# DegardinBruno/Kinetic-GAN

Measured on AMD Instinct MI355X. Metric: G+D train-step samples/sec, NTU (N,3,64,25) bs=64 at 1/2/4/8 MI355X, higher is better.
Workload: dtype f32; 1 GPU; ntu shapes (N,3,64,25), 60 classes, mlp4, G+D WGAN-GP iteration, 64 samples/GPU; global_batch=64, parallelism=dp1, launch=hipgraph

## Files before the change

include/kgan_hip.h:

```cpp
#ifndef KGAN_HIP_H
#define KGAN_HIP_H

#include <stdint.h>

#ifdef __cplusplus
extern "C" {
#endif

#define KG_ABI_VERSION 9

enum { KG_ACT_NONE = 0, KG_ACT_LRELU = 1, KG_ACT_TANH = 2 };
enum { KG_TAP_TIME = 0,
       KG_TAP_CHANBLOCK = 1  };

int         kg_abi_version(void);
const char* kg_arch(void);
const char* kg_last_error(void);
void        kg_reload_env(void);

typedef struct KgConvGroup {
    const float* x;  int64_t x_sN, x_sC;
    int32_t Cin, T_in, V_in;
    int32_t x_lead;
    const int32_t* vmap;
// ... 54 lines not shown
#define KG_WGRAD_TILE_32x64   3
#define KG_WGRAD_TILE_32x32   4
int     kg_wgrad_plan_info(const KgWgradArgs* a, int32_t* variant, int32_t* splits);

typedef struct KgWgradReduceJob {
    const float* ws;  float* dw;
    int64_t w_sT, w_sO, w_sI;
    int32_t taps, M, Cin, splits, accumulate;
} KgWgradReduceJob;
#define KG_WGRAD_REDUCE_MAX_JOBS 24
typedef struct KgWgradReduceJobs {
    int32_t njobs;
    KgWgradReduceJob job[KG_WGRAD_REDUCE_MAX_JOBS];
} KgWgradReduceJobs;
int     kg_wgrad_reduce_many(const KgWgradReduceJobs* jobs, void* stream);

int64_t kg_wgrad_many_workspace_bytes(const KgWgradArgs* jobs, int32_t njobs);
int     kg_wgrad_many(const KgWgradArgs* jobs, int32_t njobs, float* ws, int64_t ws_bytes, void* stream);
int     kg_wgrad_many_plan(const KgWgradArgs* jobs, int32_t njobs, int32_t* variant, int32_t* splits);

typedef struct KgAggArgs {
    int32_t N, C, K, V, W;
    int32_t T;
    int32_t rep;
    const float* a;
    const float* x;  int64_t x_sN, x_sC;
    const float* y;  int64_t y_sN, y_sC;
    float* out;  int64_t o_sN, o_sC;
    float* ws;  int64_t ws_bytes;
    int32_t a_transposed;
    int32_t defer_sum;
    const float* res;  int64_t r_sN, r_sC;  int32_t r_T, r_V, r_tstride;  const int32_t* r_inv;
    const float* mask;  int64_t m_sN, m_sC;  float slope;
} KgAggArgs;

int     kg_agg_expand(const KgAggArgs* a, void* stream);
int     kg_agg_reduce(const KgAggArgs* a, void* stream);
int64_t kg_agg_outer_workspace_bytes(const KgAggArgs* a);
int     kg_agg_outer(const KgAggArgs* a, void* stream);
int     kg_agg_outer_slabs(const KgAggArgs* a);
typedef struct KgOuterSumJob { const float* ws; float* out; int32_t nout, slabs; } KgOuterSumJob;
#define KG_OUTER_SUM_MAX_JOBS 16
typedef struct KgOuterSumJobs { int32_t njobs; KgOuterSumJob job[KG_OUTER_SUM_MAX_JOBS]; } KgOuterSumJobs;
int     kg_agg_outer_sum_many(const KgOuterSumJobs* jobs, void* stream);
int     kg_agg_outer_many(const KgAggArgs* jobs, int32_t njobs, void* stream);

typedef struct KgAggConvArgs {
    int32_t N, Cin, M, T, V, W, K;
    const float* x;  int64_t x_sN, x_sC;
    const float* a;  int32_t a_transposed;
    const int32_t* nbr;  int32_t pcount[3];
    const float* w;  int64_t w_sT, w_sO, w_sI;
    float* out;  int64_t o_sN, o_sC;
    const float* add;  int64_t a_sN, a_sC;  int32_t a_tstride;
    float* xa;  int64_t xa_sN, xa_sC;
} KgAggConvArgs;

int kg_aggconv_supported(const KgAggConvArgs* a);
int kg_aggconv(const KgAggConvArgs* a, void* stream);

typedef struct KgGenArgs {
    int32_t N, C, K, Cr, Tc, Vc, V, rep;
    const float* a;  const float* u;
    const float* b;
    const float* y;  float* y_out;  int64_t y_sN, y_sC;
    float* z;  int64_t z_sN, z_sC;
    float* zf;  int64_t zf_sN, zf_sC;
    const float* rs;  float* rs_out;  int64_t rs_sN, rs_sC;
    const float* rbias;
    float* r;  int64_t r_sN, r_sC;
} KgGenArgs;

int kg_gen_expand(const KgGenArgs* a, void* stream);
int kg_gen_fold(const KgGenArgs* a, void* stream);

typedef struct KgGenAdjJob {
    const float* dbt;
    const float* u;
    const float* a;
    float* out;
    int32_t K, Kd, V, Vc, accumulate;
} KgGenAdjJob;
#define KG_GEN_ADJ_MAX_JOBS 8
int kg_gen_adj_finish(const KgGenAdjJob* jobs, int32_t njobs, void* stream);

typedef struct KgGenPrepJob {
    const float* a;  const float* imp;  const float* u;
    float* aeff;  float* b;
    int32_t K, V, Vc;
} KgGenPrepJob;
int kg_gen_adj_prepare(const KgGenPrepJob* jobs, int32_t njobs, void* stream);

typedef struct KgGenTailArgs {
    int32_t N, C, T, V;  int32_t act;  float slope;
    const float* g;  int64_t g_sN, g_sC;
    const float* out;  int64_t o_sN, o_sC;
    const float* u;  int64_t u_sN, u_sC;  const float* mean_t;  const float* rstd_t;  const float* gamma_t;
    const float* r;  int64_t r_sN, r_sC;  const float* mean_r;  const float* rstd_r;  const float* gamma_r;
    const float* noise;
    float* coef;
    float* dgamma_t;  float* dbeta_t;  float* dgamma_r;  float* dbeta_r;  float* dnw;
    float* ws;  int64_t ws_bytes;  int32_t* counters;  int32_t counters_len;
    float* du;  int64_t du_sN, du_sC;
    float* dr;  int64_t dr_sN, dr_sC;
} KgGenTailArgs;
int64_t kg_gen_tail_workspace_bytes(const KgGenTailArgs* a);
int     kg_gen_tail_stats(const KgGenTailArgs* a, void* stream);
int     kg_gen_tail_apply(const KgGenTailArgs* a, void* stream);

typedef struct KgPlane { float* p;  int64_t sN, sC; } KgPlane;
typedef struct KgGenBnLayer {
    const float* gamma;  const float* beta;  float* running_mean;  float* running_var;  int64_t* num_batches_tracked;
    float momentum, eps;
    float* coef;
} KgGenBnLayer;
typedef struct KgGenBlockArgs {
    int32_t N, groups;
    int32_t Cin, C, K, Kp;
    int32_t Tc, Vc, T, V, rep;
    int32_t res_kind;
    int32_t bn_t;
    int32_t act;  float slope;
    KgPlane x;
    KgPlane pu, pr;  const float* pcoef_t;  const float* pcoef_r;  const float* pnoise;  const float* pnw;  int32_t pact;
    KgPlane xout;
    const float* wg;  const float* wr;  const float* br;  const float* wt;  const float* bt;
    const float* b;
    const float* u;
    KgPlane yc, z, r, uo;
    KgGenBnLayer bt_, br_;
    const float* noise;  const float* nw;  KgPlane out;
    float* ws;  int64_t ws_bytes;  int32_t* counters;  int32_t counters_len;
} KgGenBlockArgs;
typedef struct KgGenBlockBwdArgs {
    int32_t N;
    int32_t Cin, C, K, Kp, Tc, Vc, T, V, rep, res_kind, bn_t, act;  float slope;
    KgPlane g, out, uo, r;
    const float* coef;
    const float* wg;  const float* wr;  const float* wt;  const float* b;  const float* u;
    KgPlane du, dr, gyc, zf, gx;
    KgPlane px, pu, pr;  const float* pnoise;  int32_t pact;
    const float* pmean_t;  const float* prstd_t;  const float* pgamma_t;
    const float* pmean_r;  const float* prstd_r;  const float* pgamma_r;
    float* pcoef;  float* dgamma_t;  float* dbeta_t;  float* dgamma_r;  float* dbeta_r;  float* dnw;
    float* ws;  int64_t ws_bytes;  int32_t* counters;  int32_t counters_len;
} KgGenBlockBwdArgs;
int64_t kg_genblock_lds_bytes(const KgGenBlockArgs* a);
int64_t kg_genblock_workspace_bytes(const KgGenBlockArgs* a);
int     kg_genblock_fwd(const KgGenBlockArgs* a, void* stream);
int64_t kg_genblock_bwd_lds_bytes(const KgGenBlockBwdArgs* a);
int64_t kg_genblock_bwd_workspace_bytes(const KgGenBlockBwdArgs* a);
int     kg_genblock_bwd(const KgGenBlockBwdArgs* a, void* stream);

typedef struct KgRowsumArgs {
    int32_t N, C, T, V;
    const float* x;  int64_t x_sN, x_sC;
    const float* y;  int64_t y_sN, y_sC;
    const float* shift;
    int32_t want_second;
    float* out;
    float* ws;  int64_t ws_bytes;
    int32_t accumulate;
    float* out2;
} KgRowsumArgs;

int64_t kg_rowsum_workspace_bytes(const KgRowsumArgs* a);
int     kg_rowsum(const KgRowsumArgs* a, void* stream);
int64_t kg_rowsum_many_workspace_bytes(const KgRowsumArgs* jobs, int32_t njobs);
int     kg_rowsum_many(const KgRowsumArgs* jobs, int32_t njobs, float* ws, int64_t ws_bytes, void* stream);

typedef struct KgEltArgs {
    int32_t N, C, T, V;
    const float* x;  int64_t x_sN, x_sC;
    const float* r;  int64_t r_sN, r_sC;
    const float* noise;
    const float* sx; const float* bx; const float* sr; const float* br; const float* nw;
    float* out;  int64_t o_sN, o_sC;
    int32_t act;  float slope;
    int32_t groups;
    int64_t coef_gs;
} KgEltArgs;

int kg_act_bwd(const KgEltArgs* a, void* stream);
int kg_affine_act(const KgEltArgs* a, void* stream);

typedef struct KgBnArgs {
    int32_t N, C, T, V;
    const float* x;  int64_t x_sN, x_sC;
    const float* g;  int64_t g_sN, g_sC;
    const float* gamma; const float* beta;
    float* running_mean; float* running_var;
    int64_t* num_batches_tracked;
    const float* mean; const float* rstd;
    float momentum, eps;
    int32_t training;
    float* coef;
} KgBnArgs;

int kg_bn_fwd(const KgBnArgs* a, void* stream);
int kg_bn_bwd(const KgBnArgs* a, void* stream);

typedef struct KgBnJob {
    KgBnArgs a;
    int32_t groups;
} KgBnJob;

int64_t kg_bn_bwd_many_workspace_bytes(const KgBnArgs* jobs, int32_t njobs);
int     kg_bn_bwd_many(const KgBnArgs* jobs, int32_t njobs, float* ws, int64_t ws_bytes, int32_t* counters,
                       int32_t counters_len, void* stream);
int64_t kg_bn_fwd_many_workspace_bytes(const KgBnJob* jobs, int32_t njobs);
int     kg_bn_fwd_many(const KgBnJob* jobs, int32_t njobs, float* ws, int64_t ws_bytes, int32_t* counters,
                       int32_t counters_len, void* stream);

typedef struct KgGpArgs {
    int32_t N, C, T, V;
    const float* g;  int64_t g_sN, g_sC;
    float* nrm;
    float* gp;
    const float* gout;
    float* out;  int64_t o_sN, o_sC;
} KgGpArgs;

int kg_gp_fwd(const KgGpArgs* a, void* stream);
int kg_gp_bwd(const KgGpArgs* a, void* stream);

int kg_adam_step(float* p, const float* g, float* m, float* v, int64_t n,
                 float lr, float b1, float b2, float eps, const int32_t* step, float grad_scale,
                 void* stream);
int kg_adam_step_fused(float* p, float* g, float* m, float* v, int64_t n,
                       float lr, float b1, float b2, float eps, const int32_t* step, float grad_scale,
                       int32_t zero_grad, void* stream);
int kg_adam_step_ema(float* p, float* g, float* m, float* v, float* e, int64_t n,
                     float lr, float b1, float b2, float eps, const int32_t* step, float grad_scale,
                     int32_t zero_grad, float ema_decay, float ema_warmup, void* stream);

typedef struct KgHeadArgs {
    int32_t N, C, T, V;
    const float* h;  int64_t h_sN, h_sC;
    const float* w;  const float* b;
    float* v;
    const float* gv;
    float* g;  int64_t g_sN, g_sC;
    float slope;  int32_t masked;
    float* dw;  float* db;  int32_t accumulate;
} KgHeadArgs;
int kg_head_fwd(const KgHeadArgs* a, void* stream);
int kg_head_bwd(const KgHeadArgs* a, void* stream);
int kg_head_wgrad(const KgHeadArgs* a, void* stream);

typedef struct KgLabelBiasArgs {
    int32_t N, L, J, K, C, V, W, T;
    const int64_t* labels;
    const float* emb;
    const float* w;  int64_t w_sK, w_sC;
    const float* ak;
    float* zl;
    const float* gz;  int64_t gz_sN, gz_sC;
    float* demb;  float* dw;  int32_t accumulate;
    float* dak;  int32_t dak_accumulate;
    float* ws;  int64_t ws_bytes;
} KgLabelBiasArgs;
int     kg_label_bias_fwd(const KgLabelBiasArgs* a, void* stream);
int64_t kg_label_bias_workspace_bytes(const KgLabelBiasArgs* a);
int     kg_label_bias_bwd(const KgLabelBiasArgs* a, void* stream);
int     kg_aggconv_label(const KgAggConvArgs* a, const KgLabelBiasArgs* lb, void* stream);

typedef struct KgMixArgs {
    int32_t N, C, T, V;
    const float* real;  int64_t r_sN, r_sC;
    const float* fake;  int64_t f_sN, f_sC;
    const float* alpha;
    float* out;  int64_t o_sN, o_sC;
} KgMixArgs;
int kg_mix3(const KgMixArgs* a, void* stream);

typedef struct KgMaskedAdjArgs {
    int32_t n;
    const float* a;  const float* imp;  const int64_t* sel;
    float* ak;
    const float* g;  float* dimp;  int32_t accumulate;
} KgMaskedAdjArgs;
int kg_masked_adj_fwd(const KgMaskedAdjArgs* a, void* stream);
int kg_masked_adj_bwd(const KgMaskedAdjArgs* a, void* stream);

typedef struct KgLinearArgs {
    int32_t N, Din, Dout;
    int32_t L, J;
    const float* x;  int64_t x_ld;
    const float* emb;
    const int64_t* labels;
    const float* w;  const float* bias;
    float* y;  int64_t y_ld;
    int32_t act;  float slope;
    const float* g;  int64_t g_ld;
    float* gx;  int64_t gx_ld;  int32_t gx_cols;
    float* dw;  float* db;
    float* demb;
    int32_t accumulate;
} KgLinearArgs;
int kg_linear_fwd(const KgLinearArgs* a, void* stream);
int kg_linear_bwd(const KgLinearArgs* a, void* stream);
int kg_embed_bwd(const KgLinearArgs* a, void* stream);

#define KG_COMM_ID_BYTES 128
int kg_comm_unique_id(void* id);
int kg_comm_init(void** comm, int32_t rank, int32_t world, const void* id, int32_t device);
int kg_comm_world(const void* comm);
int kg_allreduce_flat(void* comm, float* buf, int64_t n, void* stream);
int kg_comm_destroy(void* comm);

int kg_peak_mfma_f32(float* sink, int32_t iters, double* flops, void* stream);
int kg_peak_copy(const float* src, float* dst, int64_t n, void* stream);

#define KG_MMD_MAX_BW 16
typedef struct KgMmdArgs {
    const float* x;  int64_t x_sp, x_sd, x_sg, x_sc;
    const float* y;  int64_t y_sp, y_sd, y_sg, y_sc;
    int32_t m, n, dim;
    int32_t groups, classes;
    int32_t nbw;
    double bw[KG_MMD_MAX_BW];
    float* mmd2;
    float* mmd;
    float* result;
    float* mean;
    void* ws;  int64_t ws_bytes;
} KgMmdArgs;
int64_t kg_mmd_workspace_bytes(const KgMmdArgs* a);
int     kg_mmd(const KgMmdArgs* a, void* stream);

#define KG_PRDC_MAX_K 32
#define KG_PRDC_MAX_POINTS 32768
typedef struct KgPrdcArgs {
    const float* real;  int64_t r_sc, r_sp, r_so;
    const float* fake;  int64_t f_sc, f_sp, f_so;
    int32_t n, m;
    int32_t d_outer, d_inner;
    int32_t classes, k;
    float* radii_real;
    float* radii_fake;
    int32_t* fake_hits;
    uint8_t* real_flags;
    int32_t* counts;
    float* values;
    float* mean;
    void* ws;  int64_t ws_bytes;
} KgPrdcArgs;
int64_t kg_prdc_workspace_bytes(const KgPrdcArgs* a);
int     kg_prdc(const KgPrdcArgs* a, void* stream);

#define KG_PRDC_MAX_SETS 4
typedef struct KgPrdcRadiiArgs {
    const float* x;  int64_t sc, sp, so;
    int32_t n, d_outer, d_inner, classes, k;
    float* radii;
} KgPrdcRadiiArgs;
typedef struct KgPrdcSetsArgs {
    const float* real;  int64_t r_sc, r_sp, r_so;
    const float* fake[KG_PRDC_MAX_SETS];  int64_t f_sc, f_sp, f_so;
    int32_t nsets;
    int32_t n, m;
    int32_t d_outer, d_inner;
    int32_t classes, k;
    const float* radii_real;
    float* radii_fake;
    int32_t* fake_hits;
    uint8_t* real_flags;
    int32_t* counts;
    float* values;
    float* mean;
    void* ws;  int64_t ws_bytes;
} KgPrdcSetsArgs;
int     kg_prdc_radii(const KgPrdcRadiiArgs* a, void* stream);
int64_t kg_prdc_sets_workspace_bytes(const KgPrdcSetsArgs* a);
int     kg_prdc_sets(const KgPrdcSetsArgs* a, void* stream);

#define KG_NN_MAX_K 32
#define KG_NN_MAX_POINTS 16777216
#define KG_NN_MAX_SPLIT 32
typedef struct KgNnArgs {
    const float* query;  int64_t q_sc, q_sp, q_so;
    const float* base;   int64_t b_sc, b_sp, b_so;
    int32_t Q, N;
    int32_t d_outer, d_inner;
    int32_t classes, k;
    int32_t exclude_self;
    int32_t q_affine, b_affine;
    float q_scale, q_shift, b_scale, b_shift;
    int32_t tile, split;
    int32_t* idx;
    float* d2;
    void* ws;  int64_t ws_bytes;
} KgNnArgs;
int64_t kg_nn_workspace_bytes(const KgNnArgs* a);
int     kg_nn(const KgNnArgs* a, void* stream);

#define KG_NN_MAX_SETS 4
#define KG_NN_SCORES_MAX_CLASSES 1024
typedef struct KgNnSetsArgs {
    const float* query[KG_NN_MAX_SETS];  int64_t q_sc, q_sp, q_so;
    int32_t nsets;
    const float* base;   int64_t b_sc, b_sp, b_so;
    int32_t Q, N;
    int32_t d_outer, d_inner;
    int32_t classes, k;
    int32_t q_affine, b_affine;
    float q_scale, q_shift, b_scale, b_shift;
    int32_t tile, split;
    int32_t* idx;
    float* d2;
    void* ws;  int64_t ws_bytes;
} KgNnSetsArgs;
typedef struct KgNnScoresArgs {
    int32_t nsets, Q, N, n_classes;
    int64_t ld;
    const int32_t* idx;  const float* d2;
    const int32_t* query_labels;
    const int32_t* base_labels;
    const float* base_loo;
    int64_t* counts;
    int32_t* counts_per_class;
    double* scores64;  float* scores;
} KgNnScoresArgs;
int64_t kg_nn_sets_workspace_bytes(const KgNnSetsArgs* a);
int     kg_nn_sets(const KgNnSetsArgs* a, void* stream);
int     kg_nn_scores(const KgNnScoresArgs* a, void* stream);

#define KG_NN_NORM_PARTS 64
typedef struct KgNnGramArgs {
    const float* query[KG_NN_MAX_SETS];  int64_t q_sc, q_sp, q_so;
    int32_t nsets;
    const float* base;   int64_t b_sc, b_sp, b_so;
    int32_t Q, N;
    int32_t d_outer, d_inner;
    int32_t classes, k;
    int32_t exclude_self;
    int32_t q_affine, b_affine;
    float q_scale, q_shift, b_scale, b_shift;
    int32_t cand;
    int32_t tile, split;
    const float* b_norms;
    const float* b_norm_parts;
    int32_t* idx;
    float* d2;
    int32_t* stats;
    void* ws;  int64_t ws_bytes;
} KgNnGramArgs;
int     kg_nn_norms(const KgNnGramArgs* a, float* norms, float* parts, void* stream);
int64_t kg_nn_gram_workspace_bytes(const KgNnGramArgs* a);
int     kg_nn_gram(const KgNnGramArgs* a, void* stream);

#define KG_FRECHET_MAX_DIM 96
typedef struct KgFrechetArgs {
    const float* real;  int64_t r_sc, r_ss, r_sf, r_so;
    const float* fake;  int64_t f_sc, f_ss, f_sf, f_so;
    int32_t n, m;
    int32_t frames;
    int32_t diff;
    int32_t d_outer, d_inner;
    int32_t classes;
    double* values;
    double* terms;
    double* mean;
    int32_t* sweeps;
    double* mu_real;
    double* mu_fake;
    double* cov_real;
    double* cov_fake;
    void* ws;  int64_t ws_bytes;
} KgFrechetArgs;
int64_t kg_frechet_workspace_bytes(const KgFrechetArgs* a);
int     kg_frechet(const KgFrechetArgs* a, void* stream);

#define KG_FRECHET_MAX_SETS 4
typedef struct KgFrechetRealArgs {
    const float* real;  int64_t r_sc, r_ss, r_sf, r_so;
    int32_t n;
    int32_t frames, diff;
    int32_t d_outer, d_inner;
    int32_t classes;
    double* mu_real;
    double* tr_real;
    double* G;
    int32_t* sweeps_real;
    void* ws;  int64_t ws_bytes;
} KgFrechetRealArgs;
typedef struct KgFrechetSetsArgs {
    const float* fake[KG_FRECHET_MAX_SETS];  int64_t f_sc, f_ss, f_sf, f_so;
    int32_t nsets;
    int32_t m;
    int32_t frames, diff;
    int32_t d_outer, d_inner;
    int32_t classes;
    const double* mu_real;
    const double* tr_real;
    const double* G;
    double* values;
    double* terms;
    int32_t* sweeps;
    double* mean;
    float* mean32;
    void* ws;  int64_t ws_bytes;
} KgFrechetSetsArgs;
int64_t kg_frechet_real_workspace_bytes(const KgFrechetRealArgs* a);
int     kg_frechet_real(const KgFrechetRealArgs* a, void* stream);
int64_t kg_frechet_sets_workspace_bytes(const KgFrechetSetsArgs* a);
int     kg_frechet_sets(const KgFrechetSetsArgs* a, void* stream);

#define KG_STEP_MAX_PLANES 8
#define KG_STREAM_Z 0
#define KG_STREAM_ALPHA 1
#define KG_STREAM_NOISE_D 2
#define KG_STREAM_NOISE_G 3
typedef struct KgStepInputsArgs {
    int64_t* step;
    int32_t* ticket;
    uint64_t seed;
    int32_t rank, world;
    int32_t B;
    int32_t C, T, V;
    const float* data;  int64_t d_sN, d_sC, d_sT, d_sV;
    int64_t n_rows;
    const int64_t* label_src;
    const int64_t* perm;  int64_t perm_stride;
    int64_t batches_per_epoch;
    float scale, shift;
    float* real;
    int64_t* labels;
    float* z;  int32_t latent;
    float* alpha;
    float* noise;  int32_t n_planes;  int64_t plane_len[KG_STEP_MAX_PLANES];
} KgStepInputsArgs;
int kg_step_inputs(const KgStepInputsArgs* a, void* stream);
int kg_loss_append(float* ring, int64_t ring_len, const int64_t* step, const float* d_loss, const float* g_loss,
                   void* stream);

#define KG_BN_EVAL_MAX_JOBS 8
typedef struct KgBnEvalJob {
    int32_t C;
    const float* gamma;  const float* beta;  const float* running_mean;  const float* running_var;
    float eps;
    float* coef;
} KgBnEvalJob;
int kg_bn_eval_coef(const KgBnEvalJob* jobs, int32_t njobs, void* stream);

typedef struct KgGenBlockInferArgs {
    int32_t N;
    int32_t Cin, C, K, Kp, Tc, Vc, T, V, rep, res_kind, act;  float slope;
    KgPlane x;
    const float* wg;  const float* wr;  const float* br;  const float* wt;  const float* bt;
    const float* b;
    const float* u;
    const float* coef_t;  const float* coef_r;
    const float* noise;  const float* nw;
    KgPlane out;
} KgGenBlockInferArgs;
int64_t kg_genblock_infer_lds_bytes(const KgGenBlockInferArgs* a);
int     kg_genblock_infer(const KgGenBlockInferArgs* a, void* stream);

#define KG_STREAM_SAMPLE 0x100
typedef struct KgSampleInputsArgs {
    int64_t* step;
    int32_t* ticket;
    uint64_t seed;
    int32_t B, latent;
    float* z;
    float* noise;  int64_t noise_len;
    float* t;  int32_t t_rows, t_cols;
} KgSampleInputsArgs;
int kg_sample_inputs(const KgSampleInputsArgs* a, void* stream);

int kg_trunc_lerp(float* x, int64_t x_ld, int32_t N, int32_t D, const float* t, int64_t t_ld, int32_t M, float truncation,
                  void* stream);

#define KG_EVAL_MAX_SCORES 8
typedef struct KgEvalRecordArgs {
    const float* scores[KG_EVAL_MAX_SCORES];
    int32_t nscores, select;
    const int64_t* iter;
    int64_t* count;
    float* ring_val;
    int64_t* ring_iter;
    int64_t ring_len;
    float* best_val;
    int64_t* best_iter;
    int32_t* flag;
} KgEvalRecordArgs;
int kg_eval_record(const KgEvalRecordArgs* a, void* stream);

#define KG_EVAL2_MAX_SCORES 32
typedef struct KgEvalRecord2Args {
    const float* scores[KG_EVAL2_MAX_SCORES];
    int32_t nscores, select;
    const int64_t* iter;
    int64_t* count;
    float* ring_val;
    int64_t* ring_iter;
    int64_t ring_len;
    float* best_val;
    int64_t* best_iter;
    int32_t* flag;
    int32_t maximise;
} KgEvalRecord2Args;
int kg_eval_record2(const KgEvalRecord2Args* a, void* stream);

#define KG_EVAL3_MAX_SCORES 64
// ... 124 lines not shown
```

kinetic-gan_amd/_native.py:

```python
from __future__ import annotations

import ctypes as C
import os
from typing import NamedTuple, Optional, Sequence, Tuple

import torch

_PKG = os.path.dirname(os.path.abspath(__file__))
LIB_PATH = os.environ.get("KG_LIB") or os.path.join(_PKG, "libkgan_hip.so")

ACT_NONE, ACT_LRELU, ACT_TANH = 0, 1, 2
ABI_VERSION = 9
TAP_TIME, TAP_CHANBLOCK = 0, 1

c_f32p = C.c_void_p
c_i32p = C.c_void_p


class _ConvGroup(C.Structure):
    _fields_ = [("x", c_f32p), ("x_sN", C.c_int64), ("x_sC", C.c_int64),
                ("Cin", C.c_int32), ("T_in", C.c_int32), ("V_in", C.c_int32),
                ("x_lead", C.c_int32),
                ("vmap", c_i32p),
                ("w", c_f32p), ("w_sT", C.c_int64), ("w_sO", C.c_int64), ("w_sI", C.c_int64),
                ("w_sMB", C.c_int64), ("w_MB", C.c_int32),
                ("taps", C.c_int32), ("tap_mode", C.c_int32), ("t_stride", C.c_int32),
                ("transposed", C.c_int32)]


class _ConvArgs(C.Structure):
    _fields_ = [("N", C.c_int32), ("M", C.c_int32), ("T_out", C.c_int32), ("V_out", C.c_int32),
                ("out", c_f32p), ("o_sN", C.c_int64), ("o_sC", C.c_int64),
                ("ngroups", C.c_int32),
                ("g", _ConvGroup * 2),
                ("bias0", c_f32p), ("bias1", c_f32p),
                ("add", c_f32p), ("a_sN", C.c_int64), ("a_sC", C.c_int64), ("a_tstride", C.c_int32),
                ("act", C.c_int32), ("slope", C.c_float),
                ("ws", c_f32p), ("ws_bytes", C.c_int64),
                ("mask", c_f32p), ("m_sN", C.c_int64), ("m_sC", C.c_int64),
                ("sync", C.c_void_p), ("sync_len", C.c_int32),
                ("o_tstride", C.c_int32),
                ("wpack", C.c_void_p), ("wpack_bytes", C.c_int64)]


class _WgradPair(C.Structure):
    _fields_ = [("N", C.c_int32),
                ("g", c_f32p), ("g_sN", C.c_int64), ("g_sC", C.c_int64),
                ("x", c_f32p), ("x_sN", C.c_int64), ("x_sC", C.c_int64)]


class _WgradArgs(C.Structure):
    _fields_ = [("N", C.c_int32), ("M", C.c_int32), ("T_out", C.c_int32), ("V_out", C.c_int32),
                ("g", c_f32p), ("g_sN", C.c_int64), ("g_sC", C.c_int64),
                ("x", c_f32p), ("x_sN", C.c_int64), ("x_sC", C.c_int64),
                ("Cin", C.c_int32), ("T_in", C.c_int32), ("V_in", C.c_int32),
                ("vmap", c_i32p),
                ("taps", C.c_int32), ("tap_mode", C.c_int32), ("t_stride", C.c_int32),
                ("dw", c_f32p), ("w_sT", C.c_int64), ("w_sO", C.c_int64), ("w_sI", C.c_int64),
                ("ws", c_f32p), ("ws_bytes", C.c_int64), ("accumulate", C.c_int32),
                ("nextra", C.c_int32), ("extra", _WgradPair * 2), ("defer_reduce", C.c_int32)]


class _WgradReduceJob(C.Structure):
    _fields_ = [("ws", c_f32p), ("dw", c_f32p), ("w_sT", C.c_int64), ("w_sO", C.c_int64), ("w_sI", C.c_int64),
                ("taps", C.c_int32), ("M", C.c_int32), ("Cin", C.c_int32), ("splits", C.c_int32),
                ("accumulate", C.c_int32)]


WGRAD_REDUCE_MAX_JOBS = 24
WGRAD_TILE_128x128, WGRAD_TILE_64x64, WGRAD_TILE_64x32, WGRAD_TILE_32x64, WGRAD_TILE_32x32 = 0, 1, 2, 3, 4
WGRAD_TILE_NAMES = {WGRAD_TILE_128x128: "128x128", WGRAD_TILE_64x64: "64x64", WGRAD_TILE_64x32: "64x32",
                    WGRAD_TILE_32x64: "32x64", WGRAD_TILE_32x32: "32x32"}
WGRAD_MAX_SPLITS = 128


class _WgradReduceJobs(C.Structure):
    _fields_ = [("njobs", C.c_int32), ("job", _WgradReduceJob * WGRAD_REDUCE_MAX_JOBS)]


class _AggArgs(C.Structure):
    _fields_ = [("N", C.c_int32), ("C", C.c_int32), ("K", C.c_int32), ("V", C.c_int32), ("W", C.c_int32),
                ("T", C.c_int32), ("rep", C.c_int32),
                ("a", c_f32p),
                ("x", c_f32p), ("x_sN", C.c_int64), ("x_sC", C.c_int64),
                ("y", c_f32p), ("y_sN", C.c_int64), ("y_sC", C.c_int64),
                ("out", c_f32p), ("o_sN", C.c_int64), ("o_sC", C.c_int64),
                ("ws", c_f32p), ("ws_bytes", C.c_int64), ("a_transposed", C.c_int32), ("defer_sum", C.c_int32),
                ("res", c_f32p), ("r_sN", C.c_int64), ("r_sC", C.c_int64), ("r_T", C.c_int32), ("r_V", C.c_int32),
                ("r_tstride", C.c_int32), ("r_inv", c_i32p),
                ("mask", c_f32p), ("m_sN", C.c_int64), ("m_sC", C.c_int64), ("slope", C.c_float)]


class _OuterSumJob(C.Structure):
    _fields_ = [("ws", c_f32p), ("out", c_f32p), ("nout", C.c_int32), ("slabs", C.c_int32)]


OUTER_SUM_MAX_JOBS = 16


class _OuterSumJobs(C.Structure):
    _fields_ = [("njobs", C.c_int32), ("job", _OuterSumJob * OUTER_SUM_MAX_JOBS)]


class _AggConvArgs(C.Structure):
    _fields_ = [("N", C.c_int32), ("Cin", C.c_int32), ("M", C.c_int32), ("T", C.c_int32), ("V", C.c_int32),
                ("W", C.c_int32), ("K", C.c_int32),
                ("x", c_f32p), ("x_sN", C.c_int64), ("x_sC", C.c_int64),
                ("a", c_f32p), ("a_transposed", C.c_int32),
                ("nbr", c_i32p), ("pcount", C.c_int32 * 3),
                ("w", c_f32p), ("w_sT", C.c_int64), ("w_sO", C.c_int64), ("w_sI", C.c_int64),
                ("out", c_f32p), ("o_sN", C.c_int64), ("o_sC", C.c_int64),
                ("add", c_f32p), ("a_sN", C.c_int64), ("a_sC", C.c_int64), ("a_tstride", C.c_int32),
                ("xa", c_f32p), ("xa_sN", C.c_int64), ("xa_sC", C.c_int64)]


class _RowsumArgs(C.Structure):
    _fields_ = [("N", C.c_int32), ("C", C.c_int32), ("T", C.c_int32), ("V", C.c_int32),
                ("x", c_f32p), ("x_sN", C.c_int64), ("x_sC", C.c_int64),
                ("y", c_f32p), ("y_sN", C.c_int64), ("y_sC", C.c_int64),
                ("shift", c_f32p),
                ("want_second", C.c_int32),
                ("out", c_f32p),
                ("ws", c_f32p), ("ws_bytes", C.c_int64), ("accumulate", C.c_int32), ("out2", c_f32p)]


class _BnArgs(C.Structure):
    _fields_ = [("N", C.c_int32), ("C", C.c_int32), ("T", C.c_int32), ("V", C.c_int32),
                ("x", c_f32p), ("x_sN", C.c_int64), ("x_sC", C.c_int64),
                ("g", c_f32p), ("g_sN", C.c_int64), ("g_sC", C.c_int64),
                ("gamma", c_f32p), ("beta", c_f32p),
                ("running_mean", c_f32p), ("running_var", c_f32p),
                ("num_batches_tracked", C.c_void_p),
                ("mean", c_f32p), ("rstd", c_f32p),
                ("momentum", C.c_float), ("eps", C.c_float),
                ("training", C.c_int32),
                ("coef", c_f32p)]


class _BnJob(C.Structure):
    _fields_ = [("a", _BnArgs), ("groups", C.c_int32)]


class _GpArgs(C.Structure):
    _fields_ = [("N", C.c_int32), ("C", C.c_int32), ("T", C.c_int32), ("V", C.c_int32),
                ("g", c_f32p), ("g_sN", C.c_int64), ("g_sC", C.c_int64),
                ("nrm", c_f32p), ("gp", c_f32p), ("gout", c_f32p),
                ("out", c_f32p), ("o_sN", C.c_int64), ("o_sC", C.c_int64)]


class _EltArgs(C.Structure):
    _fields_ = [("N", C.c_int32), ("C", C.c_int32), ("T", C.c_int32), ("V", C.c_int32),
                ("x", c_f32p), ("x_sN", C.c_int64), ("x_sC", C.c_int64),
                ("r", c_f32p), ("r_sN", C.c_int64), ("r_sC", C.c_int64),
                ("noise", c_f32p),
                ("sx", c_f32p), ("bx", c_f32p), ("sr", c_f32p), ("br", c_f32p), ("nw", c_f32p),
                ("out", c_f32p), ("o_sN", C.c_int64), ("o_sC", C.c_int64),
                ("act", C.c_int32), ("slope", C.c_float),
                ("groups", C.c_int32), ("coef_gs", C.c_int64)]


class _GenArgs(C.Structure):
    _fields_ = [("N", C.c_int32), ("C", C.c_int32), ("K", C.c_int32), ("Cr", C.c_int32), ("Tc", C.c_int32),
                ("Vc", C.c_int32), ("V", C.c_int32), ("rep", C.c_int32),
                ("a", c_f32p), ("u", c_f32p), ("b", c_f32p),
                ("y", c_f32p), ("y_out", c_f32p), ("y_sN", C.c_int64), ("y_sC", C.c_int64),
                ("z", c_f32p), ("z_sN", C.c_int64), ("z_sC", C.c_int64),
                ("zf", c_f32p), ("zf_sN", C.c_int64), ("zf_sC", C.c_int64),
                ("rs", c_f32p), ("rs_out", c_f32p), ("rs_sN", C.c_int64), ("rs_sC", C.c_int64),
                ("rbias", c_f32p),
                ("r", c_f32p), ("r_sN", C.c_int64), ("r_sC", C.c_int64)]


class _GenAdjJob(C.Structure):
    _fields_ = [("dbt", c_f32p), ("u", c_f32p), ("a", c_f32p), ("out", c_f32p),
                ("K", C.c_int32), ("Kd", C.c_int32), ("V", C.c_int32), ("Vc", C.c_int32), ("accumulate", C.c_int32)]


class _HeadArgs(C.Structure):
    _fields_ = [("N", C.c_int32), ("C", C.c_int32), ("T", C.c_int32), ("V", C.c_int32),
                ("h", c_f32p), ("h_sN", C.c_int64), ("h_sC", C.c_int64),
                ("w", c_f32p), ("b", c_f32p), ("v", c_f32p), ("gv", c_f32p),
                ("g", c_f32p), ("g_sN", C.c_int64), ("g_sC", C.c_int64),
                ("slope", C.c_float), ("masked", C.c_int32),
                ("dw", c_f32p), ("db", c_f32p), ("accumulate", C.c_int32)]


class _LinearArgs(C.Structure):
    _fields_ = [("N", C.c_int32), ("Din", C.c_int32), ("Dout", C.c_int32), ("L", C.c_int32), ("J", C.c_int32),
                ("x", c_f32p), ("x_ld", C.c_int64), ("emb", c_f32p), ("labels", C.c_void_p),
                ("w", c_f32p), ("bias", c_f32p), ("y", c_f32p), ("y_ld", C.c_int64),
                ("act", C.c_int32), ("slope", C.c_float),
                ("g", c_f32p), ("g_ld", C.c_int64),
                ("gx", c_f32p), ("gx_ld", C.c_int64), ("gx_cols", C.c_int32),
                ("dw", c_f32p), ("db", c_f32p), ("demb", c_f32p), ("accumulate", C.c_int32)]


class _LabelBiasArgs(C.Structure):
    _fields_ = [("N", C.c_int32), ("L", C.c_int32), ("J", C.c_int32), ("K", C.c_int32), ("C", C.c_int32),
                ("V", C.c_int32), ("W", C.c_int32), ("T", C.c_int32),
                ("labels", C.c_void_p), ("emb", c_f32p),
                ("w", c_f32p), ("w_sK", C.c_int64), ("w_sC", C.c_int64),
                ("ak", c_f32p), ("zl", c_f32p),
                ("gz", c_f32p), ("gz_sN", C.c_int64), ("gz_sC", C.c_int64),
                ("demb", c_f32p), ("dw", c_f32p), ("accumulate", C.c_int32),
                ("dak", c_f32p), ("dak_accumulate", C.c_int32),
                ("ws", c_f32p), ("ws_bytes", C.c_int64)]


class _MixArgs(C.Structure):
    _fields_ = [("N", C.c_int32), ("C", C.c_int32), ("T", C.c_int32), ("V", C.c_int32),
                ("real", c_f32p), ("r_sN", C.c_int64), ("r_sC", C.c_int64),
                ("fake", c_f32p), ("f_sN", C.c_int64), ("f_sC", C.c_int64),
                ("alpha", c_f32p),
                ("out", c_f32p), ("o_sN", C.c_int64), ("o_sC", C.c_int64)]


class _MaskedAdjArgs(C.Structure):
    _fields_ = [("n", C.c_int32), ("a", c_f32p), ("imp", c_f32p), ("sel", C.c_void_p), ("ak", c_f32p),
                ("g", c_f32p), ("dimp", c_f32p), ("accumulate", C.c_int32)]


class _GenTailArgs(C.Structure):
    _fields_ = [("N", C.c_int32), ("C", C.c_int32), ("T", C.c_int32), ("V", C.c_int32), ("act", C.c_int32), ("slope", C.c_float),
                ("g", c_f32p), ("g_sN", C.c_int64), ("g_sC", C.c_int64),
                ("out", c_f32p), ("o_sN", C.c_int64), ("o_sC", C.c_int64),
                ("u", c_f32p), ("u_sN", C.c_int64), ("u_sC", C.c_int64), ("mean_t", c_f32p), ("rstd_t", c_f32p), ("gamma_t", c_f32p),
                ("r", c_f32p), ("r_sN", C.c_int64), ("r_sC", C.c_int64), ("mean_r", c_f32p), ("rstd_r", c_f32p), ("gamma_r", c_f32p),
                ("noise", c_f32p), ("coef", c_f32p),
                ("dgamma_t", c_f32p), ("dbeta_t", c_f32p), ("dgamma_r", c_f32p), ("dbeta_r", c_f32p), ("dnw", c_f32p),
                ("ws", c_f32p), ("ws_bytes", C.c_int64), ("counters", C.c_void_p), ("counters_len", C.c_int32),
                ("du", c_f32p), ("du_sN", C.c_int64), ("du_sC", C.c_int64),
                ("dr", c_f32p), ("dr_sN", C.c_int64), ("dr_sC", C.c_int64)]


class _GenPrepJob(C.Structure):
    _fields_ = [("a", c_f32p), ("imp", c_f32p), ("u", c_f32p), ("aeff", c_f32p), ("b", c_f32p),
                ("K", C.c_int32), ("V", C.c_int32), ("Vc", C.c_int32)]


class _Plane(C.Structure):
    _fields_ = [("p", c_f32p), ("sN", C.c_int64), ("sC", C.c_int64)]


class _GenBnLayer(C.Structure):
    _fields_ = [("gamma", c_f32p), ("beta", c_f32p), ("running_mean", c_f32p), ("running_var", c_f32p),
                ("num_batches_tracked", C.c_void_p), ("momentum", C.c_float), ("eps", C.c_float), ("coef", c_f32p)]


class _GenBlockArgs(C.Structure):
    _fields_ = [("N", C.c_int32), ("groups", C.c_int32),
                ("Cin", C.c_int32), ("C", C.c_int32), ("K", C.c_int32), ("Kp", C.c_int32),
                ("Tc", C.c_int32), ("Vc", C.c_int32), ("T", C.c_int32), ("V", C.c_int32), ("rep", C.c_int32),
                ("res_kind", C.c_int32), ("bn_t", C.c_int32), ("act", C.c_int32), ("slope", C.c_float),
                ("x", _Plane),
                ("pu", _Plane), ("pr", _Plane), ("pcoef_t", c_f32p), ("pcoef_r", c_f32p), ("pnoise", c_f32p), ("pnw", c_f32p),
                ("pact", C.c_int32), ("xout", _Plane),
                ("wg", c_f32p), ("wr", c_f32p), ("br", c_f32p), ("wt", c_f32p), ("bt", c_f32p),
                ("b", c_f32p), ("u", c_f32p),
                ("yc", _Plane), ("z", _Plane), ("r", _Plane), ("uo", _Plane),
                ("bt_", _GenBnLayer), ("br_", _GenBnLayer),
                ("noise", c_f32p), ("nw", c_f32p), ("out", _Plane),
                ("ws", c_f32p), ("ws_bytes", C.c_int64), ("counters", C.c_void_p), ("counters_len", C.c_int32)]


class _GenBlockBwdArgs(C.Structure):
    _fields_ = [("N", C.c_int32),
                ("Cin", C.c_int32), ("C", C.c_int32), ("K", C.c_int32), ("Kp", C.c_int32),
                ("Tc", C.c_int32), ("Vc", C.c_int32), ("T", C.c_int32), ("V", C.c_int32), ("rep", C.c_int32),
                ("res_kind", C.c_int32), ("bn_t", C.c_int32), ("act", C.c_int32), ("slope", C.c_float),
                ("g", _Plane), ("out", _Plane), ("uo", _Plane), ("r", _Plane),
                ("coef", c_f32p),
                ("wg", c_f32p), ("wr", c_f32p), ("wt", c_f32p), ("b", c_f32p), ("u", c_f32p),
                ("du", _Plane), ("dr", _Plane), ("gyc", _Plane), ("zf", _Plane), ("gx", _Plane),
                ("px", _Plane), ("pu", _Plane), ("pr", _Plane), ("pnoise", c_f32p), ("pact", C.c_int32),
                ("pmean_t", c_f32p), ("prstd_t", c_f32p), ("pgamma_t", c_f32p),
                ("pmean_r", c_f32p), ("prstd_r", c_f32p), ("pgamma_r", c_f32p),
                ("pcoef", c_f32p), ("dgamma_t", c_f32p), ("dbeta_t", c_f32p), ("dgamma_r", c_f32p), ("dbeta_r", c_f32p),
                ("dnw", c_f32p),
                ("ws", c_f32p), ("ws_bytes", C.c_int64), ("counters", C.c_void_p), ("counters_len", C.c_int32)]



MMD_MAX_BW = 16


class _MmdArgs(C.Structure):
    _fields_ = [("x", c_f32p), ("x_sp", C.c_int64), ("x_sd", C.c_int64), ("x_sg", C.c_int64), ("x_sc", C.c_int64),
                ("y", c_f32p), ("y_sp", C.c_int64), ("y_sd", C.c_int64), ("y_sg", C.c_int64), ("y_sc", C.c_int64),
                ("m", C.c_int32), ("n", C.c_int32), ("dim", C.c_int32),
                ("groups", C.c_int32), ("classes", C.c_int32), ("nbw", C.c_int32),
                ("bw", C.c_double * MMD_MAX_BW),
                ("mmd2", c_f32p), ("mmd", c_f32p), ("result", c_f32p), ("mean", c_f32p),
                ("ws", C.c_void_p), ("ws_bytes", C.c_int64)]

PRDC_MAX_K = 32
PRDC_MAX_POINTS = 32768


class _PrdcArgs(C.Structure):
    _fields_ = [("real", c_f32p), ("r_sc", C.c_int64), ("r_sp", C.c_int64), ("r_so", C.c_int64),
                ("fake", c_f32p), ("f_sc", C.c_int64), ("f_sp", C.c_int64), ("f_so", C.c_int64),
                ("n", C.c_int32), ("m", C.c_int32), ("d_outer", C.c_int32), ("d_inner", C.c_int32),
                ("classes", C.c_int32), ("k", C.c_int32),
                ("radii_real", c_f32p), ("radii_fake", c_f32p), ("fake_hits", C.c_void_p), ("real_flags", C.c_void_p),
                ("counts", C.c_void_p), ("values", c_f32p), ("mean", c_f32p),
                ("ws", C.c_void_p), ("ws_bytes", C.c_int64)]

PRDC_MAX_SETS = 4


class _PrdcRadiiArgs(C.Structure):
    _fields_ = [("x", c_f32p), ("sc", C.c_int64), ("sp", C.c_int64), ("so", C.c_int64),
                ("n", C.c_int32), ("d_outer", C.c_int32), ("d_inner", C.c_int32), ("classes", C.c_int32), ("k", C.c_int32),
                ("radii", c_f32p)]


class _PrdcSetsArgs(C.Structure):
    _fields_ = [("real", c_f32p), ("r_sc", C.c_int64), ("r_sp", C.c_int64), ("r_so", C.c_int64),
                ("fake", c_f32p * PRDC_MAX_SETS), ("f_sc", C.c_int64), ("f_sp", C.c_int64), ("f_so", C.c_int64),
                ("nsets", C.c_int32), ("n", C.c_int32), ("m", C.c_int32), ("d_outer", C.c_int32), ("d_inner", C.c_int32),
                ("classes", C.c_int32), ("k", C.c_int32),
                ("radii_real", c_f32p), ("radii_fake", c_f32p), ("fake_hits", C.c_void_p), ("real_flags", C.c_void_p),
                ("counts", C.c_void_p), ("values", c_f32p), ("mean", c_f32p),
                ("ws", C.c_void_p), ("ws_bytes", C.c_int64)]

NN_MAX_K = 32
NN_MAX_POINTS = 1 << 24
NN_MAX_SPLIT = 32


class _NnArgs(C.Structure):
    _fields_ = [("query", c_f32p), ("q_sc", C.c_int64), ("q_sp", C.c_int64), ("q_so", C.c_int64),
                ("base", c_f32p), ("b_sc", C.c_int64), ("b_sp", C.c_int64), ("b_so", C.c_int64),
                ("Q", C.c_int32), ("N", C.c_int32), ("d_outer", C.c_int32), ("d_inner", C.c_int32),
                ("classes", C.c_int32), ("k", C.c_int32), ("exclude_self", C.c_int32),
                ("q_affine", C.c_int32), ("b_affine", C.c_int32),
                ("q_scale", C.c_float), ("q_shift", C.c_float), ("b_scale", C.c_float), ("b_shift", C.c_float),
                ("tile", C.c_int32), ("split", C.c_int32),
                ("idx", C.c_void_p), ("d2", c_f32p),
                ("ws", C.c_void_p), ("ws_bytes", C.c_int64)]

NN_MAX_SETS = 4
NN_SCORES_MAX_CLASSES = 1024


class _NnSetsArgs(C.Structure):
    _fields_ = [("query", c_f32p * NN_MAX_SETS), ("q_sc", C.c_int64), ("q_sp", C.c_int64), ("q_so", C.c_int64),
                ("nsets", C.c_int32),
                ("base", c_f32p), ("b_sc", C.c_int64), ("b_sp", C.c_int64), ("b_so", C.c_int64),
                ("Q", C.c_int32), ("N", C.c_int32), ("d_outer", C.c_int32), ("d_inner", C.c_int32),
                ("classes", C.c_int32), ("k", C.c_int32),
                ("q_affine", C.c_int32), ("b_affine", C.c_int32),
                ("q_scale", C.c_float), ("q_shift", C.c_float), ("b_scale", C.c_float), ("b_shift", C.c_float),
                ("tile", C.c_int32), ("split", C.c_int32),
                ("idx", C.c_void_p), ("d2", c_f32p),
                ("ws", C.c_void_p), ("ws_bytes", C.c_int64)]


NN_NORM_PARTS = 64


class _NnGramArgs(C.Structure):
    _fields_ = [("query", c_f32p * NN_MAX_SETS), ("q_sc", C.c_int64), ("q_sp", C.c_int64), ("q_so", C.c_int64),
                ("nsets", C.c_int32),
                ("base", c_f32p), ("b_sc", C.c_int64), ("b_sp", C.c_int64), ("b_so", C.c_int64),
                ("Q", C.c_int32), ("N", C.c_int32), ("d_outer", C.c_int32), ("d_inner", C.c_int32),
                ("classes", C.c_int32), ("k", C.c_int32), ("exclude_self", C.c_int32),
                ("q_affine", C.c_int32), ("b_affine", C.c_int32),
                ("q_scale", C.c_float), ("q_shift", C.c_float), ("b_scale", C.c_float), ("b_shift", C.c_float),
                ("cand", C.c_int32), ("tile", C.c_int32), ("split", C.c_int32),
                ("b_norms", c_f32p), ("b_norm_parts", c_f32p),
                ("idx", C.c_void_p), ("d2", c_f32p), ("stats", C.c_void_p),
                ("ws", C.c_void_p), ("ws_bytes", C.c_int64)]


class _NnScoresArgs(C.Structure):
    _fields_ = [("nsets", C.c_int32), ("Q", C.c_int32), ("N", C.c_int32), ("n_classes", C.c_int32),
                ("ld", C.c_int64),
                ("idx", C.c_void_p), ("d2", c_f32p),
                ("query_labels", C.c_void_p), ("base_labels", C.c_void_p), ("base_loo", c_f32p),
                ("counts", C.c_void_p), ("counts_per_class", C.c_void_p),
                ("scores64", C.c_void_p), ("scores", c_f32p)]

FRECHET_MAX_DIM = 96


class _FrechetArgs(C.Structure):
    _fields_ = [("real", c_f32p), ("r_sc", C.c_int64), ("r_ss", C.c_int64), ("r_sf", C.c_int64), ("r_so", C.c_int64),
                ("fake", c_f32p), ("f_sc", C.c_int64), ("f_ss", C.c_int64), ("f_sf", C.c_int64), ("f_so", C.c_int64),
                ("n", C.c_int32), ("m", C.c_int32), ("frames", C.c_int32), ("diff", C.c_int32),
                ("d_outer", C.c_int32), ("d_inner", C.c_int32), ("classes", C.c_int32),
                ("values", C.c_void_p), ("terms", C.c_void_p), ("mean", C.c_void_p), ("sweeps", C.c_void_p),
                ("mu_real", C.c_void_p), ("mu_fake", C.c_void_p), ("cov_real", C.c_void_p), ("cov_fake", C.c_void_p),
                ("ws", C.c_void_p), ("ws_bytes", C.c_int64)]

FRECHET_MAX_SETS = 4


class _FrechetRealArgs(C.Structure):
    _fields_ = [("real", c_f32p), ("r_sc", C.c_int64), ("r_ss", C.c_int64), ("r_sf", C.c_int64), ("r_so", C.c_int64),
                ("n", C.c_int32), ("frames", C.c_int32), ("diff", C.c_int32),
                ("d_outer", C.c_int32), ("d_inner", C.c_int32), ("classes", C.c_int32),
                ("mu_real", C.c_void_p), ("tr_real", C.c_void_p), ("G", C.c_void_p), ("sweeps_real", C.c_void_p),
                ("ws", C.c_void_p), ("ws_bytes", C.c_int64)]


class _FrechetSetsArgs(C.Structure):
    _fields_ = [("fake", c_f32p * FRECHET_MAX_SETS), ("f_sc", C.c_int64), ("f_ss", C.c_int64), ("f_sf", C.c_int64),
                ("f_so", C.c_int64),
                ("nsets", C.c_int32), ("m", C.c_int32), ("frames", C.c_int32), ("diff", C.c_int32),
                ("d_outer", C.c_int32), ("d_inner", C.c_int32), ("classes", C.c_int32),
                ("mu_real", C.c_void_p), ("tr_real", C.c_void_p), ("G", C.c_void_p),
                ("values", C.c_void_p), ("terms", C.c_void_p), ("sweeps", C.c_void_p), ("mean", C.c_void_p),
                ("mean32", c_f32p),
                ("ws", C.c_void_p), ("ws_bytes", C.c_int64)]

KIN_DESC = 6
KIN_MAX_JOINTS, KIN_MAX_BONES, KIN_MAX_MIRROR = 32, 32, 16
KIN_MIN_FRAMES = 4
KIN_MAX_ELEMS = 32768
KIN_MAX_SETS = 4
KIN_MAX_POINTS = 16384


class _KinDescArgs(C.Structure):
    _fields_ = [("x", c_f32p), ("sc", C.c_int64), ("ss", C.c_int64), ("sf", C.c_int64), ("so", C.c_int64),
                ("n", C.c_int32), ("T", C.c_int32), ("C", C.c_int32), ("V", C.c_int32), ("classes", C.c_int32),
                ("B", C.c_int32), ("M", C.c_int32),
                ("bones", C.c_void_p), ("mirror", C.c_void_p), ("still_eps", C.c_double),
                ("desc", c_f32p), ("degenerate", C.c_void_p),
                ("ws", c_f32p), ("ws_bytes", C.c_int64), ("counters", C.c_void_p), ("counters_len", C.c_int32)]


class _KinDescSetsArgs(C.Structure):
    _fields_ = [("x", c_f32p * KIN_MAX_SETS), ("sc", C.c_int64), ("ss", C.c_int64), ("sf", C.c_int64), ("so", C.c_int64),
                ("nsets", C.c_int32),
                ("n", C.c_int32), ("T", C.c_int32), ("C", C.c_int32), ("V", C.c_int32), ("classes", C.c_int32),
                ("B", C.c_int32), ("M", C.c_int32),
                ("bones", C.c_void_p), ("mirror", C.c_void_p), ("still_eps", C.c_double),
                ("desc", c_f32p * KIN_MAX_SETS), ("degenerate", C.c_void_p),
                ("ws", c_f32p), ("ws_bytes", C.c_int64), ("counters", C.c_void_p), ("counters_len", C.c_int32)]


class _KinScoresArgs(C.Structure):
    _fields_ = [("real", c_f32p), ("fake", c_f32p * KIN_MAX_SETS),
                ("nsets", C.c_int32), ("n", C.c_int32), ("m", C.c_int32), ("classes", C.c_int32),
                ("mean_real", C.c_void_p), ("mean_fake", C.c_void_p), ("w1", C.c_void_p), ("w1_mean", C.c_void_p),
                ("scores", c_f32p), ("nonfinite", C.c_void_p)]

STEP_MAX_PLANES = 8
STREAM_Z, STREAM_ALPHA, STREAM_NOISE_D, STREAM_NOISE_G = 0, 1, 2, 3


class _StepInputsArgs(C.Structure):
    _fields_ = [("step", C.c_void_p), ("ticket", C.c_void_p), ("seed", C.c_uint64),
                ("rank", C.c_int32), ("world", C.c_int32), ("B", C.c_int32),
                ("C", C.c_int32), ("T", C.c_int32), ("V", C.c_int32),
                ("data", c_f32p), ("d_sN", C.c_int64), ("d_sC", C.c_int64), ("d_sT", C.c_int64), ("d_sV", C.c_int64),
                ("n_rows", C.c_int64), ("label_src", C.c_void_p),
                ("perm", C.c_void_p), ("perm_stride", C.c_int64), ("batches_per_epoch", C.c_int64),
                ("scale", C.c_float), ("shift", C.c_float),
                ("real", c_f32p), ("labels", C.c_void_p),
                ("z", c_f32p), ("latent", C.c_int32), ("alpha", c_f32p),
                ("noise", c_f32p), ("n_planes", C.c_int32), ("plane_len", C.c_int64 * STEP_MAX_PLANES)]

BN_EVAL_MAX_JOBS = 8
STREAM_SAMPLE = 0x100


class _BnEvalJob(C.Structure):
    _fields_ = [("C", C.c_int32), ("gamma", c_f32p), ("beta", c_f32p), ("running_mean", c_f32p), ("running_var", c_f32p),
                ("eps", C.c_float), ("coef", c_f32p)]


class _GenBlockInferArgs(C.Structure):
    _fields_ = [("N", C.c_int32),
                ("Cin", C.c_int32), ("C", C.c_int32), ("K", C.c_int32), ("Kp", C.c_int32),
                ("Tc", C.c_int32), ("Vc", C.c_int32), ("T", C.c_int32), ("V", C.c_int32), ("rep", C.c_int32),
                ("res_kind", C.c_int32), ("act", C.c_int32), ("slope", C.c_float),
                ("x", _Plane),
                ("wg", c_f32p), ("wr", c_f32p), ("br", c_f32p), ("wt", c_f32p), ("bt", c_f32p),
                ("b", c_f32p), ("u", c_f32p),
                ("coef_t", c_f32p), ("coef_r", c_f32p),
                ("noise", c_f32p), ("nw", c_f32p), ("out", _Plane)]


class _SampleInputsArgs(C.Structure):
    _fields_ = [("step", C.c_void_p), ("ticket", C.c_void_p), ("seed", C.c_uint64),
                ("B", C.c_int32), ("latent", C.c_int32), ("z", c_f32p),
                ("noise", c_f32p), ("noise_len", C.c_int64),
                ("t", c_f32p), ("t_rows", C.c_int32), ("t_cols", C.c_int32)]

GEN_ADJ_MAX_JOBS = 8
EVAL_MAX_SCORES = 8
COPY_IF_MAX_JOBS = 32


def _eval_record_struct(name: str, most: int, sense: bool):
    fields = [("scores", c_f32p * most), ("nscores", C.c_int32), ("select", C.c_int32),
              ("iter", C.c_void_p), ("count", C.c_void_p), ("ring_val", c_f32p), ("ring_iter", C.c_void_p),
              ("ring_len", C.c_int64), ("best_val", c_f32p), ("best_iter", C.c_void_p), ("flag", C.c_void_p)]
    return type(name, (C.Structure,), {"_fields_": fields + ([("maximise", C.c_int32)] if sense else [])})


EVAL2_MAX_SCORES = 32
EVAL3_MAX_SCORES = 64
_EvalRecordArgs = _eval_record_struct("_EvalRecordArgs", EVAL_MAX_SCORES, False)
_EvalRecord2Args = _eval_record_struct("_EvalRecord2Args", EVAL2_MAX_SCORES, True)
_EvalRecord3Args = _eval_record_struct("_EvalRecord3Args", EVAL3_MAX_SCORES, True)


class _CopyJob(C.Structure):
    _fields_ = [("src", C.c_void_p), ("dst", C.c_void_p), ("nwords", C.c_int64)]


CLS_TILE = 4
CLS_MAX_C = 1024
CLS_MAX_CLASSES = 1024


class _ClsHeadArgs(C.Structure):
    _fields_ = [("N", C.c_int32), ("C", C.c_int32), ("T", C.c_int32), ("V", C.c_int32), ("F", C.c_int32), ("L", C.c_int32),
                ("h", c_f32p), ("h_sN", C.c_int64), ("h_sC", C.c_int64),
                ("w1", c_f32p), ("b1", c_f32p), ("w2", c_f32p), ("b2", c_f32p),
                ("labels", C.c_void_p),
                ("slope", C.c_float), ("masked", C.c_int32),
                ("pooled", c_f32p), ("feat", c_f32p), ("logits", c_f32p), ("loss_per_sample", c_f32p),
                ("pred", C.c_void_p), ("loss", c_f32p), ("correct", C.c_void_p),
                ("gtop", c_f32p),
                ("g", c_f32p), ("g_sN", C.c_int64), ("g_sC", C.c_int64),
                ("dw1", c_f32p), ("db1", c_f32p), ("dw2", c_f32p), ("db2", c_f32p), ("accumulate", C.c_int32),
                ("ws", C.c_void_p), ("ws_bytes", C.c_int64)]


CLS_MAX_SETS = 4


class _ClsScoresArgs(C.Structure):
    _fields_ = [("nsets", C.c_int32), ("N", C.c_int32), ("F", C.c_int32), ("K", C.c_int32), ("Sd", C.c_int32), ("Sl", C.c_int32),
                ("feat_ld", C.c_int64),
                ("feat", c_f32p * CLS_MAX_SETS), ("pred", C.c_void_p * CLS_MAX_SETS),
                ("labels", C.c_void_p), ("div_pairs", C.c_void_p), ("mm_pairs", C.c_void_p),
                ("dist", C.c_void_p), ("scores64", C.c_void_p), ("scores", c_f32p),
                ("correct", C.c_void_p), ("correct_per_class", C.c_void_p), ("count_per_class", C.c_void_p)]


EXPORTS = {
    "kg_abi_version": (C.c_int, []),
    "kg_arch": (C.c_char_p, []),
    "kg_last_error": (C.c_char_p, []),
    "kg_reload_env": (None, []),
    "kg_peak_mfma_f32": (C.c_int, [C.c_void_p, C.c_int32, C.POINTER(C.c_double), C.c_void_p]),
    "kg_peak_copy": (C.c_int, [C.c_void_p, C.c_void_p, C.c_int64, C.c_void_p]),
    "kg_conv_workspace_bytes": (C.c_int64, [C.POINTER(_ConvArgs)]),
    "kg_conv_plan_info": (C.c_int, [C.POINTER(_ConvArgs), C.POINTER(C.c_int32), C.POINTER(C.c_int32)]),
    "kg_conv": (C.c_int, [C.POINTER(_ConvArgs), C.c_void_p]),
    "kg_conv_pack_bytes": (C.c_int64, [C.POINTER(_ConvArgs)]),
    "kg_conv_pack": (C.c_int, [C.POINTER(_ConvArgs), C.c_void_p, C.c_int64, C.c_void_p]),
    "kg_conv_many": (C.c_int, [C.POINTER(_ConvArgs), C.c_int32, C.c_void_p]),
    "kg_conv_many_plan": (C.c_int, [C.POINTER(_ConvArgs), C.c_int32, C.POINTER(C.c_int32)]),
    "kg_wgrad_workspace_bytes": (C.c_int64, [C.POINTER(_WgradArgs)]),
    "kg_wgrad": (C.c_int, [C.POINTER(_WgradArgs), C.c_void_p]),
    "kg_wgrad_plan_info": (C.c_int, [C.POINTER(_WgradArgs), C.POINTER(C.c_int32), C.POINTER(C.c_int32)]),
    "kg_wgrad_reduce_many": (C.c_int, [C.POINTER(_WgradReduceJobs), C.c_void_p]),
    "kg_wgrad_many_workspace_bytes": (C.c_int64, [C.POINTER(_WgradArgs), C.c_int32]),
    "kg_wgrad_many": (C.c_int, [C.POINTER(_WgradArgs), C.c_int32, C.c_void_p, C.c_int64, C.c_void_p]),
    "kg_wgrad_many_plan": (C.c_int, [C.POINTER(_WgradArgs), C.c_int32, C.POINTER(C.c_int32), C.POINTER(C.c_int32)]),
    "kg_aggconv_supported": (C.c_int, [C.POINTER(_AggConvArgs)]),
    "kg_aggconv": (C.c_int, [C.POINTER(_AggConvArgs), C.c_void_p]),
    "kg_agg_expand": (C.c_int, [C.POINTER(_AggArgs), C.c_void_p]),
    "kg_agg_reduce": (C.c_int, [C.POINTER(_AggArgs), C.c_void_p]),
    "kg_agg_outer_workspace_bytes": (C.c_int64, [C.POINTER(_AggArgs)]),
    "kg_agg_outer": (C.c_int, [C.POINTER(_AggArgs), C.c_void_p]),
    "kg_agg_outer_slabs": (C.c_int, [C.POINTER(_AggArgs)]),
    "kg_agg_outer_many": (C.c_int, [C.POINTER(_AggArgs), C.c_int32, C.c_void_p]),
    "kg_agg_outer_sum_many": (C.c_int, [C.POINTER(_OuterSumJobs), C.c_void_p]),
    "kg_gen_expand": (C.c_int, [C.POINTER(_GenArgs), C.c_void_p]),
    "kg_gen_fold": (C.c_int, [C.POINTER(_GenArgs), C.c_void_p]),
    "kg_gen_adj_finish": (C.c_int, [C.POINTER(_GenAdjJob), C.c_int32, C.c_void_p]),
    "kg_gen_tail_workspace_bytes": (C.c_int64, [C.POINTER(_GenTailArgs)]),
    "kg_gen_tail_stats": (C.c_int, [C.POINTER(_GenTailArgs), C.c_void_p]),
    "kg_gen_tail_apply": (C.c_int, [C.POINTER(_GenTailArgs), C.c_void_p]),
    "kg_gen_adj_prepare": (C.c_int, [C.POINTER(_GenPrepJob), C.c_int32, C.c_void_p]),
    "kg_genblock_lds_bytes": (C.c_int64, [C.POINTER(_GenBlockArgs)]),
    "kg_genblock_workspace_bytes": (C.c_int64, [C.POINTER(_GenBlockArgs)]),
    "kg_genblock_fwd": (C.c_int, [C.POINTER(_GenBlockArgs), C.c_void_p]),
    "kg_genblock_bwd_lds_bytes": (C.c_int64, [C.POINTER(_GenBlockBwdArgs)]),
    "kg_genblock_bwd_workspace_bytes": (C.c_int64, [C.POINTER(_GenBlockBwdArgs)]),
    "kg_genblock_bwd": (C.c_int, [C.POINTER(_GenBlockBwdArgs), C.c_void_p]),
    "kg_head_fwd": (C.c_int, [C.POINTER(_HeadArgs), C.c_void_p]),
    "kg_head_bwd": (C.c_int, [C.POINTER(_HeadArgs), C.c_void_p]),
    "kg_head_wgrad": (C.c_int, [C.POINTER(_HeadArgs), C.c_void_p]),
    "kg_linear_fwd": (C.c_int, [C.POINTER(_LinearArgs), C.c_void_p]),
    "kg_linear_bwd": (C.c_int, [C.POINTER(_LinearArgs), C.c_void_p]),
    "kg_embed_bwd": (C.c_int, [C.POINTER(_LinearArgs), C.c_void_p]),
    "kg_label_bias_fwd": (C.c_int, [C.POINTER(_LabelBiasArgs), C.c_void_p]),
    "kg_label_bias_workspace_bytes": (C.c_int64, [C.POINTER(_LabelBiasArgs)]),
    "kg_label_bias_bwd": (C.c_int, [C.POINTER(_LabelBiasArgs), C.c_void_p]),
    "kg_aggconv_label": (C.c_int, [C.POINTER(_AggConvArgs), C.POINTER(_LabelBiasArgs), C.c_void_p]),
    "kg_mix3": (C.c_int, [C.POINTER(_MixArgs), C.c_void_p]),
    "kg_masked_adj_fwd": (C.c_int, [C.POINTER(_MaskedAdjArgs), C.c_void_p]),
    "kg_masked_adj_bwd": (C.c_int, [C.POINTER(_MaskedAdjArgs), C.c_void_p]),
    "kg_rowsum_workspace_bytes": (C.c_int64, [C.POINTER(_RowsumArgs)]),
    "kg_rowsum": (C.c_int, [C.POINTER(_RowsumArgs), C.c_void_p]),
    "kg_rowsum_many_workspace_bytes": (C.c_int64, [C.POINTER(_RowsumArgs), C.c_int32]),
    "kg_rowsum_many": (C.c_int, [C.POINTER(_RowsumArgs), C.c_int32, C.c_void_p, C.c_int64, C.c_void_p]),
    "kg_bn_fwd": (C.c_int, [C.POINTER(_BnArgs), C.c_void_p]),
    "kg_bn_bwd_many_workspace_bytes": (C.c_int64, [C.POINTER(_BnArgs), C.c_int32]),
    "kg_bn_bwd_many": (C.c_int, [C.POINTER(_BnArgs), C.c_int32, c_f32p, C.c_int64, C.c_void_p, C.c_int32, C.c_void_p]),
    "kg_bn_fwd_many_workspace_bytes": (C.c_int64, [C.POINTER(_BnJob), C.c_int32]),
    "kg_bn_fwd_many": (C.c_int, [C.POINTER(_BnJob), C.c_int32, c_f32p, C.c_int64, C.c_void_p, C.c_int32, C.c_void_p]),
    "kg_bn_bwd": (C.c_int, [C.POINTER(_BnArgs), C.c_void_p]),
    "kg_gp_fwd": (C.c_int, [C.POINTER(_GpArgs), C.c_void_p]),
    "kg_gp_bwd": (C.c_int, [C.POINTER(_GpArgs), C.c_void_p]),
    "kg_act_bwd": (C.c_int, [C.POINTER(_EltArgs), C.c_void_p]),
    "kg_affine_act": (C.c_int, [C.POINTER(_EltArgs), C.c_void_p]),
    "kg_comm_unique_id": (C.c_int, [C.c_void_p]),
    "kg_comm_init": (C.c_int, [C.POINTER(C.c_void_p), C.c_int32, C.c_int32, C.c_void_p, C.c_int32]),
    "kg_comm_world": (C.c_int, [C.c_void_p]),
    "kg_allreduce_flat": (C.c_int, [C.c_void_p, C.c_void_p, C.c_int64, C.c_void_p]),
    "kg_comm_destroy": (C.c_int, [C.c_void_p]),
    "kg_adam_step": (C.c_int, [C.c_void_p, C.c_void_p, C.c_void_p, C.c_void_p, C.c_int64, C.c_float, C.c_float,
                               C.c_float, C.c_float, C.c_void_p, C.c_float, C.c_void_p]),
    "kg_mmd_workspace_bytes": (C.c_int64, [C.POINTER(_MmdArgs)]),
    "kg_mmd": (C.c_int, [C.POINTER(_MmdArgs), C.c_void_p]),
    "kg_prdc_workspace_bytes": (C.c_int64, [C.POINTER(_PrdcArgs)]),
    "kg_prdc": (C.c_int, [C.POINTER(_PrdcArgs), C.c_void_p]),
    "kg_prdc_radii": (C.c_int, [C.POINTER(_PrdcRadiiArgs), C.c_void_p]),
    "kg_prdc_sets_workspace_bytes": (C.c_int64, [C.POINTER(_PrdcSetsArgs)]),
    "kg_prdc_sets": (C.c_int, [C.POINTER(_PrdcSetsArgs), C.c_void_p]),
    "kg_nn_workspace_bytes": (C.c_int64, [C.POINTER(_NnArgs)]),
    "kg_nn": (C.c_int, [C.POINTER(_NnArgs), C.c_void_p]),
    "kg_nn_sets_workspace_bytes": (C.c_int64, [C.POINTER(_NnSetsArgs)]),
    "kg_nn_sets": (C.c_int, [C.POINTER(_NnSetsArgs), C.c_void_p]),
    "kg_nn_scores": (C.c_int, [C.POINTER(_NnScoresArgs), C.c_void_p]),
    "kg_nn_norms": (C.c_int, [C.POINTER(_NnGramArgs), C.c_void_p, C.c_void_p, C.c_void_p]),
    "kg_nn_gram_workspace_bytes": (C.c_int64, [C.POINTER(_NnGramArgs)]),
    "kg_nn_gram": (C.c_int, [C.POINTER(_NnGramArgs), C.c_void_p]),
    "kg_frechet_workspace_bytes": (C.c_int64, [C.POINTER(_FrechetArgs)]),
    "kg_frechet": (C.c_int, [C.POINTER(_FrechetArgs), C.c_void_p]),
    "kg_frechet_real_workspace_bytes": (C.c_int64, [C.POINTER(_FrechetRealArgs)]),
    "kg_frechet_real": (C.c_int, [C.POINTER(_FrechetRealArgs), C.c_void_p]),
    "kg_frechet_sets_workspace_bytes": (C.c_int64, [C.POINTER(_FrechetSetsArgs)]),
    "kg_frechet_sets": (C.c_int, [C.POINTER(_FrechetSetsArgs), C.c_void_p]),
    "kg_step_inputs": (C.c_int, [C.POINTER(_StepInputsArgs), C.c_void_p]),
    "kg_loss_append": (C.c_int, [C.c_void_p, C.c_int64, C.c_void_p, C.c_void_p, C.c_void_p, C.c_void_p]),
    "kg_adam_step_fused": (C.c_int, [C.c_void_p, C.c_void_p, C.c_void_p, C.c_void_p, C.c_int64, C.c_float, C.c_float,
                                     C.c_float, C.c_float, C.c_void_p, C.c_float, C.c_int32, C.c_void_p]),
    "kg_adam_step_ema": (C.c_int, [C.c_void_p, C.c_void_p, C.c_void_p, C.c_void_p, C.c_void_p, C.c_int64, C.c_float, C.c_float,
                                   C.c_float, C.c_float, C.c_void_p, C.c_float, C.c_int32, C.c_float, C.c_float, C.c_void_p]),
    "kg_bn_eval_coef": (C.c_int, [C.POINTER(_BnEvalJob), C.c_int32, C.c_void_p]),
    "kg_genblock_infer_lds_bytes": (C.c_int64, [C.POINTER(_GenBlockInferArgs)]),
    "kg_genblock_infer": (C.c_int, [C.POINTER(_GenBlockInferArgs), C.c_void_p]),
    "kg_sample_inputs": (C.c_int, [C.POINTER(_SampleInputsArgs), C.c_void_p]),
    "kg_trunc_lerp": (C.c_int, [C.c_void_p, C.c_int64, C.c_int32, C.c_int32, C.c_void_p, C.c_int64, C.c_int32, C.c_float,
                                C.c_void_p]),
    "kg_eval_record": (C.c_int, [C.POINTER(_EvalRecordArgs), C.c_void_p]),
    "kg_eval_record2": (C.c_int, [C.POINTER(_EvalRecord2Args), C.c_void_p]),
    "kg_eval_record3": (C.c_int, [C.POINTER(_EvalRecord3Args), C.c_void_p]),
    "kg_copy_if": (C.c_int, [C.c_void_p, C.POINTER(_CopyJob), C.c_int32, C.c_void_p]),
    "kg_cls_head_workspace_bytes": (C.c_int64, [C.POINTER(_ClsHeadArgs)]),
    "kg_cls_head_fwd": (C.c_int, [C.POINTER(_ClsHeadArgs), C.c_void_p]),
    "kg_cls_head_bwd": (C.c_int, [C.POINTER(_ClsHeadArgs), C.c_void_p]),
    "kg_cls_head_wgrad": (C.c_int, [C.POINTER(_ClsHeadArgs), C.c_void_p]),
    "kg_cls_scores": (C.c_int, [C.POINTER(_ClsScoresArgs), C.c_void_p]),
    "kg_kin_desc_workspace_bytes": (C.c_int64, [C.POINTER(_KinDescArgs)]),
    "kg_kin_desc_lds_bytes": (C.c_int64, [C.POINTER(_KinDescArgs)]),
    "kg_kin_desc": (C.c_int, [C.POINTER(_KinDescArgs), C.c_void_p]),
    "kg_kin_desc_sets_workspace_bytes": (C.c_int64, [C.POINTER(_KinDescSetsArgs)]),
    "kg_kin_desc_sets_lds_bytes": (C.c_int64, [C.POINTER(_KinDescSetsArgs)]),
    "kg_kin_desc_sets": (C.c_int, [C.POINTER(_KinDescSetsArgs), C.c_void_p]),
    "kg_kin_scores_lds_bytes": (C.c_int64, [C.POINTER(_KinScoresArgs)]),
    "kg_kin_scores": (C.c_int, [C.POINTER(_KinScoresArgs), C.c_void_p]),
}

_lib = None


def load_library():
    global _lib
    if _lib is not None:
        return _lib
    if not os.path.exists(LIB_PATH):
        raise RuntimeError(
            f"{LIB_PATH} is missing: run `python -c 'import __graft_entry__ as g; g.build()'` "
            "(hipcc --offload-arch=gfx950). There is no CPU fallback for the st_gcn path.")
    lib = C.CDLL(LIB_PATH)
    for name, (res, args) in EXPORTS.items():
        fn = getattr(lib, name)
        fn.restype = res
        fn.argtypes = args
    if lib.kg_abi_version() != ABI_VERSION:
        raise RuntimeError("libkgan_hip.so ABI version mismatch")
    _lib = lib
    return lib


def _check(rc: int, what: str):
    if rc != 0:
        msg = load_library().kg_last_error().decode()
        raise RuntimeError(f"{what} failed (rc={rc}): {msg}")


def _stream() -> int:
    return torch.cuda.current_stream().cuda_stream


def peak_mfma_f32(sink: torch.Tensor, iters: int) -> float:
    fl = C.c_double(0.0)
    _check(load_library().kg_peak_mfma_f32(sink.data_ptr(), int(iters), C.byref(fl), _stream()), "kg_peak_mfma_f32")
    return fl.value


def peak_copy(src: torch.Tensor, dst: torch.Tensor) -> int:
    n = src.numel()
    _check(load_library().kg_peak_copy(src.data_ptr(), dst.data_ptr(), n, _stream()), "kg_peak_copy")
    return 8 * n


def reload_env():
    load_library().kg_reload_env()


SYNC_LEN = 8192
_sync_bufs = {}


def _sync_buffer(device) -> torch.Tensor:
    key = (device.index, torch.cuda.current_stream(device).cuda_stream)
    buf = _sync_bufs.get(key)
    if buf is None:
        buf = _sync_bufs[key] = torch.zeros(SYNC_LEN, dtype=torch.int32, device=device)
    return buf



def is_plane(x: torch.Tensor) -> bool:
    if x.dim() != 4:
        return False
    n, c, t, v = x.shape
    return (v == 1 or x.stride(3) == 1) and (t == 1 or x.stride(2) == v)


def as_plane(x: torch.Tensor) -> torch.Tensor:
    if x.dtype != torch.float32:
        raise TypeError(f"st_gcn path is fp32 only, got {x.dtype}")
    if is_plane(x):
        return x
    out = new_plane(x.shape[0], x.shape[1], x.shape[2], x.shape[3], x.device)
    out.copy_(x)
    return out


PLANE_LEAD = 32


def new_plane(n, c, t, v, device, zero=False) -> torch.Tensor:
    numel = c * n * t * v
    buf = (torch.zeros if zero else torch.empty)(numel + PLANE_LEAD, dtype=torch.float32, device=device)
    return buf[PLANE_LEAD:].view(c, n, t, v).permute(1, 0, 2, 3)


def _sn_sc(x: torch.Tensor):
    n, c, t, v = x.shape
    sn = x.stride(0) if n > 1 else t * v
    sc = x.stride(1) if c > 1 else t * v
    return sn, sc


def _need_cuda(*ts):
    cur = None
    for t in ts:
        if t is None:
            continue
        if not t.is_cuda:
            raise RuntimeError("kinetic_gan_amd: the st_gcn hot path runs on the GPU only "
                               "(tensor on %s); there is no CPU fallback" % t.device)
        if cur is None:
            cur = torch.cuda.current_device()
        if t.device.index != cur:
            raise RuntimeError("kinetic_gan_amd: tensor on %s but the current device is cuda:%d - select the device "
                               "first (torch.cuda.set_device / `with torch.cuda.device(...)`)" % (t.device, cur))


def _ptr(t: Optional[torch.Tensor]):
    return None if t is None else t.data_ptr()


def _bind(a, field: str, pre: str, t: torch.Tensor, convert: bool = False) -> torch.Tensor:
    if convert:
        t = as_plane(t)
    setattr(a, field, t.data_ptr())
    sn, sc = _sn_sc(t)
    setattr(a, pre + "_sN", sn)
    setattr(a, pre + "_sC", sc)
    return t


def _query(query: str, a, count: Optional[int] = None) -> int:
    fn = getattr(load_library(), query)
    nbytes = fn(C.byref(a)) if count is None else fn(a, count)
    if nbytes < 0:
        _check(-1, query)
    return nbytes


def _workspace(query: str, a, device, count: Optional[int] = None, tickets: Optional[str] = None, lazy: bool = False):
    nbytes = _query(query, a, count)
    if lazy and nbytes == 0:
        return None
    ws = torch.empty(nbytes // 4 if lazy else max(1, nbytes // 4), dtype=torch.float32, device=device)
    if count is None:
        a.ws, a.ws_bytes = ws.data_ptr(), nbytes if lazy else ws.numel() * 4
        if tickets is not None:
            sync = _sync_buffer(device)
            setattr(a, tickets, sync.data_ptr())
            setattr(a, tickets + "_len", sync.numel())
    return ws


def _dest(t: torch.Tensor, n: int, msg: str) -> torch.Tensor:
    if t.numel() != n or not t.is_contiguous() or t.dtype != torch.float32:
        raise ValueError(msg)
    return t


def _chunks(jobs: Sequence, most: int):
    for i in range(0, len(jobs), most):
        yield jobs[i:i + most]



class WView(NamedTuple):
    sT: int
    sO: int
    sI: int
    sMB: int = 0
    MB: int = 1 << 30


class Group(NamedTuple):
    x: torch.Tensor
    w: torch.Tensor
    wv: WView
    Cin: int
    taps: int = 1
    tap_mode: int = TAP_TIME
    t_stride: int = 1
    transposed: bool = False
    vmap: Optional[torch.Tensor] = None


last_conv_plan = None

flop_count = None


def _count(kind: str, flops: float):
    if flop_count is not None:
        flop_count[kind] = flop_count.get(kind, 0.0) + float(flops)


def _conv_args(groups: Sequence[Group], N: int, M: int, T_out: int, V_out: int,
               bias0=None, bias1=None, add=None, add_tstride: int = 1,
               act: int = ACT_NONE, slope: float = 0.2, mask=None, out: Optional[torch.Tensor] = None, out_t0: int = 0,
               out_tstride: int = 1, wpack: Optional[torch.Tensor] = None, alloc_out: bool = True):
    a = _ConvArgs()
    if wpack is not None:
        _need_cuda(wpack)
        a.wpack, a.wpack_bytes = wpack.data_ptr(), wpack.numel() * wpack.element_size()
    a.N, a.M, a.T_out, a.V_out = N, M, T_out, V_out
    keep = []
    dev = groups[0].x.device
    a.ngroups = len(groups)
    for i, g in enumerate(groups):
        x = as_plane(g.x)
        w = g.w if g.w.is_contiguous() else g.w.contiguous()
        _need_cuda(x, w, g.vmap)
        keep += [x, w]
        cg = a.g[i]
        _bind(cg, "x", "x", x)
        cg.Cin, cg.T_in, cg.V_in = g.Cin, x.shape[2], x.shape[3]
        cg.x_lead = min(int(x.storage_offset()), 1 << 20)
        cg.vmap = _ptr(g.vmap)
        cg.w = w.data_ptr()
        cg.w_sT, cg.w_sO, cg.w_sI, cg.w_sMB = g.wv.sT, g.wv.sO, g.wv.sI, g.wv.sMB
        cg.w_MB = min(g.wv.MB, 1 << 30)
        cg.taps, cg.tap_mode, cg.t_stride, cg.transposed = g.taps, g.tap_mode, g.t_stride, int(g.transposed)
    if out is None and not alloc_out:
        pass
    elif out is None:
        out = new_plane(N, M, T_out, V_out, dev)
        a.out = out.data_ptr()
    else:
        if (not is_plane(out) or out.shape[0] != N or out.shape[1] != M or out.shape[3] != V_out
                or out_t0 + (T_out - 1) * out_tstride >= out.shape[2] or out_tstride < 1 or out_t0 < 0):
            raise ValueError("conv: out must be a plane tensor (N, M, T, V_out) that holds frames out_t0 + to * out_tstride")
        _need_cuda(out)
# ... 404 lines not shown
    gy = grs = zf = None
    if gz is not None:
        gz = as_plane(gz)
        c = gz.shape[1]
        a.C, a.K = c, K
        _bind(a, "z", "z", gz)
        gy = y_out if y_out is not None else new_plane(n, K * c, tc, vc, gz.device)
        assert tuple(gy.shape) == (n, K * c, tc, vc) and is_plane(gy)
        _bind(a, "y_out", "y", gy)
        if want_zf:
            zf = gz if rep == 1 else _bind(a, "zf", "zf", new_plane(n, c, tc, v, gz.device))
        _count("kg_agg", 2.0 * K * vc * v * c * n * tf)
    if gr is not None:
        gr = as_plane(gr)
        a.Cr = gr.shape[1]
        _bind(a, "r", "r", gr)
        grs = rs_out if rs_out is not None else new_plane(n, gr.shape[1], tc, vc, gr.device)
        assert tuple(grs.shape) == (n, gr.shape[1], tc, vc) and is_plane(grs)
        _bind(a, "rs_out", "rs", grs)
        _count("kg_agg", 2.0 * vc * v * gr.shape[1] * n * tf)
    _check(lib.kg_gen_fold(C.byref(a), _stream()), "kg_gen_fold")
    return gy, grs, zf


def gen_tail_bwd(g, out, act: int, u=None, bn_t=None, r=None, bn_r=None, noise=None, sinks=None, slope: float = 0.2,
                 coef: Optional[torch.Tensor] = None, stats_only: bool = False):
    lib = load_library()
    g, out = as_plane(g), as_plane(out)
    n, c, t, v = g.shape
    sinks = sinks or {}
    a = _GenTailArgs()
    a.N, a.C, a.T, a.V, a.act, a.slope = n, c, t, v, act, slope
    _bind(a, "g", "g", g)
    _bind(a, "out", "o", out)
    keep = [g, out]
    if bn_t is not None:
        u = as_plane(u)
        gam, mean, rstd = (_vec(q, c, "gen_tail_bwd") for q in bn_t)
        _bind(a, "u", "u", u)
        a.gamma_t, a.mean_t, a.rstd_t = _ptr(gam), mean.data_ptr(), rstd.data_ptr()
        keep += [u, gam, mean, rstd]
    if r is not None:
        r = _bind(a, "r", "r", r, True)
        keep.append(r)
        if bn_r is not None:
            gam, mean, rstd = (_vec(q, c, "gen_tail_bwd") for q in bn_r)
            a.gamma_r, a.mean_r, a.rstd_r = _ptr(gam), mean.data_ptr(), rstd.data_ptr()
            keep += [gam, mean, rstd]
    if noise is not None:
        noise = noise.contiguous()
        a.noise = noise.data_ptr()
        keep.append(noise)
    _need_cuda(*keep, *sinks.values())
    for k_, t_ in sinks.items():
        if t_ is not None and (t_.numel() != c or not t_.is_contiguous()):
            raise ValueError("gen_tail_bwd: sink %s must be a contiguous (C,) tensor" % k_)
    a.dgamma_t, a.dbeta_t = _ptr(sinks.get("gamma_t")), _ptr(sinks.get("beta_t"))
    a.dgamma_r, a.dbeta_r, a.dnw = _ptr(sinks.get("gamma_r")), _ptr(sinks.get("beta_r")), _ptr(sinks.get("nw"))
    have_coef = coef is not None
    if have_coef:
        if tuple(coef.shape) != (6, c) or not coef.is_contiguous():
            raise ValueError("gen_tail_bwd: coef must be a contiguous (6, C) tensor")
        _need_cuda(coef)
    else:
        coef = torch.empty((6, c), dtype=torch.float32, device=g.device)
    a.coef = coef.data_ptr()
    if not have_coef:
        if c > SYNC_LEN:
            raise ValueError("gen_tail_bwd: %d channels exceed the %d ticket counters" % (c, SYNC_LEN))
        ws = _workspace("kg_gen_tail_workspace_bytes", a, g.device, tickets="counters")
        _check(lib.kg_gen_tail_stats(C.byref(a), _stream()), "kg_gen_tail_stats")
    if stats_only:
        return coef
    du = _bind(a, "du", "du", new_plane(n, c, t, v, g.device))
    dr = None
    if r is not None:
        dr = du if bn_t is None and bn_r is None else _bind(a, "dr", "dr", new_plane(n, c, t, v, g.device))
    _check(lib.kg_gen_tail_apply(C.byref(a), _stream()), "kg_gen_tail_apply")
    return du, dr


def gen_adj_finish(jobs: Sequence[dict]):
    lib = load_library()
    for chunk in _chunks(jobs, GEN_ADJ_MAX_JOBS):
        arr = (_GenAdjJob * len(chunk))()
        for q, j in enumerate(chunk):
            dbt, out = j["dbt"], j["out"]
            _need_cuda(dbt, j.get("u"), j.get("a"), out)
            assert dbt.is_contiguous() and out.is_contiguous() and dbt.dim() == 3 and out.dim() == 3
            k, v, _ = out.shape
            kd, v2, vc = dbt.shape
            assert v2 == v and kd <= k, (dbt.shape, out.shape)
            e = arr[q]
            e.dbt, e.u, e.a, e.out = dbt.data_ptr(), _ptr(j.get("u")), _ptr(j.get("a")), out.data_ptr()
            e.K, e.Kd, e.V, e.Vc, e.accumulate = k, kd, v, vc, int(bool(j.get("accumulate", False)))
        _check(lib.kg_gen_adj_finish(arr, len(chunk), _stream()), "kg_gen_adj_finish")



def _plane(t: Optional[torch.Tensor]) -> _Plane:
    p = _Plane()
    if t is not None:
        if not is_plane(t) or t.dtype != torch.float32:
            raise ValueError("genblock: plane tensor expected, got %s / strides %s" % (tuple(t.shape), t.stride()))
        p.p = t.data_ptr()
        p.sN, p.sC = _sn_sc(t)
    return p


class GenBlockDims(NamedTuple):
    Cin: int
    C: int
    K: int
    Kp: int
    Tc: int
    Vc: int
    T: int
    V: int
    rep: int
    res_kind: int
    bn_t: bool
    act: int


def _gb_common(a, d: GenBlockDims, slope):
    a.Cin, a.C, a.K, a.Kp, a.Tc, a.Vc, a.T, a.V, a.rep = d.Cin, d.C, d.K, d.Kp, d.Tc, d.Vc, d.T, d.V, d.rep
    a.res_kind, a.bn_t, a.act, a.slope = d.res_kind, int(d.bn_t), d.act, slope


def _gb_weights(a, wg, wr, wt, B, U):
    for t in (wg, wr, wt, B, U):
        if t is not None and (not t.is_contiguous() or t.dtype != torch.float32):
            raise ValueError("genblock: weights / adjacency must be contiguous fp32")
    a.wg, a.wr, a.wt, a.b, a.u = wg.data_ptr(), _ptr(wr), wt.data_ptr(), B.data_ptr(), _ptr(U)


def genblock_supported(d: GenBlockDims, n: int, wg, wr, wt, backward: bool = False) -> bool:
    lib = load_library()
    if backward:
        a = _GenBlockBwdArgs()
        a.N = n
        _gb_common(a, d, 0.2)
        return lib.kg_genblock_bwd_lds_bytes(C.byref(a)) >= 0
    a = _GenBlockArgs()
    a.N, a.groups = n, 1
    _gb_common(a, d, 0.2)
    a.wg, a.wr, a.wt = wg.data_ptr(), _ptr(wr), wt.data_ptr()
    return lib.kg_genblock_lds_bytes(C.byref(a)) >= 0


def _gb_bn(layer: _GenBnLayer, bn: dict, c: int, groups: int, device):
    vecs = [_vec(bn.get(k), c, "genblock_fwd") for k in ("gamma", "beta", "running_mean", "running_var")]
    nbt = bn.get("num_batches_tracked")
    _need_cuda(*vecs, nbt)
    layer.gamma, layer.beta, layer.running_mean, layer.running_var = [_ptr(q) for q in vecs]
    if nbt is not None:
        assert nbt.dtype == torch.int64
        layer.num_batches_tracked = nbt.data_ptr()
    layer.momentum, layer.eps = float(bn["momentum"]), float(bn["eps"])
    coef = torch.empty((groups, 4, c), dtype=torch.float32, device=device)
    layer.coef = coef.data_ptr()
    return coef


def genblock_fwd(d: GenBlockDims, *, x=None, pend=None, wg, wr=None, br=None, wt, bt=None, B, U=None, bn_t=None, bn_r=None,
                 groups: int = 1, noise=None, nw=None, slope: float = 0.2) -> dict:
    lib = load_library()
    a = _GenBlockArgs()
    _gb_common(a, d, slope)
    if (bn_t is not None) != bool(d.bn_t) or (bn_r is not None) != (d.res_kind == 2):
        raise ValueError("genblock_fwd: BatchNorm layers do not match the block's geometry")
    keep = []
    if x is not None:
        x = as_plane(x)
        n = x.shape[0]
        a.x = _plane(x)
        dev = x.device
        if tuple(x.shape[1:]) != (d.Cin, d.Tc, d.Vc):
            raise ValueError("genblock_fwd: input %s does not match (%d, %d, %d)" % (tuple(x.shape), d.Cin, d.Tc, d.Vc))
    else:
        pu = as_plane(pend["u"])
        n, dev = pu.shape[0], pu.device
        if tuple(pu.shape[1:]) != (d.Cin, d.Tc, d.Vc):
            raise ValueError("genblock_fwd: pending tail %s does not match (%d, %d, %d)" % (tuple(pu.shape), d.Cin, d.Tc, d.Vc))
        a.pu = _plane(pu)
        pr = pend.get("r")
        if pr is not None:
            pr = as_plane(pr)
            a.pr = _plane(pr)
        for key, fld in (("ct", "pcoef_t"), ("cr", "pcoef_r")):
            cf = pend.get(key)
            if cf is not None:
                if tuple(cf.shape) != (groups, 4, d.Cin) or not cf.is_contiguous():
                    raise ValueError("genblock_fwd: pending %s must be a contiguous (groups, 4, Cin) tensor" % key)
                setattr(a, fld, cf.data_ptr())
        pn, pw = pend.get("noise"), pend.get("nw")
        if pn is not None and pw is not None:
            pn, pw = pn.contiguous(), pw.reshape(-1).contiguous()
            a.pnoise, a.pnw = pn.data_ptr(), pw.data_ptr()
        a.pact = int(pend["act"])
        x = new_plane(n, d.Cin, d.Tc, d.Vc, dev)
        a.xout = _plane(x)
        keep += [pu, pr, pn, pw, pend.get("ct"), pend.get("cr")]
        _need_cuda(*keep)
    a.N, a.groups = n, groups
    _gb_weights(a, wg, wr, wt, B, U)
    a.br, a.bt = _ptr(br), _ptr(bt)
    _need_cuda(x, wg, wr, br, wt, bt, B, U, noise, nw)
    Mh = d.Kp * d.C + (d.C if d.res_kind == 2 else 0)
    yc = new_plane(n, Mh, d.Tc, d.Vc, dev)
    z = new_plane(n, d.C, d.T, d.V, dev)
    u = new_plane(n, d.C, d.T, d.V, dev)
    r = new_plane(n, d.C, d.T, d.V, dev) if d.res_kind != 0 else None
    a.yc, a.z, a.uo, a.r = _plane(yc), _plane(z), _plane(u), _plane(r)
    ct = _gb_bn(a.bt_, bn_t, d.C, groups, dev) if bn_t is not None else None
    cr = _gb_bn(a.br_, bn_r, d.C, groups, dev) if bn_r is not None else None
    out = None
    if ct is None and cr is None:
        out = new_plane(n, d.C, d.T, d.V, dev)
        a.out = _plane(out)
        if noise is not None and nw is not None:
            noise, nw = noise.contiguous(), nw.reshape(-1).contiguous()
            a.noise, a.nw = noise.data_ptr(), nw.data_ptr()
    else:
        ws = _workspace("kg_genblock_workspace_bytes", a, dev, tickets="counters")
    _count("kg_genblock", 2.0 * n * (Mh * d.Cin * d.Tc * d.Vc + 3 * d.C * d.C * d.T * d.V) +
           2.0 * n * (d.Kp + (1 if d.res_kind else 0)) * d.Vc * d.V * d.C * d.Tc)
    _check(lib.kg_genblock_fwd(C.byref(a), _stream()), "kg_genblock_fwd")
    return dict(x=x, yc=yc, z=z, r=r, u=u, ct=ct, cr=cr, out=out)


def genblock_bwd(d: GenBlockDims, *, g, out, u=None, r=None, coef, wg, wr=None, wt, B, U=None, prev=None, slope: float = 0.2) -> dict:
    lib = load_library()
    a = _GenBlockBwdArgs()
    _gb_common(a, d, slope)
    g, out = as_plane(g), as_plane(out)
    n, dev = g.shape[0], g.device
    a.N = n
    a.g, a.out = _plane(g), _plane(out)
    keep = [g, out, coef]
    if d.bn_t:
        u = as_plane(u)
        a.uo = _plane(u)
        keep.append(u)
    if d.res_kind == 2:
        r = as_plane(r)
        a.r = _plane(r)
        keep.append(r)
    if tuple(coef.shape) != (6, d.C) or not coef.is_contiguous():
        raise ValueError("genblock_bwd: coef must be a contiguous (6, C) tensor")
    a.coef = coef.data_ptr()
    _gb_weights(a, wg, wr, wt, B, U)
    _need_cuda(*keep, wg, wr, wt, B, U)
    Mh = d.Kp * d.C + (d.C if d.res_kind == 2 else 0)
    du = new_plane(n, d.C, d.T, d.V, dev)
    dr = None
    if d.res_kind == 2 or (d.res_kind == 1 and d.bn_t):
        dr = new_plane(n, d.C, d.T, d.V, dev)
    gyc = new_plane(n, Mh, d.Tc, d.Vc, dev)
    zf = new_plane(n, d.C, d.Tc, d.V, dev)
    gx = new_plane(n, d.Cin, d.Tc, d.Vc, dev)
    a.du, a.dr, a.gyc, a.zf, a.gx = _plane(du), _plane(dr), _plane(gyc), _plane(zf), _plane(gx)
    pcoef = None
    if prev is not None:
        px = as_plane(prev["x"])
        a.px = _plane(px)
        a.pact = int(prev["act"])
        sinks = prev.get("sinks") or {}
        keep2 = [px]
        if prev.get("bn_t") is not None:
            pu = as_plane(prev["u"])
            gam, mean, rstd = (_vec(q, d.Cin, "genblock_bwd") for q in prev["bn_t"])
            a.pu = _plane(pu)
            a.pgamma_t, a.pmean_t, a.prstd_t = _ptr(gam), mean.data_ptr(), rstd.data_ptr()
            keep2 += [pu, gam, mean, rstd]
        if prev.get("bn_r") is not None:
            pr = as_plane(prev["r"])
            gam, mean, rstd = (_vec(q, d.Cin, "genblock_bwd") for q in prev["bn_r"])
            a.pr = _plane(pr)
            a.pgamma_r, a.pmean_r, a.prstd_r = _ptr(gam), mean.data_ptr(), rstd.data_ptr()
            keep2 += [pr, gam, mean, rstd]
        pn = prev.get("noise")
        if pn is not None:
            pn = pn.contiguous()
            a.pnoise = pn.data_ptr()
            keep2.append(pn)
        for k_, t_ in sinks.items():
            if t_ is not None and (t_.numel() != d.Cin or not t_.is_contiguous()):
                raise ValueError("genblock_bwd: sink %s must be a contiguous (Cin,) tensor" % k_)
        _need_cuda(*keep2, *sinks.values())
        a.dgamma_t, a.dbeta_t = _ptr(sinks.get("gamma_t")), _ptr(sinks.get("beta_t"))
        a.dgamma_r, a.dbeta_r, a.dnw = _ptr(sinks.get("gamma_r")), _ptr(sinks.get("beta_r")), _ptr(sinks.get("nw"))
        pcoef = torch.empty((6, d.Cin), dtype=torch.float32, device=dev)
        a.pcoef = pcoef.data_ptr()
        ws = _workspace("kg_genblock_bwd_workspace_bytes", a, dev, tickets="counters")
    _count("kg_genblock", 2.0 * n * (Mh * d.Cin * d.Tc * d.Vc + 3 * d.C * d.C * d.T * d.V) +
           2.0 * n * (d.Kp + (1 if d.res_kind else 0)) * d.Vc * d.V * d.C * d.T)
    _check(lib.kg_genblock_bwd(C.byref(a), _stream()), "kg_genblock_bwd")
    if dr is None and d.res_kind != 0:
        dr = du
    return dict(du=du, dr=dr, gyc=gyc, zf=zf, gx=gx, pcoef=pcoef)


def _rowsum_fill(a, x, y, want_second: int, out, out2, accumulate: int):
    n, c, t, v = x.shape
    a.N, a.C, a.T, a.V = n, c, t, v
    _bind(a, "x", "x", x)
    if y is not None:
        if y.shape[1] == 1 and c > 1:
            y = y.contiguous()
            a.y, a.y_sN, a.y_sC = y.data_ptr(), t * v, 0
        else:
            y = _bind(a, "y", "y", y, True)
    a.want_second = want_second
    a.out, a.out2, a.accumulate = out.data_ptr(), _ptr(out2), accumulate
    return x, y


def rowsum(x: torch.Tensor, y: Optional[torch.Tensor] = None, second: bool = False,
           shift: Optional[torch.Tensor] = None, out: Optional[torch.Tensor] = None,
           accumulate: bool = False, out2: Optional[torch.Tensor] = None) -> torch.Tensor:
    lib = load_library()
    x = as_plane(x)
    _need_cuda(x, y, shift)
    c = x.shape[1]
    a = _RowsumArgs()
    if shift is not None:
        shift = shift.reshape(-1).contiguous()
        a.shift = shift.data_ptr()
    rows = 2 if int(second) == 1 else 1
    if out is None:
        if accumulate:
            raise ValueError("rowsum: accumulate needs out")
        out = torch.empty((rows, c), dtype=torch.float32, device=x.device)
    else:
        _need_cuda(_dest(out, rows * c, "rowsum: out must be a contiguous fp32 tensor of %d elements" % (rows * c)))
    if out2 is not None:
        _need_cuda(_dest(out2, rows * c, "rowsum: out2 must be a contiguous fp32 tensor of %d elements" % (rows * c)))
    held = _rowsum_fill(a, x, y, int(second), out, out2, int(accumulate))
    ws = _workspace("kg_rowsum_workspace_bytes", a, x.device)
    _check(lib.kg_rowsum(C.byref(a), _stream()), "kg_rowsum")
    return out


def rowsum_many(jobs: Sequence[dict]):
    lib = load_library()
    if not jobs:
        return
    arr = (_RowsumArgs * len(jobs))()
    held = []
    for i, j in enumerate(jobs):
        x = as_plane(j["x"])
        out, out2, y = j["out"], j.get("out2"), j.get("y")
        _need_cuda(x, out, out2)
        for o in (out, out2):
            if o is not None:
                _dest(o, x.shape[1], "rowsum_many: destinations must be contiguous fp32 vectors of C elements")
        _need_cuda(y)
        held.append(_rowsum_fill(arr[i], x, y, 0 if y is None else 2, out, out2, int(bool(j.get("accumulate", False)))))
    ws = _workspace("kg_rowsum_many_workspace_bytes", arr, jobs[0]["x"].device, len(jobs))
    _check(lib.kg_rowsum_many(arr, len(jobs), ws.data_ptr(), ws.numel() * 4, _stream()), "kg_rowsum_many")


def _elt_args(x, out, act, slope):
    a = _EltArgs()
    a.N, a.C, a.T, a.V = x.shape
    _bind(a, "x", "x", x)
    _bind(a, "out", "o", out)
    a.act, a.slope = act, slope
    return a


def act_bwd(g: torch.Tensor, ref: torch.Tensor, act: int, slope: float = 0.2) -> torch.Tensor:
    lib = load_library()
    g = as_plane(g)
    ref = as_plane(ref)
    _need_cuda(g, ref)
    out = new_plane(*g.shape, g.device)
    a = _elt_args(g, out, act, slope)
    _bind(a, "r", "r", ref)
    _check(lib.kg_act_bwd(C.byref(a), _stream()), "kg_act_bwd")
    return out


def affine_act(x, sx=None, bx=None, r=None, sr=None, br=None, noise=None, nw=None,
               act: int = ACT_NONE, slope: float = 0.2, out: Optional[torch.Tensor] = None,
               groups: int = 1, coef_gs: int = 0) -> torch.Tensor:
    lib = load_library()
    x = as_plane(x)
    vecs = [None if t is None else t.reshape(-1).contiguous() for t in (sx, bx, sr, br, nw)]
    _need_cuda(x, r, noise, out, *vecs)
    if out is None:
        out = new_plane(*x.shape, x.device)
    elif tuple(out.shape) != tuple(x.shape) or not is_plane(out) or out.dtype != torch.float32:
        raise ValueError("affine_act: out must be a plane tensor of x's shape")
    a = _elt_args(x, out, act, slope)
    if r is not None:
        r = _bind(a, "r", "r", r, True)
    if noise is not None:
        noise = noise.contiguous()
        a.noise = noise.data_ptr()
    a.sx, a.bx, a.sr, a.br, a.nw = [_ptr(t) for t in vecs]
    a.groups, a.coef_gs = int(groups), int(coef_gs)
    _check(lib.kg_affine_act(C.byref(a), _stream()), "kg_affine_act")
    return out


def _gp_args(g):
    a = _GpArgs()
    a.N, a.C, a.T, a.V = g.shape
    _bind(a, "g", "g", g)
    return a


def gp_fwd(g: torch.Tensor):
    lib = load_library()
    g = as_plane(g)
    _need_cuda(g)
    a = _gp_args(g)
    nrm = torch.empty(g.shape[0], dtype=torch.float32, device=g.device)
    gp = torch.empty((), dtype=torch.float32, device=g.device)
    a.nrm, a.gp = nrm.data_ptr(), gp.data_ptr()
    _check(lib.kg_gp_fwd(C.byref(a), _stream()), "kg_gp_fwd")
    return nrm, gp


def gp_bwd(g: torch.Tensor, nrm: torch.Tensor, gout: torch.Tensor) -> torch.Tensor:
    lib = load_library()
    g = as_plane(g)
    gout = gout.reshape(1).contiguous()
    _need_cuda(g, nrm, gout)
    a = _gp_args(g)
    a.nrm, a.gout = nrm.data_ptr(), gout.data_ptr()
    out = _bind(a, "out", "o", new_plane(*g.shape, g.device))
    _check(lib.kg_gp_bwd(C.byref(a), _stream()), "kg_gp_bwd")
    return out


def _vec(t: Optional[torch.Tensor], c: int, what: str):
    return None if t is None else _dest(t, c, f"{what}: expected a contiguous fp32 vector of {c} elements")


def _bn_fwd_fill(a, who: str, x, gamma, beta, running_mean, running_var, nbt, momentum, eps, training, groups: Optional[int] = None):
    n, c, t, v = x.shape
    vecs = [_vec(q, c, who) for q in (gamma, beta, running_mean, running_var)]
    _need_cuda(x, *vecs, nbt)
    a.N, a.C, a.T, a.V = n // (groups or 1), c, t, v
    _bind(a, "x", "x", x)
    a.gamma, a.beta, a.running_mean, a.running_var = [_ptr(q) for q in vecs]
    if nbt is not None:
        assert nbt.dtype == torch.int64
        a.num_batches_tracked = nbt.data_ptr()
    a.momentum, a.eps, a.training = float(momentum), float(eps), int(bool(training))
    coef = torch.empty((4, c) if groups is None else (groups, 4, c), dtype=torch.float32, device=x.device)
    a.coef = coef.data_ptr()
    return coef


def bn_fwd(x: torch.Tensor, gamma, beta, running_mean, running_var, num_batches_tracked, training: bool,
           momentum: float, eps: float) -> torch.Tensor:
    lib = load_library()
    x = as_plane(x)
    a = _BnArgs()
    coef = _bn_fwd_fill(a, "bn_fwd", x, gamma, beta, running_mean, running_var, num_batches_tracked, momentum, eps, training)
    _check(lib.kg_bn_fwd(C.byref(a), _stream()), "kg_bn_fwd")
    return coef


def _bn_many(who: str, arr, coefs):
    total_c = sum(cf.shape[-1] for cf in coefs)
    if total_c > SYNC_LEN:
        raise ValueError("%s: %d channels exceed the %d ticket counters" % (who, total_c, SYNC_LEN))
    ws = _workspace("kg_%s_workspace_bytes" % who, arr, coefs[0].device if coefs else None, len(arr))
    sync = _sync_buffer(coefs[0].device)
    _check(getattr(load_library(), "kg_" + who)(arr, len(arr), ws.data_ptr(), ws.numel() * 4, sync.data_ptr(), sync.numel(),
                                               _stream()), "kg_" + who)
    return coefs


def bn_fwd_many(jobs: Sequence[dict]):
    arr = (_BnJob * len(jobs))()
    xs, coefs = [], []
    for i, j in enumerate(jobs):
        x = as_plane(j["x"])
        groups = int(j.get("groups", 1))
        if x.shape[0] % groups:
            raise ValueError("bn_fwd_many: N=%d is not a multiple of groups=%d" % (x.shape[0], groups))
        coefs.append(_bn_fwd_fill(arr[i].a, "bn_fwd_many", x, j.get("gamma"), j.get("beta"), j.get("running_mean"),
                                  j.get("running_var"), j.get("num_batches_tracked"), j["momentum"], j["eps"], True, groups))
        arr[i].groups = groups
        xs.append(x)
    return _bn_many("bn_fwd_many", arr, coefs)


def _bn_bwd_fill(a, who: str, g, x, gamma, mean, rstd, training):
    g, x = as_plane(g), as_plane(x)
    n, c, t, v = x.shape
    gamma, mean, rstd = _vec(gamma, c, who), _vec(mean, c, who), _vec(rstd, c, who)
    _need_cuda(g, x, gamma, mean, rstd)
    a.N, a.C, a.T, a.V = n, c, t, v
    _bind(a, "x", "x", x)
    _bind(a, "g", "g", g)
    a.gamma, a.mean, a.rstd = _ptr(gamma), _ptr(mean), _ptr(rstd)
    a.training = int(bool(training))
    coef = torch.empty((5, c), dtype=torch.float32, device=x.device)
    a.coef = coef.data_ptr()
    return coef, (g, x)


def bn_bwd(g: torch.Tensor, x: torch.Tensor, gamma, mean: torch.Tensor, rstd: torch.Tensor, training: bool) -> torch.Tensor:
    lib = load_library()
    a = _BnArgs()
    coef, held = _bn_bwd_fill(a, "bn_bwd", g, x, gamma, mean, rstd, training)
    _check(lib.kg_bn_bwd(C.byref(a), _stream()), "kg_bn_bwd")
    return coef


def bn_bwd_many(jobs: Sequence[dict]):
    arr = (_BnArgs * len(jobs))()
    filled = [_bn_bwd_fill(arr[i], "bn_bwd_many", j["g"], j["x"], j.get("gamma"), j["mean"], j["rstd"], j["training"])
              for i, j in enumerate(jobs)]
    return _bn_many("bn_bwd_many", arr, [coef for coef, _ in filled])


def adam_step(p, g, m, v, lr, b1, b2, eps, step_t: torch.Tensor, grad_scale: float = 1.0, zero_grad: bool = False):
    lib = load_library()
    _need_cuda(p, g, m, v, step_t)
    assert p.is_contiguous() and g.is_contiguous() and m.is_contiguous() and v.is_contiguous()
    assert step_t.dtype == torch.int32
    if zero_grad:
        _check(lib.kg_adam_step_fused(p.data_ptr(), g.data_ptr(), m.data_ptr(), v.data_ptr(), p.numel(), lr, b1, b2, eps,
                                      step_t.data_ptr(), grad_scale, 1, _stream()), "kg_adam_step_fused")
        return
    _check(lib.kg_adam_step(p.data_ptr(), g.data_ptr(), m.data_ptr(), v.data_ptr(), p.numel(),
                            lr, b1, b2, eps, step_t.data_ptr(), grad_scale, _stream()), "kg_adam_step")


def adam_step_ema(p, g, m, v, e, lr, b1, b2, eps, step_t: torch.Tensor, grad_scale: float, zero_grad: bool, decay: float,
                  warmup: float):
    lib = load_library()
    _need_cuda(p, g, m, v, e, step_t)
    assert p.is_contiguous() and g.is_contiguous() and m.is_contiguous() and v.is_contiguous() and e.is_contiguous()
    assert g.numel() == m.numel() == v.numel() == e.numel() == p.numel() and e.dtype == torch.float32
    assert step_t.dtype == torch.int32
    _check(lib.kg_adam_step_ema(p.data_ptr(), g.data_ptr(), m.data_ptr(), v.data_ptr(), e.data_ptr(), p.numel(), lr, b1, b2, eps,
                                step_t.data_ptr(), grad_scale, 1 if zero_grad else 0, decay, warmup, _stream()),
           "kg_adam_step_ema")



def _head_args(h, w=None, gv=None):
    a = _HeadArgs()
    h = _bind(a, "h", "h", h, True)
    a.N, a.C, a.T, a.V = h.shape
    if w is not None:
        w = w.reshape(-1)
        assert w.is_contiguous() and w.numel() == h.shape[1]
        a.w = w.data_ptr()
    if gv is not None:
        assert gv.numel() == h.shape[0]
        a.gv = gv.data_ptr()
    return a, h


def head_fwd(h: torch.Tensor, w: torch.Tensor, b: Optional[torch.Tensor]) -> torch.Tensor:
    lib = load_library()
    _need_cuda(h, w, b)
    a, h = _head_args(h, w)
    a.b = _ptr(b)
    v = torch.empty(h.shape[0], dtype=torch.float32, device=h.device)
    a.v = v.data_ptr()
    _check(lib.kg_head_fwd(C.byref(a), _stream()), "kg_head_fwd")
    return v


def head_bwd(gv: torch.Tensor, w: torch.Tensor, h: torch.Tensor, masked: bool = True, slope: float = 0.2) -> torch.Tensor:
    lib = load_library()
    gv = gv.reshape(-1).contiguous()
    _need_cuda(gv, w, h)
    a, h = _head_args(h, w, gv)
    a.masked, a.slope = int(bool(masked)), slope
    g = _bind(a, "g", "g", new_plane(*h.shape, h.device))
    _check(lib.kg_head_bwd(C.byref(a), _stream()), "kg_head_bwd")
    return g


def head_wgrad(x: torch.Tensor, gv: torch.Tensor, dw: torch.Tensor, db: Optional[torch.Tensor], accumulate: bool = True):
    lib = load_library()
    gv = gv.reshape(-1).contiguous()
    _need_cuda(x, gv, dw, db)
    a, x = _head_args(x, None, gv)
    assert dw.is_contiguous() and dw.numel() == x.shape[1] and (db is None or db.numel() == 1)
    a.dw, a.db, a.accumulate = dw.data_ptr(), _ptr(db), int(bool(accumulate))
    _check(lib.kg_head_wgrad(C.byref(a), _stream()), "kg_head_wgrad")



def _cls_head_args(n: int, c: int, t: int, v: int, f: int, l: int, slope: float = 0.2) -> _ClsHeadArgs:
    a = _ClsHeadArgs()
    a.N, a.C, a.T, a.V, a.F, a.L, a.slope = int(n), int(c), int(t), int(v), int(f), int(l), float(slope)
    return a


def _cls_flat(t: torch.Tensor, n: int, dtype, what: str) -> torch.Tensor:
    if t.numel() != n or not t.is_contiguous() or t.dtype != dtype:
        raise ValueError(f"kg_cls_head: {what} must be contiguous {dtype} of {n} elements")
# ... 1291 lines not shown
```

kinetic-gan_amd/build.py:

```python
from __future__ import annotations

import os
import subprocess
import sys

PKG = os.path.dirname(os.path.abspath(__file__))
ROOT = os.path.dirname(PKG)
CSRC = os.path.join(PKG, "csrc")
LIB = os.path.join(PKG, "libkgan_hip.so")
SOURCES = ["kg_conv.hip", "kg_wgrad.hip", "kg_agg.hip", "kg_aggconv.hip", "kg_gen.hip", "kg_genblock.hip", "kg_disc.hip", "kg_map.hip", "kg_comm.hip", "kg_misc.hip", "kg_mmd.hip", "kg_input.hip", "kg_sample.hip", "kg_eval.hip", "kg_prdc.hip", "kg_frechet.hip", "kg_cls.hip", "kg_nn.hip", "kg_nn_gram.hip", "kg_kin.hip"]


def _stale() -> bool:
    if not os.path.exists(LIB):
        return True
    t = os.path.getmtime(LIB)
    deps = [os.path.join(CSRC, f) for f in os.listdir(CSRC)] + [os.path.join(ROOT, "include", "kgan_hip.h")]
    return any(os.path.getmtime(d) > t for d in deps)


LIB_ASAN = os.path.join(PKG, "libkgan_hip_asan.so")
RING_SOURCE = os.path.join(ROOT, "tools", "probe", "kg_conv_ring.hip")


def _with_ring() -> bool:
    return os.environ.get("KG_WITH_RING", "0") == "1" or "--with-ring" in sys.argv


def build_asan() -> str:
    hipcc = os.environ.get("HIPCC", "/opt/rocm/bin/hipcc")
    cmd = [hipcc, "--offload-arch=gfx950", "-O1", "-g", "-fno-omit-frame-pointer", "-fsanitize=address", "-shared-libsan",
           "-Wno-option-ignored", "-std=c++17", "-fPIC", "-shared", "-mllvm", "-amdgpu-mfma-vgpr-form",
           "-I", os.path.join(ROOT, "include"), "-I", CSRC, "-o", LIB_ASAN] + [os.path.join(CSRC, s) for s in SOURCES] + ["-ldl"]
    r = subprocess.run(cmd, capture_output=True, text=True)
    if r.returncode != 0:
        raise RuntimeError("hipcc (asan) failed:\n" + r.stdout + r.stderr)
    return LIB_ASAN


last_action = None


def build(force: bool = False, verbose: bool = False) -> str:
    global last_action
    if not force and not _stale():
        last_action = "reused"
        return LIB
    last_action = "compiled"
    hipcc = os.environ.get("HIPCC", "/opt/rocm/bin/hipcc")
    cmd = [hipcc, "--offload-arch=gfx950", "-O3", "-std=c++17", "-fPIC", "-shared",
           "-mllvm", "-amdgpu-mfma-vgpr-form",
           "-I", os.path.join(ROOT, "include"), "-I", CSRC,
           "-o", LIB] + [os.path.join(CSRC, s) for s in SOURCES] + ["-ldl"]
    if _with_ring():
        cmd += ["-DKG_WITH_RING", RING_SOURCE]
    if verbose:
        cmd.insert(1, "-Rpass-analysis=kernel-resource-usage")
    r = subprocess.run(cmd, capture_output=True, text=True)
    if r.returncode != 0:
        raise RuntimeError("hipcc failed:\n" + r.stdout + r.stderr)
    if verbose:
        sys.stderr.write(r.stderr)
    return LIB


if __name__ == "__main__":
    if "--asan" in sys.argv:
        print(build_asan())
    else:
        print(build(force="--force" in sys.argv, verbose="-v" in sys.argv))
```

kinetic-gan_amd/csrc/kg_map.hip:

```cpp
#include "kg_common.h"

namespace {

constexpr int NTM = 1024;
constexpr int NWV = 16;
constexpr int NJB = 6;
constexpr int NJA = 5;
constexpr unsigned OOB = 0x80000000u;
typedef float kg_f32x4 __attribute__((ext_vector_type(4)));
typedef float kg_f32x2 __attribute__((ext_vector_type(2)));

__device__ __forceinline__ __amdgpu_buffer_rsrc_t rsrc_of(const void* p, long bytes) {
    return __builtin_amdgcn_make_buffer_rsrc(kg_uniform_ptr(p), 0, p ? (int)(bytes > 0x7fffffffL ? 0x7fffffffL : bytes) : 0, 0x00020000);
}
__device__ __forceinline__ float load1(__amdgpu_buffer_rsrc_t r, unsigned off) {
    return __builtin_bit_cast(float, __builtin_amdgcn_raw_buffer_load_b32(r, off, 0, 0));
}

template <int VW>
__device__ __forceinline__ void load_vec(__amdgpu_buffer_rsrc_t r, unsigned off, float (&v)[VW]) {
    if constexpr (VW == 4) {
        const kg_f32x4 t = __builtin_bit_cast(kg_f32x4, __builtin_amdgcn_raw_buffer_load_b128(r, off, 0, 0));
        v[0] = t[0]; v[1] = t[1]; v[2] = t[2]; v[3] = t[3];
    } else if constexpr (VW == 2) {
        const kg_f32x2 t = __builtin_bit_cast(kg_f32x2, __builtin_amdgcn_raw_buffer_load_b64(r, off, 0, 0));
        v[0] = t[0]; v[1] = t[1];
    } else {
        v[0] = load1(r, off);
    }
}
template <int VW>
__device__ __forceinline__ void mask_tail(float (&v)[VW], int k, int len) {
    if (k + VW > len) {
#pragma unroll
        for (int t = 0; t < VW; ++t)
            if (k + t >= len) v[t] = 0.f;
    }
}

__device__ __forceinline__ float reduce_rows(const kg_f32x16& acc, float* red, int wave, int lane) {
#pragma unroll
    for (int r = 0; r < 16; ++r) red[(wave * 16 + r) * 64 + lane] = acc[r];
    __syncthreads();
    float v = 0.f;
#pragma unroll
    for (int w = 0; w < NWV; ++w) v += red[(w * 16 + wave) * 64 + lane];
    return v;
}
__device__ __forceinline__ int row_of_reg(int r, int h) { return (r & 3) + 8 * (r >> 2) + 4 * h; }

template <int VW>
__device__ __forceinline__ void load_xin(const KgLinearArgs& a, __amdgpu_buffer_rsrc_t rx, __amdgpu_buffer_rsrc_t re, int n, long lab, int k,
                                         bool ok, float (&v)[VW]) {
    const bool in_emb = k < a.J;
    const unsigned off_x = (unsigned)((long)n * a.x_ld + (k - a.J)) * 4u;
    const unsigned off_e = (unsigned)(lab * a.J + k) * 4u;
    load_vec<VW>(in_emb ? re : rx, (ok && k < a.Din) ? (in_emb ? off_e : off_x) : OOB, v);
    mask_tail<VW>(v, k, a.Din);
}

template <int VW>
__global__ __launch_bounds__(NTM) void kg_linear_fwd_kernel(const KgLinearArgs a) {
    __shared__ float red[NWV * 16 * 64];
    const int tid = threadIdx.x, lane = tid & 63, wave = tid >> 6;
    const int l32 = lane & 31, h = lane >> 5;
    const int o0 = blockIdx.x * 32, n0 = blockIdx.y * 32;
    const __amdgpu_buffer_rsrc_t rx = rsrc_of(a.x, (long)a.N * a.x_ld * 4), re = rsrc_of(a.emb, (long)a.L * a.J * 4);
    const __amdgpu_buffer_rsrc_t rw = rsrc_of(a.w, (long)a.Dout * a.Din * 4), rb = rsrc_of(a.bias, (long)a.Dout * 4);
    const int n = n0 + l32, o = o0 + l32;
    const bool n_ok = n < a.N, o_ok = o < a.Dout;
    const float bias = load1(rb, o_ok ? (unsigned)o * 4u : OOB);
    long lab = 0;
    if (a.J > 0 && n_ok) {
        lab = a.labels[n];
        if (lab < 0 || lab >= a.L) lab = -1;
    }
    kg_f32x16 acc;
#pragma unroll
    for (int r = 0; r < 16; ++r) acc[r] = 0.f;
    constexpr int CH = 2 * VW;
    const int nch = (a.Din + CH - 1) / CH;
    for (int c0 = wave; c0 < nch; c0 += NWV * NJB) {
        float av[NJB][VW], bv[NJB][VW];
#pragma unroll
        for (int j = 0; j < NJB; ++j) {
            const int c = c0 + NWV * j;
            const int k = c * CH + VW * h;
            const bool live = c < nch;
            load_xin<VW>(a, rx, re, n, lab < 0 ? 0 : lab, k, live && n_ok, av[j]);
            load_vec<VW>(rw, (live && o_ok && k < a.Din) ? (unsigned)((long)o * a.Din + k) * 4u : OOB, bv[j]);
            mask_tail<VW>(bv[j], k, a.Din);
            if (lab < 0 && k < a.J) {
#pragma unroll
                for (int t = 0; t < VW; ++t) av[j][t] = __builtin_nanf("");
            }
        }
#pragma unroll
        for (int j = 0; j < NJB; ++j)
#pragma unroll
            for (int t = 0; t < VW; ++t) acc = __builtin_amdgcn_mfma_f32_32x32x2f32(av[j][t], bv[j][t], acc, 0, 0, 0);
    }
    const float v = reduce_rows(acc, red, wave, lane);
    const int nn = n0 + row_of_reg(wave, h);
    if (o_ok && nn < a.N) a.y[(long)nn * a.y_ld + o] = kg_act(v + bias, a.act, a.slope);
}

template <int VW>
__global__ __launch_bounds__(NTM) void kg_linear_bwd_kernel(const KgLinearArgs a, int nwg_a, int itiles_a, int igroups_b) {
    __shared__ float red[NWV * 16 * 64];
    const int tid = threadIdx.x, lane = tid & 63, wave = tid >> 6;
    const int l32 = lane & 31, h = lane >> 5;
    const __amdgpu_buffer_rsrc_t rg = rsrc_of(a.g, (long)a.N * a.g_ld * 4), ry = rsrc_of(a.y, (long)a.N * a.y_ld * 4);
    kg_f32x16 acc;
#pragma unroll
    for (int r = 0; r < 16; ++r) acc[r] = 0.f;
    const float slope = a.slope;
    const bool lrelu = a.act == KG_ACT_LRELU;
    auto dact = [&](float gv, float yv) { return (lrelu && !(yv > 0.f)) ? gv * slope : gv; };
    if ((int)blockIdx.x < nwg_a) {
        const int it = blockIdx.x % itiles_a, nt = blockIdx.x / itiles_a;
        const int n0 = nt * 32, i0 = it * 32;
        const __amdgpu_buffer_rsrc_t rw = rsrc_of(a.w, (long)a.Dout * a.Din * 4);
        const int n = n0 + l32, i = i0 + l32;
        const bool n_ok = n < a.N, i_ok = i < a.gx_cols;
        constexpr int CH = 2 * VW;
        const int nch = (a.Dout + CH - 1) / CH;
        for (int c0 = wave; c0 < nch; c0 += NWV * NJA) {
            float gv[NJA][VW], yv[NJA][VW], bv[NJA][VW];
#pragma unroll
            for (int j = 0; j < NJA; ++j) {
                const int c = c0 + NWV * j;
                const int k = c * CH + VW * h;
                const bool live = c < nch && k < a.Dout;
                load_vec<VW>(rg, (live && n_ok) ? (unsigned)((long)n * a.g_ld + k) * 4u : OOB, gv[j]);
                load_vec<VW>(ry, (live && n_ok) ? (unsigned)((long)n * a.y_ld + k) * 4u : OOB, yv[j]);
#pragma unroll
                for (int t = 0; t < VW; ++t)
                    bv[j][t] = load1(rw, (live && i_ok && k + t < a.Dout) ? (unsigned)((long)(k + t) * a.Din + i) * 4u : OOB);
            }
#pragma unroll
            for (int j = 0; j < NJA; ++j) {
                const int k = (c0 + NWV * j) * CH + VW * h;
#pragma unroll
                for (int t = 0; t < VW; ++t) {
                    const float av = k + t < a.Dout ? dact(gv[j][t], yv[j][t]) : 0.f;
                    acc = __builtin_amdgcn_mfma_f32_32x32x2f32(av, bv[j][t], acc, 0, 0, 0);
                }
            }
        }
        const float v = reduce_rows(acc, red, wave, lane);
        const int nn = n0 + row_of_reg(wave, h);
        if (i_ok && nn < a.N) a.gx[(long)nn * a.gx_ld + i] = v;
        return;
    }
    const int wg = (int)blockIdx.x - nwg_a;
    const int ot = wg / igroups_b, ig = wg - ot * igroups_b;
    const int itl = wave & 3, kg = wave >> 2;
    const int o0 = ot * 32, i0 = (ig * 4 + itl) * 32;
    const __amdgpu_buffer_rsrc_t rx = rsrc_of(a.x, (long)a.N * a.x_ld * 4), re = rsrc_of(a.emb, (long)a.L * a.J * 4);
    const int o = o0 + l32, i = i0 + l32;
    const bool o_ok = o < a.Dout, i_ok = i < a.Din;
    const bool from_emb = i < a.J;
    float bsum = 0.f;
    const int npairs = (a.N + 1) / 2;
    for (int s0 = kg; s0 < npairs; s0 += 4 * NJB) {
        float gv[NJB], yv[NJB], xv[NJB];
        long lab[NJB];
        if (from_emb) {
#pragma unroll
            for (int j = 0; j < NJB; ++j) {
                const int n = 2 * (s0 + 4 * j) + h;
                lab[j] = n < a.N ? (long)a.labels[n] : -1;
            }
        }
#pragma unroll
        for (int j = 0; j < NJB; ++j) {
            const int n = 2 * (s0 + 4 * j) + h;
            const bool n_ok = n < a.N;
            gv[j] = load1(rg, (n_ok && o_ok) ? (unsigned)((long)n * a.g_ld + o) * 4u : OOB);
            yv[j] = load1(ry, (n_ok && o_ok) ? (unsigned)((long)n * a.y_ld + o) * 4u : OOB);
            if (from_emb) xv[j] = load1(re, (n_ok && lab[j] >= 0 && lab[j] < a.L) ? (unsigned)(lab[j] * a.J + i) * 4u : OOB);
            else          xv[j] = load1(rx, (n_ok && i_ok) ? (unsigned)((long)n * a.x_ld + (i - a.J)) * 4u : OOB);
        }
#pragma unroll
        for (int j = 0; j < NJB; ++j) {
            const float av = dact(gv[j], yv[j]);
            bsum += av;
            acc = __builtin_amdgcn_mfma_f32_32x32x2f32(av, xv[j], acc, 0, 0, 0);
        }
    }
#pragma unroll
    for (int r = 0; r < 16; ++r) red[(wave * 16 + r) * 64 + lane] = acc[r];
    __syncthreads();
    if (a.dw && i_ok) {
#pragma unroll
        for (int q = 0; q < 4; ++q) {
            const int r = 4 * kg + q;
            float v = 0.f;
#pragma unroll
            for (int k2 = 0; k2 < 4; ++k2) v += red[((k2 * 4 + itl) * 16 + r) * 64 + lane];
            const int oo = o0 + row_of_reg(r, h);
            if (oo < a.Dout) {
                float* p = a.dw + (long)oo * a.Din + i;
                *p = (a.accumulate ? *p : 0.f) + v;
            }
        }
    }
    if (a.db == nullptr || ig != 0) return;
    __syncthreads();
    bsum += __shfl_xor(bsum, 32, 64);
    if (itl == 0 && h == 0) red[kg * 32 + l32] = bsum;
    __syncthreads();
    if (wave == 0 && h == 0 && o_ok) {
        const float t = (red[l32] + red[32 + l32]) + (red[64 + l32] + red[96 + l32]);
        a.db[o] = (a.accumulate ? a.db[o] : 0.f) + t;
    }
}

__global__ __launch_bounds__(256) void kg_embed_bwd_kernel(const KgLinearArgs a) {
    __shared__ int lab_s[256];
    const int e = blockIdx.x * 256 + threadIdx.x;
    const bool ok = e < a.L * a.J;
    const int l = ok ? e / a.J : 0, j = ok ? e - l * a.J : 0;
    float s = 0.f;
    for (int n0 = 0; n0 < a.N; n0 += 256) {
        const int nb = a.N - n0 < 256 ? a.N - n0 : 256;
        __syncthreads();
        if ((int)threadIdx.x < nb) lab_s[threadIdx.x] = (int)a.labels[n0 + threadIdx.x];
        __syncthreads();
        for (int q0 = 0; q0 < nb; q0 += 16) {
            float v[16];
#pragma unroll
            for (int q = 0; q < 16; ++q) v[q] = (q0 + q < nb) ? a.gx[(long)(n0 + q0 + q) * a.gx_ld + j] : 0.f;
#pragma unroll
            for (int q = 0; q < 16; ++q) s += (q0 + q < nb && lab_s[q0 + q] == l) ? v[q] : 0.f;
        }
    }
    if (ok) a.demb[e] = (a.accumulate ? a.demb[e] : 0.f) + s;
}

int validate(const KgLinearArgs* a, const char* what) {
    KG_REQUIRE(a != nullptr, "%s: null args", what);
    KG_REQUIRE(a->N > 0 && a->Din > 0 && a->Dout > 0, "%s: bad dims N=%d Din=%d Dout=%d", what, a->N, a->Din, a->Dout);
    KG_REQUIRE(a->J >= 0 && a->J <= a->Din, "%s: J=%d outside [0, Din=%d]", what, a->J, a->Din);
    KG_REQUIRE(a->J == 0 || (a->emb != nullptr && a->labels != nullptr && a->L > 0), "%s: embedding columns without table / labels", what);
    KG_REQUIRE(a->J == a->Din || a->x != nullptr, "%s: null x", what);
    KG_REQUIRE(a->x_ld >= a->Din - a->J, "%s: x_ld=%ld < %d", what, (long)a->x_ld, a->Din - a->J);
    KG_REQUIRE(a->act == KG_ACT_NONE || a->act == KG_ACT_LRELU, "%s: act=%d (none or LeakyReLU)", what, a->act);
    KG_REQUIRE((long)a->N * (a->x_ld > a->Dout ? a->x_ld : a->Dout) < (1L << 28) && (long)a->Dout * a->Din < (1L << 28),
               "%s: operand too large for 32-bit offsets", what);
    KG_REQUIRE(a->y_ld >= 0 && a->g_ld >= 0 && a->gx_ld >= 0 && (long)a->N * a->y_ld < (1L << 28) && (long)a->N * a->g_ld < (1L << 28) &&
               (long)a->N * a->gx_ld < (1L << 28) && (long)a->L * a->J < (1L << 28),
               "%s: y / g / gx / embedding table too large for 32-bit offsets", what);
    return 0;
}

int vec_width(long ld_a, long ld_b, long ld_c) {
    auto ok = [&](int v) { return ld_a % v == 0 && ld_b % v == 0 && ld_c % v == 0; };
    if (ok(4)) return 4;
    if (ok(2)) return 2;
    return 1;
}

}

extern "C" int kg_linear_fwd(const KgLinearArgs* a, void* stream) {
    if (int rc = validate(a, "kg_linear_fwd")) return rc;
    KG_REQUIRE(a->w != nullptr && a->y != nullptr, "kg_linear_fwd: null w / y");
    KG_REQUIRE(a->y_ld >= a->Dout, "kg_linear_fwd: y_ld=%ld < Dout=%d", (long)a->y_ld, a->Dout);
    const bool al16 = ((uintptr_t)a->x % 16 == 0) && ((uintptr_t)a->w % 16 == 0) && (a->J == 0 || (uintptr_t)a->emb % 16 == 0);
    const int vw = al16 ? vec_width(a->x_ld, a->Din, a->J) : 1;
    dim3 grid(kg_cdiv(a->Dout, 32), kg_cdiv(a->N, 32));
    hipStream_t s = (hipStream_t)stream;
    if (vw == 4)      hipLaunchKernelGGL(kg_linear_fwd_kernel<4>, grid, dim3(NTM), 0, s, *a);
    else if (vw == 2) hipLaunchKernelGGL(kg_linear_fwd_kernel<2>, grid, dim3(NTM), 0, s, *a);
    else              hipLaunchKernelGGL(kg_linear_fwd_kernel<1>, grid, dim3(NTM), 0, s, *a);
    return kg_launch_status("kg_linear_fwd");
}

extern "C" int kg_linear_bwd(const KgLinearArgs* a, void* stream) {
    if (int rc = validate(a, "kg_linear_bwd")) return rc;
    KG_REQUIRE(a->g != nullptr && a->y != nullptr && a->w != nullptr, "kg_linear_bwd: null g / y / w");
    KG_REQUIRE(a->g_ld >= a->Dout && a->y_ld >= a->Dout, "kg_linear_bwd: g_ld / y_ld < Dout");
    KG_REQUIRE(a->gx_cols >= 0 && a->gx_cols <= a->Din, "kg_linear_bwd: gx_cols=%d", a->gx_cols);
    KG_REQUIRE(a->gx_cols == 0 || (a->gx != nullptr && a->gx_ld >= a->gx_cols), "kg_linear_bwd: gx / gx_ld");
    KG_REQUIRE(a->dw != nullptr || a->db != nullptr || a->gx_cols > 0, "kg_linear_bwd: nothing to compute");
    const bool al16 = ((uintptr_t)a->g % 16 == 0) && ((uintptr_t)a->y % 16 == 0);
    const int vw = al16 ? vec_width(a->g_ld, a->y_ld, 0) : 1;
    const int itiles_a = kg_cdiv(a->gx_cols, 32);
    const int nwg_a = itiles_a * kg_cdiv(a->N, 32);
    const int igroups_b = kg_cdiv(kg_cdiv(a->Din, 32), 4);
    const int nwg_b = (a->dw || a->db) ? kg_cdiv(a->Dout, 32) * igroups_b : 0;
    hipStream_t s = (hipStream_t)stream;
    dim3 grid(nwg_a + nwg_b);
    if (vw == 4)      hipLaunchKernelGGL(kg_linear_bwd_kernel<4>, grid, dim3(NTM), 0, s, *a, nwg_a, itiles_a > 0 ? itiles_a : 1, igroups_b);
    else if (vw == 2) hipLaunchKernelGGL(kg_linear_bwd_kernel<2>, grid, dim3(NTM), 0, s, *a, nwg_a, itiles_a > 0 ? itiles_a : 1, igroups_b);
    else              hipLaunchKernelGGL(kg_linear_bwd_kernel<1>, grid, dim3(NTM), 0, s, *a, nwg_a, itiles_a > 0 ? itiles_a : 1, igroups_b);
    return kg_launch_status("kg_linear_bwd");
}

extern "C" int kg_embed_bwd(const KgLinearArgs* a, void* stream) {
    KG_REQUIRE(a != nullptr, "kg_embed_bwd: null args");
    KG_REQUIRE(a->N > 0 && a->L > 0 && a->J > 0, "kg_embed_bwd: bad dims N=%d L=%d J=%d", a->N, a->L, a->J);
    KG_REQUIRE(a->gx != nullptr && a->labels != nullptr && a->demb != nullptr && a->gx_ld >= a->J, "kg_embed_bwd: null pointer / gx_ld");
    hipLaunchKernelGGL(kg_embed_bwd_kernel, dim3(kg_cdiv((long)a->L * a->J, 256)), dim3(256), 0, (hipStream_t)stream, *a);
    return kg_launch_status("kg_embed_bwd");
}
```

kinetic-gan_amd/gen_trunk.py:

```python
from __future__ import annotations

import os
from typing import List, Optional

import numpy as np
import torch
from torch.autograd import Function

from . import _native as nv
from . import ops
from ._native import ACT_LRELU, ACT_TANH, TAP_TIME, Group, WView

SLOPE = 0.2
FUSED = os.environ.get("KG_GEN_FUSED", "1") != "0"
FUSED_MIN_COLS = int(os.environ.get("KG_GEN_FUSED_MINCOLS", "16"))


class GenBlockGeom:

    def __init__(self, blk, Tc: int, Vc: int, device):
        self.cin, self.cout, self.K = blk.in_channels, blk.out_channels, blk.gcn.kernel_size
        self.res = blk.res_kind
        self.bn_t = len(blk.tcn) > 1
        self.act = ACT_TANH if blk.tan else ACT_LRELU
        self.Tc, self.Vc = Tc, Vc
        self.T = blk.up_t
        self.ok = self.T >= Tc and self.T % Tc == 0 and self.K <= 3
        self.rep = self.T // Tc if self.ok else 1
        if blk.up_s:
            self.U = torch.as_tensor(blk.graph.upsample_matrix(blk.lvl), dtype=torch.float32, device=device).contiguous()
            self.V = self.U.shape[1]
            self.ok = self.ok and self.U.shape[0] == Vc
        else:
            self.U, self.V = None, Vc
        a_lvl = np.asarray(blk.graph.As[blk.lvl])
        self.ok = self.ok and a_lvl.shape[1] == self.V
        self.Kp = 1 if bool(getattr(blk.gcn, "single_partition", False)) and self.V == 1 else self.K
        C = self.cout
        self.Mg = self.Kp * C
        self.Mh = self.Mg + (C if self.res == "conv" else 0)
        self.dims = nv.GenBlockDims(Cin=self.cin, C=C, K=self.K, Kp=self.Kp, Tc=Tc, Vc=Vc, T=self.T, V=self.V, rep=self.rep,
                                    res_kind={"none": 0, "identity": 1, "conv": 2}[self.res], bn_t=self.bn_t, act=self.act)
        self.A_fixed = torch.as_tensor(a_lvl, dtype=torch.float32, device=device).contiguous()
        self.spec_g = ops.ConvSpec(M=self.Mg, Cin=self.cin, taps=1, tap_mode=TAP_TIME, t_stride=1, T_in=Tc, V_in=Vc,
                                   T_out=Tc, V_out=Vc, wv=WView(sT=0, sO=self.cin, sI=1), w_shape=(self.Mg * self.cin,))
        self.spec_r = ops.ConvSpec(M=C, Cin=self.cin, taps=1, tap_mode=TAP_TIME, t_stride=1, T_in=Tc, V_in=Vc,
                                   T_out=Tc, V_out=Vc, wv=WView(sT=0, sO=self.cin, sI=1), w_shape=(C * self.cin,))
        if self.T == 1:
            self.spec_t = ops.ConvSpec(M=C, Cin=C, taps=1, tap_mode=TAP_TIME, t_stride=1, T_in=1, V_in=self.V, T_out=1,
                                       V_out=self.V, wv=WView(sT=0, sO=3 * C, sI=3), w_shape=(3 * C * C - 1,))
        else:
            self.spec_t = ops.ConvSpec(M=C, Cin=C, taps=3, tap_mode=TAP_TIME, t_stride=1, T_in=self.T, V_in=self.V,
                                       T_out=self.T, V_out=self.V, wv=WView(sT=1, sO=3 * C, sI=3), w_shape=(3 * C * C,))


class GenTrunkMeta:
    def __init__(self, G, device):
        self.geoms: List[GenBlockGeom] = []
        t, v = 1, G.graph.num_node[G.st_gcn_networks[0].lvl]
        self.ok = True
        for blk in G.st_gcn_networks:
            g = GenBlockGeom(blk, t, v, device)
            self.ok = self.ok and g.ok
            self.geoms.append(g)
            t, v = g.T, g.V
        self.nb = len(self.geoms)
        self.poff, off = [], 0
        for g in self.geoms:
            self.poff.append(off)
            off += 4 + (2 if g.bn_t else 0) + (4 if g.res == "conv" else 0)
        self.nparams = off
        self.adj_off, off = [], 0
        for g in self.geoms:
            na, nb_ = g.K * g.V * g.V, g.K * g.Vc * g.V
            self.adj_off.append((off, off + na))
            off += na + nb_
        self.adj_numel = off

    def block_params(self, params, i):
        g = self.geoms[i]
        p = params[self.poff[i]:]
        d = dict(wg=p[0], wt=p[1], bt=p[2], nw=p[3], gam_t=None, bet_t=None, wr=None, br=None, gam_r=None, bet_r=None)
        q = 4
        if g.bn_t:
            d["gam_t"], d["bet_t"] = p[q], p[q + 1]
            q += 2
        if g.res == "conv":
            d["wr"], d["br"], d["gam_r"], d["bet_r"] = p[q:q + 4]
        return d


def collect_params(G):
    params, bns = [], []
    for blk in G.st_gcn_networks:
        params += [blk.gcn.conv.weight, blk.tcn[0].weight, blk.tcn[0].bias, blk.noise.weight]
        bn_t = blk.tcn[1] if len(blk.tcn) > 1 else None
        bn_r = blk.residual[1] if blk.res_kind == "conv" else None
        if bn_t is not None:
            params += [bn_t.weight, bn_t.bias]
        if bn_r is not None:
            params += [blk.residual[0].weight, blk.residual[0].bias, bn_r.weight, bn_r.bias]
        bns.append((bn_t, bn_r))
    return params, bns


def trunk_supported(G, bns) -> bool:
    for bn_t, bn_r in bns:
        for b in (bn_t, bn_r):
            if b is not None and (b.running_mean is None or b.momentum is None or not b.affine):
                return False
    return True


def _rowblock_delta(wg: torch.Tensor, wr: torch.Tensor) -> Optional[int]:
    if not (wg.is_contiguous() and wr.is_contiguous()):
        return None
    if wg.untyped_storage().data_ptr() != wr.untyped_storage().data_ptr():
        return None
    d = wr.storage_offset() - wg.storage_offset()
    return d if 0 < d < (1 << 27) else None


def _head_conv(g: GenBlockGeom, x, wg, wr):
    n = x.shape[0]
    if g.res != "conv":
        return nv.conv([Group(x, wg, WView(0, g.cin, 1), g.cin, 1)], n, g.Mg, g.Tc, g.Vc)
    delta = _rowblock_delta(wg, wr)
    if delta is not None:
        return nv.conv([Group(x, wg, WView(0, g.cin, 1, delta, g.Mg), g.cin, 1)], n, g.Mh, g.Tc, g.Vc)
    yc = nv.new_plane(n, g.Mh, g.Tc, g.Vc, x.device)
    nv.conv([Group(x, wg, WView(0, g.cin, 1), g.cin, 1)], n, g.Mg, g.Tc, g.Vc, out=yc[:, :g.Mg])
    nv.conv([Group(x, wr, WView(0, g.cin, 1), g.cin, 1)], n, g.cout, g.Tc, g.Vc, out=yc[:, g.Mg:])
    return yc


def _tcn_weight(g: GenBlockGeom, wt):
    return wt.reshape(-1)[1:] if g.T == 1 else wt


def _bn_job(bn, gamma, beta):
    return dict(gamma=gamma, beta=beta, running_mean=bn.running_mean, running_var=bn.running_var,
                num_batches_tracked=bn.num_batches_tracked, momentum=bn.momentum, eps=bn.eps)


def _finish_tail(pend, groups: int):
    ct, cr, C = pend["ct"], pend["cr"], pend["u"].shape[1]
    return nv.affine_act(pend["u"], ct[0, 0] if ct is not None else None, ct[0, 1] if ct is not None else None, pend["r"],
                         cr[0, 0] if cr is not None else None, cr[0, 1] if cr is not None else None,
                         pend["noise"], pend["nw"].reshape(-1), pend["act"], SLOPE,
                         groups=groups if (ct is not None or cr is not None) else 1, coef_gs=4 * C)


def _fusable(g: GenBlockGeom, n: int, p, backward: bool = False) -> bool:
    return (FUSED and g.T > 1 and g.Tc * g.Vc >= FUSED_MIN_COLS and
            nv.genblock_supported(g.dims, n, p["wg"], p["wr"] if g.res == "conv" else None, p["wt"], backward=backward))


def fwd_pass(meta: GenTrunkMeta, w, noise, adjs, params, bns, groups: int, keep: bool):
    x = w.view(w.shape[0], w.shape[1], 1, 1)
    tape = []
    pend = None
    nall = w.shape[0]
    for i, g in enumerate(meta.geoms):
        p = meta.block_params(params, i)
        bn_t, bn_r = bns[i]
        n, C = nall, g.cout
        if _fusable(g, n, p):
            res = nv.genblock_fwd(g.dims, x=x if pend is None else None, pend=pend, wg=p["wg"], wr=p["wr"], br=p["br"],
                                  wt=p["wt"], bt=p["bt"], B=adjs[i], U=g.U,
                                  bn_t=_bn_job(bn_t, p["gam_t"], p["bet_t"]) if bn_t is not None else None,
                                  bn_r=_bn_job(bn_r, p["gam_r"], p["bet_r"]) if bn_r is not None else None,
                                  groups=groups, noise=noise[i], nw=p["nw"], slope=SLOPE)
            if pend is not None and keep:
                tape[i - 1]["out"] = res["x"]
            if keep:
                tape.append(dict(x=res["x"], yc=res["yc"], z=res["z"], u=res["u"], r=res["r"], out=res["out"], ct=res["ct"], cr=res["cr"]))
            if res["out"] is not None:
                x, pend = res["out"], None
            else:
                x, pend = None, dict(u=res["u"], r=res["r"], ct=res["ct"], cr=res["cr"], noise=noise[i], nw=p["nw"], act=g.act)
            continue
        if pend is not None:
            x = _finish_tail(pend, groups)
            if keep:
                tape[i - 1]["out"] = x
            pend = None
        yc = _head_conv(g, x, p["wg"], p["wr"])
        rs = yc[:, g.Mg:] if g.res == "conv" else (x if g.res == "identity" else None)
        z, r = nv.gen_expand(yc[:, :g.Mg], None, g.U, g.rep, C, rs=rs, rbias=p["br"] if g.res == "conv" else None, B=adjs[i])
        st = g.spec_t
        u = nv.conv([Group(z, _tcn_weight(g, p["wt"]), st.wv, C, st.taps, TAP_TIME, 1, False, None)], n, C, g.T, g.V,
                    bias0=p["bt"])
        jobs = []
        if bn_t is not None:
            jobs.append(dict(_bn_job(bn_t, p["gam_t"], p["bet_t"]), x=u, groups=groups))
        if bn_r is not None:
            jobs.append(dict(_bn_job(bn_r, p["gam_r"], p["bet_r"]), x=r, groups=groups))
        coefs = nv.bn_fwd_many(jobs) if jobs else []
        ct = coefs[0] if bn_t is not None else None
        cr = coefs[-1] if bn_r is not None else None
        out = _finish_tail(dict(u=u, r=r, ct=ct, cr=cr, noise=noise[i], nw=p["nw"], act=g.act), groups)
        if keep:
            tape.append(dict(x=x, yc=yc, z=z, u=u, r=r, out=out, ct=ct, cr=cr))
        x = out
    if pend is not None:
        x = _finish_tail(pend, groups)
        if keep:
            tape[-1]["out"] = x
    return x, tape


def _tail_operands(geo: GenBlockGeom, tp, p, sl, noise_i):
    ct, cr = tp["ct"], tp["cr"]
    sinks = dict(nw=ops._sink_of(p["nw"]))
    bn_t = bn_r = None
    if ct is not None:
        bn_t = (p["gam_t"], ct[-1, 2], ct[-1, 3])
        sinks.update(gamma_t=ops._sink_of(p["gam_t"]), beta_t=ops._sink_of(p["bet_t"]))
    if cr is not None:
        bn_r = (p["gam_r"], cr[-1, 2], cr[-1, 3])
        sinks.update(gamma_r=ops._sink_of(p["gam_r"]), beta_r=ops._sink_of(p["bet_r"]))
    r = tp["r"][sl] if tp["r"] is not None else None
    return dict(u=tp["u"][sl] if ct is not None else None, bn_t=bn_t, r=r, bn_r=bn_r, noise=noise_i[sl], sinks=sinks)


def bwd_pass(meta: GenTrunkMeta, tape, g, noise, adjs, params, lo: int, hi: int, imp_sinks, need_gx0: bool = True):
    outer_jobs, adj_jobs = [], []
    sl = slice(lo, hi)
    coef_next = None
    for i in range(meta.nb - 1, -1, -1):
        geo = meta.geoms[i]
        tp = tape[i]
        p = meta.block_params(params, i)
        C, n = geo.cout, hi - lo
        x, yc, z, out = tp["x"][sl], tp["yc"][sl], tp["z"][sl], tp["out"][sl]
        tail = _tail_operands(geo, tp, p, sl, noise[i])
        st = geo.spec_t
        wt_sink = ops._sink_of(p["wt"])
        wg_sink = ops._sink_of(p["wg"])
        if _fusable(geo, n, p, backward=True):
            coef = coef_next if coef_next is not None else nv.gen_tail_bwd(g, out, geo.act, slope=SLOPE, stats_only=True, **tail)
            prev = None
            if i > 0:
                pg = meta.geoms[i - 1]
                prev = _tail_operands(pg, tape[i - 1], meta.block_params(params, i - 1), sl, noise[i - 1])
                prev.update(x=x, act=pg.act)
            res = nv.genblock_bwd(geo.dims, g=g, out=out, u=tail["u"], r=tail["r"] if tail["bn_r"] is not None else None, coef=coef,
                                  wg=p["wg"], wr=p["wr"], wt=p["wt"], B=adjs[i], U=geo.U, prev=prev, slope=SLOPE)
            coef_next = res["pcoef"]
            du, dr, gyc, zf = res["du"], res["dr"], res["gyc"], res["zf"]
            ops._wgrad_into(wt_sink, z, du, st)
            ops._rowsum_into([ops._sink_of(p["bt"])], du)
            ops._wgrad_into(wg_sink[:geo.Mg * geo.cin], x, gyc[:, :geo.Mg], geo.spec_g)
            if geo.res == "conv":
                ops._wgrad_into(ops._sink_of(p["wr"]), x, gyc[:, geo.Mg:], geo.spec_r)
                ops._rowsum_into([ops._sink_of(p["br"])], dr)
            dbt = nv.agg_outer(zf, yc[:, :geo.Mg], geo.Kp, 1, defer=outer_jobs)
            adj_jobs.append(dict(dbt=dbt, u=geo.U, a=geo.A_fixed, out=imp_sinks[i].view(geo.K, geo.V, geo.V), accumulate=True))
            g = res["gx"]
            continue
        du, dr = nv.gen_tail_bwd(g, out, geo.act, slope=SLOPE, coef=coef_next, **tail)
        coef_next = None
        ops._wgrad_into(wt_sink[1:] if geo.T == 1 else wt_sink, z, du, st)
        ops._rowsum_into([ops._sink_of(p["bt"])], du)
        gz = nv.conv([Group(du, _tcn_weight(geo, p["wt"]), WView(st.wv.sT, st.wv.sI, st.wv.sO), C, st.taps, TAP_TIME, 1, True, None)],
                     n, C, geo.T, geo.V)
        gyc = nv.new_plane(n, geo.Mh, geo.Tc, geo.Vc, g.device)
        b_i = adjs[i]
        if geo.res == "conv":
            _, _, zf = nv.gen_fold(gz, None, geo.U, geo.rep, geo.Kp, gr=dr, want_zf=True, y_out=gyc[:, :geo.Mg], rs_out=gyc[:, geo.Mg:], B=b_i)
            gid = None
        elif geo.res == "identity":
            _, gid, zf = nv.gen_fold(gz, None, geo.U, geo.rep, geo.Kp, gr=dr, want_zf=True, y_out=gyc, B=b_i)
        else:
            _, _, zf = nv.gen_fold(gz, None, geo.U, geo.rep, geo.Kp, want_zf=True, y_out=gyc, B=b_i)
            gid = None
        ops._wgrad_into(wg_sink[:geo.Mg * geo.cin], x, gyc[:, :geo.Mg], geo.spec_g)
        if geo.res == "conv":
            ops._wgrad_into(ops._sink_of(p["wr"]), x, gyc[:, geo.Mg:], geo.spec_r)
            ops._rowsum_into([ops._sink_of(p["br"])], dr)
        dbt = nv.agg_outer(zf, yc[:, :geo.Mg], geo.Kp, 1, defer=outer_jobs)
        adj_jobs.append(dict(dbt=dbt, u=geo.U, a=geo.A_fixed, out=imp_sinks[i].view(geo.K, geo.V, geo.V), accumulate=True))
        if i == 0 and not need_gx0:
            g = None
            break
        grp = [Group(gyc[:, :geo.Mg], p["wg"], WView(0, 1, geo.cin), geo.Mg, 1)]
        if geo.res == "conv":
            grp.append(Group(gyc[:, geo.Mg:], p["wr"], WView(0, 1, geo.cin), C, 1))
        out0 = None
        if i == 0 and geo.Tc == 1 and geo.Vc == 1:
            out0 = torch.empty((n, geo.cin, 1, 1), dtype=torch.float32, device=gyc.device)
        g = nv.conv(grp, n, geo.cin, geo.Tc, geo.Vc, add=gid, out=out0)
    nv.agg_outer_finish(outer_jobs)
    nv.gen_adj_finish(adj_jobs)
    return None if g is None else g.reshape(g.shape[0], -1)


class GenTrunkFn(Function):

    @staticmethod
    def forward(ctx, cfg, w_all, w_b, *rest):
        meta, bns, groups = cfg
        nb = meta.nb
        noise, imps, params = list(rest[:nb]), list(rest[nb:2 * nb]), list(rest[2 * nb:])
        ctx.set_materialize_grads(False)
        need = any(ctx.needs_input_grad[1:])
        with torch.no_grad():
            pack = torch.empty(meta.adj_numel, dtype=torch.float32, device=w_all.device)
            adjs, jobs = [], []
            for g, imp, (oa, ob) in zip(meta.geoms, imps, meta.adj_off):
                k, v, vc = g.K, g.V, g.Vc
                ae = pack[oa:oa + k * v * v].view(k, v, v)
                b = pack[ob:ob + k * vc * v].view(k, vc, v)
                jobs.append(dict(a=g.A_fixed, imp=imp.detach(), u=g.U, aeff=ae, b=b))
                adjs.append(b[:g.Kp])
            nv.gen_adj_prepare(jobs)
            out, tape = fwd_pass(meta, w_all.detach(), [t.detach() for t in noise], adjs, [p.detach() for p in params], bns,
                                 groups, keep=need)
        ctx.meta, ctx.tape, ctx.adjs, ctx.noise = meta, tape, adjs, noise
        ctx.n_all = w_all.shape[0]
        ctx.n_b = w_b.shape[0] if w_b is not None else ctx.n_all
        ctx.paired = w_b is not None
        ctx.imp_sinks = [ops._sink_of(p) for p in imps]
        ctx.save_for_backward(*params)
        if w_b is None:
            return out
        ctx.mark_non_differentiable(out)
        return out, out[ctx.n_all - ctx.n_b:]

    @staticmethod
    @torch.autograd.function.once_differentiable
    def backward(ctx, *gs):
        meta = ctx.meta
        nret = 3 + 2 * meta.nb + meta.nparams
        g = gs[-1]
        if g is None:
            return (None,) * nret
        params = list(ctx.saved_tensors)
        lo = ctx.n_all - ctx.n_b
        need_w = ctx.needs_input_grad[2] if ctx.paired else ctx.needs_input_grad[1]
        with torch.no_grad():
            gw = bwd_pass(meta, ctx.tape, nv.as_plane(g), [t.detach() for t in ctx.noise], ctx.adjs, params, lo, ctx.n_all,
                          ctx.imp_sinks, need_gx0=need_w)
        ctx.tape = None
        if ctx.paired:
            return (None, None, gw) + (None,) * (nret - 3)
        return (None, gw, None) + (None,) * (nret - 3)


def all_sinks_registered(G) -> bool:
    return all(ops._sink_of(p) is not None for p in G.parameters() if p.requires_grad)
```

Baseline: 20670 samples/s.

## Add dense MFMA kernels for V=1 generator blocks in forward and backward

Adds a new gendense HIP kernel pair that handles the early generator blocks, where the spatial extent is one joint and one time step, as dense matrix products on MFMA, with optional fused BN, noise and activation epilogues. The generator trunk routes eligible blocks through these kernels instead of the general genblock path. In backward it also fuses the previous block's tail gradient into the head stage. Shared tile helpers move from kg_map into a common header. The forward route with BN or a residual conv is off by default behind an env flag, so only the no-BN forward blocks and the backward blocks use the new path. This adds code complexity and a separate numeric path for those blocks.

```diff
diff --git a/include/kgan_hip.h b/include/kgan_hip.h
--- a/include/kgan_hip.h
+++ b/include/kgan_hip.h
@@ -380,6 +380,52 @@
 int kg_linear_bwd(const KgLinearArgs* a, void* stream);
 int kg_embed_bwd(const KgLinearArgs* a, void* stream);
 
+#define KG_GD_HEAD 0
+#define KG_GD_TCN 1
+#define KG_GD_MAX_GROUPS 4
+#define KG_GD_MAX_BN_ROWS 256
+typedef struct KgGenDenseArgs {
+    int32_t N, K, C, Cr;
+    int32_t rep, groups;
+    int32_t stage;
+    int32_t x_rowmajor;
+    int32_t act;  float slope;
+    const float* x;  int64_t x_ld;
+    const float* w;  const float* w2;
+    const float* a;
+    const float* bias;
+    float* yc;  int64_t yc_sC;
+    float* z;  int64_t z_sC;
+    float* r;  int64_t r_sC;
+    float* u;  int64_t u_sC;
+    float* out;  int64_t out_sC;
+    const float* noise;  const float* nw;
+    const float* coef_r;
+    const float* gamma;  const float* beta;
+    float* running_mean;  float* running_var;  int64_t* num_batches_tracked;
+    float momentum, eps;
+    float* coef;
+} KgGenDenseArgs;
+int kg_gendense_fwd(const KgGenDenseArgs* a, void* stream);
+int kg_gendense_check(const KgGenDenseArgs* a);
+
+typedef struct KgGenDenseBwdArgs {
+    int32_t N, K, C, Cr;
+    int32_t rep, stage;
+    int32_t gx_rowmajor;  int32_t act;  float slope;
+    const float* w;  const float* w2;
+    const float* a;
+    const float* du;  int64_t du_sC;
+    const float* dr;  int64_t dr_sC;
+    float* zf;  int64_t zf_sC;
+    float* gyc;  int64_t gyc_sC;
+    float* gx;  int64_t gx_ld;
+    const float* out;  int64_t out_sC;
+    const float* noise;  float* dnw;
+} KgGenDenseBwdArgs;
+int kg_gendense_bwd(const KgGenDenseBwdArgs* a, void* stream);
+int kg_gendense_bwd_check(const KgGenDenseBwdArgs* a);
+
 #define KG_COMM_ID_BYTES 128
 int kg_comm_unique_id(void* id);
 int kg_comm_init(void** comm, int32_t rank, int32_t world, const void* id, int32_t device);
diff --git a/kinetic-gan_amd/_native.py b/kinetic-gan_amd/_native.py
--- a/kinetic-gan_amd/_native.py
+++ b/kinetic-gan_amd/_native.py
@@ -193,6 +193,28 @@
                 ("g", c_f32p), ("g_ld", C.c_int64),
                 ("gx", c_f32p), ("gx_ld", C.c_int64), ("gx_cols", C.c_int32),
                 ("dw", c_f32p), ("db", c_f32p), ("demb", c_f32p), ("accumulate", C.c_int32)]
+
+
+class _GenDenseArgs(C.Structure):
+    _fields_ = [("N", C.c_int32), ("K", C.c_int32), ("C", C.c_int32), ("Cr", C.c_int32),
+                ("rep", C.c_int32), ("groups", C.c_int32), ("stage", C.c_int32), ("x_rowmajor", C.c_int32),
+                ("act", C.c_int32), ("slope", C.c_float),
+                ("x", c_f32p), ("x_ld", C.c_int64), ("w", c_f32p), ("w2", c_f32p), ("a", c_f32p), ("bias", c_f32p),
+                ("yc", c_f32p), ("yc_sC", C.c_int64), ("z", c_f32p), ("z_sC", C.c_int64), ("r", c_f32p), ("r_sC", C.c_int64),
+                ("u", c_f32p), ("u_sC", C.c_int64), ("out", c_f32p), ("out_sC", C.c_int64),
+                ("noise", c_f32p), ("nw", c_f32p), ("coef_r", c_f32p),
+                ("gamma", c_f32p), ("beta", c_f32p), ("running_mean", c_f32p), ("running_var", c_f32p),
+                ("num_batches_tracked", C.c_void_p), ("momentum", C.c_float), ("eps", C.c_float), ("coef", c_f32p)]
+
+
+class _GenDenseBwdArgs(C.Structure):
+    _fields_ = [("N", C.c_int32), ("K", C.c_int32), ("C", C.c_int32), ("Cr", C.c_int32),
+                ("rep", C.c_int32), ("stage", C.c_int32), ("gx_rowmajor", C.c_int32), ("act", C.c_int32), ("slope", C.c_float),
+                ("w", c_f32p), ("w2", c_f32p), ("a", c_f32p),
+                ("du", c_f32p), ("du_sC", C.c_int64), ("dr", c_f32p), ("dr_sC", C.c_int64),
+                ("zf", c_f32p), ("zf_sC", C.c_int64), ("gyc", c_f32p), ("gyc_sC", C.c_int64),
+                ("gx", c_f32p), ("gx_ld", C.c_int64), ("out", c_f32p), ("out_sC", C.c_int64),
+                ("noise", c_f32p), ("dnw", c_f32p)]
 
 
 class _LabelBiasArgs(C.Structure):
@@ -594,6 +616,10 @@
     "kg_linear_fwd": (C.c_int, [C.POINTER(_LinearArgs), C.c_void_p]),
     "kg_linear_bwd": (C.c_int, [C.POINTER(_LinearArgs), C.c_void_p]),
     "kg_embed_bwd": (C.c_int, [C.POINTER(_LinearArgs), C.c_void_p]),
+    "kg_gendense_fwd": (C.c_int, [C.POINTER(_GenDenseArgs), C.c_void_p]),
+    "kg_gendense_check": (C.c_int, [C.POINTER(_GenDenseArgs)]),
+    "kg_gendense_bwd": (C.c_int, [C.POINTER(_GenDenseBwdArgs), C.c_void_p]),
+    "kg_gendense_bwd_check": (C.c_int, [C.POINTER(_GenDenseBwdArgs)]),
     "kg_label_bias_fwd": (C.c_int, [C.POINTER(_LabelBiasArgs), C.c_void_p]),
     "kg_label_bias_workspace_bytes": (C.c_int64, [C.POINTER(_LabelBiasArgs)]),
     "kg_label_bias_bwd": (C.c_int, [C.POINTER(_LabelBiasArgs), C.c_void_p]),
@@ -1604,6 +1630,154 @@
     return dict(du=du, dr=dr, gyc=gyc, zf=zf, gx=gx, pcoef=pcoef)
 
 
+
+GD_HEAD, GD_TCN = 0, 1
+GD_MAX_GROUPS, GD_MAX_BN_ROWS = 4, 256
+
+
+def _gd_plane(t: torch.Tensor, what: str):
+    n, c, tt, v = t.shape
+    sn, sc = _sn_sc(t)
+    if t.dtype != torch.float32 or not is_plane(t) or sn != tt * v or (c > 1 and sc < n * tt * v):
+        raise ValueError("gendense: %s is not a channel-major plane" % what)
+    return t.data_ptr(), sc
+
+
+def gendense_geometry_ok(d: GenBlockDims, n: int, groups: int = 1, backward: bool = False, tail: bool = False) -> bool:
+    if not (d.V == 1 and d.Vc == 1 and d.Tc == 1 and d.Kp == 1 and d.res_kind in (0, 2)):
+        return False
+    lib = load_library()
+    res = d.res_kind == 2
+    one = 16
+    if backward:
+        b = _GenDenseBwdArgs()
+        b.N, b.K, b.C, b.Cr, b.rep, b.stage, b.act = n, d.Cin, d.C, d.C if res else 0, d.rep, GD_TCN, d.act
+        b.w = b.w2 = b.du = b.zf = b.gyc = b.gx = one
+        b.du_sC = b.dr_sC = n * d.rep
+        b.zf_sC = b.gyc_sC = b.gx_ld = b.out_sC = n
+        if res:
+            b.dr = one
+        if lib.kg_gendense_bwd_check(C.byref(b)) != 0:
+            return False
+        b.stage = GD_HEAD
+        if tail:
+            b.out = one
+        return lib.kg_gendense_bwd_check(C.byref(b)) == 0
+    a = _GenDenseArgs()
+    a.N, a.K, a.C, a.Cr, a.rep, a.groups, a.stage, a.act = n, d.Cin, d.C, d.C if res else 0, d.rep, groups, GD_HEAD, d.act
+    a.x = a.w = a.w2 = a.yc = a.z = a.r = a.u = a.out = one
+    a.x_ld = a.yc_sC = n
+    a.z_sC = a.r_sC = a.u_sC = a.out_sC = n * d.rep
+    if res:
+        a.coef = one
+    if lib.kg_gendense_check(C.byref(a)) != 0:
+        return False
+    a.stage, a.K, a.Cr, a.x_ld = GD_TCN, d.C, 0, n * d.rep
+    a.coef = one if d.bn_t else None
+    if not res:
+        a.r = None
+    return lib.kg_gendense_check(C.byref(a)) == 0
+
+
+def _gd_bn(a: _GenDenseArgs, bn: dict, c: int, groups: int, device):
+    vecs = [_vec(bn.get(k), c, "gendense_fwd") for k in ("gamma", "beta", "running_mean", "running_var")]
+    nbt = bn.get("num_batches_tracked")
+    _need_cuda(*vecs, nbt)
+    a.gamma, a.beta, a.running_mean, a.running_var = [_ptr(q) for q in vecs]
+    if nbt is not None:
+        assert nbt.dtype == torch.int64
+        a.num_batches_tracked = nbt.data_ptr()
+    a.momentum, a.eps = float(bn["momentum"]), float(bn["eps"])
+    coef = torch.empty((groups, 4, c), dtype=torch.float32, device=device)
+    a.coef = coef.data_ptr()
+    return coef
+
+
+def gendense_fwd(d: GenBlockDims, *, x, wg, wr=None, br=None, wt, bt=None, a_eff, bn_t=None, bn_r=None, groups: int = 1,
+                 noise=None, nw=None, slope: float = 0.2) -> dict:
+    lib = load_library()
+    n, dev = x.shape[0], x.device
+    res = d.res_kind == 2
+    if (bn_t is not None) != bool(d.bn_t) or (bn_r is not None) != res or x.dtype != torch.float32 or tuple(x.shape[1:]) != (d.Cin, 1, 1):
+        raise ValueError("gendense_fwd: operands do not match the block's geometry")
+    _need_cuda(x, wg, wr, br, wt, bt, a_eff, noise, nw)
+    C_, rep = d.C, d.rep
+    Mh = C_ + (C_ if res else 0)
+    a = _GenDenseArgs()
+    a.N, a.K, a.C, a.Cr, a.rep, a.groups, a.stage, a.act, a.slope = n, d.Cin, C_, Mh - C_, rep, groups, GD_HEAD, d.act, slope
+    if x.stride(1) == 1 and (n == 1 or x.stride(0) >= d.Cin):
+        a.x, a.x_ld, a.x_rowmajor = x.data_ptr(), x.stride(0) if n > 1 else d.Cin, 1
+    else:
+        a.x, a.x_ld = _gd_plane(x, "x")
+    a.w, a.w2, a.a, a.bias = wg.data_ptr(), _ptr(wr), a_eff.data_ptr(), _ptr(br) if res else None
+    yc, z = new_plane(n, Mh, 1, 1, dev), new_plane(n, C_, rep, 1, dev)
+    r = new_plane(n, C_, rep, 1, dev) if res else None
+    a.yc, a.yc_sC = _gd_plane(yc, "yc")
+    a.z, a.z_sC = _gd_plane(z, "z")
+    if res:
+        a.r, a.r_sC = _gd_plane(r, "r")
+    cr = _gd_bn(a, bn_r, C_, groups, dev) if bn_r is not None else None
+    _count("kg_gendense", 2.0 * n * Mh * d.Cin)
+    _check(lib.kg_gendense_fwd(C.byref(a), _stream()), "kg_gendense_fwd")
+    t = _GenDenseArgs()
+    t.N, t.K, t.C, t.Cr, t.rep, t.groups, t.stage, t.act, t.slope = n, C_, C_, 0, rep, groups, GD_TCN, d.act, slope
+    t.x, t.x_ld = a.z, a.z_sC
+    t.w, t.bias = wt.data_ptr(), _ptr(bt)
+    u, out = new_plane(n, C_, rep, 1, dev), new_plane(n, C_, rep, 1, dev)
+    t.u, t.u_sC = _gd_plane(u, "u")
+    t.out, t.out_sC = _gd_plane(out, "out")
+    if res:
+        t.r, t.r_sC, t.coef_r = a.r, a.r_sC, _ptr(cr)
+    if noise is not None and nw is not None:
+        noise, nw = noise.contiguous(), nw.reshape(-1).contiguous()
+        t.noise, t.nw = noise.data_ptr(), nw.data_ptr()
+    ct = _gd_bn(t, bn_t, C_, groups, dev) if bn_t is not None else None
+    _count("kg_gendense", 2.0 * n * C_ * C_ * (3 if rep > 1 else 1))
+    _check(lib.kg_gendense_fwd(C.byref(t), _stream()), "kg_gendense_fwd")
+    return dict(yc=yc, z=z, r=r, u=u, ct=ct, cr=cr, out=out)
+
+
+def gendense_bwd(d: GenBlockDims, *, du, dr=None, wg, wr=None, wt, a_eff, gx_rowmajor: bool = False, prev=None,
+                 want_gx: bool = True, slope: float = 0.2) -> dict:
+    lib = load_library()
+    n, dev = du.shape[0], du.device
+    res = d.res_kind == 2
+    C_, rep = d.C, d.rep
+    Mh = C_ + (C_ if res else 0)
+    _need_cuda(du, dr, wg, wr, wt, a_eff)
+    b = _GenDenseBwdArgs()
+    b.N, b.K, b.C, b.Cr, b.rep, b.stage, b.slope = n, d.Cin, C_, Mh - C_, rep, GD_TCN, slope
+    b.w, b.a = wt.data_ptr(), a_eff.data_ptr()
+    b.du, b.du_sC = _gd_plane(du, "du")
+    if res:
+        b.dr, b.dr_sC = _gd_plane(dr, "dr")
+    zf, gyc = new_plane(n, C_, 1, 1, dev), new_plane(n, Mh, 1, 1, dev)
+    b.zf, b.zf_sC = _gd_plane(zf, "zf")
+    b.gyc, b.gyc_sC = _gd_plane(gyc, "gyc")
+    _count("kg_gendense", 2.0 * n * C_ * C_ * (3 if rep > 1 else 1))
+    _check(lib.kg_gendense_bwd(C.byref(b), _stream()), "kg_gendense_bwd")
+    if not want_gx:
+        return dict(zf=zf, gyc=gyc, gx=None)
+    b.stage, b.w, b.w2, b.gx_rowmajor = GD_HEAD, wg.data_ptr(), _ptr(wr), int(gx_rowmajor)
+    pn = None
+    if gx_rowmajor:
+        gx = torch.empty((n, d.Cin, 1, 1), dtype=torch.float32, device=dev)
+        b.gx, b.gx_ld = gx.data_ptr(), d.Cin
+    else:
+        gx = new_plane(n, d.Cin, 1, 1, dev)
+        b.gx, b.gx_ld = _gd_plane(gx, "gx")
+        if prev is not None:
+            b.out, b.out_sC = _gd_plane(prev["out"], "the previous block's out")
+            b.act = int(prev["act"])
+            if prev.get("noise") is not None and prev.get("dnw") is not None:
+                pn = prev["noise"].contiguous()
+                _need_cuda(pn, prev["dnw"], prev["out"])
+                b.noise, b.dnw = pn.data_ptr(), _vec(prev["dnw"], d.Cin, "gendense_bwd").data_ptr()
+    _count("kg_gendense", 2.0 * n * Mh * d.Cin)
+    _check(lib.kg_gendense_bwd(C.byref(b), _stream()), "kg_gendense_bwd")
+    return dict(zf=zf, gyc=gyc, gx=gx)
+
+
 def _rowsum_fill(a, x, y, want_second: int, out, out2, accumulate: int):
     n, c, t, v = x.shape
     a.N, a.C, a.T, a.V = n, c, t, v
diff --git a/kinetic-gan_amd/build.py b/kinetic-gan_amd/build.py
--- a/kinetic-gan_amd/build.py
+++ b/kinetic-gan_amd/build.py
@@ -8,7 +8,7 @@
 ROOT = os.path.dirname(PKG)
 CSRC = os.path.join(PKG, "csrc")
 LIB = os.path.join(PKG, "libkgan_hip.so")
-SOURCES = ["kg_conv.hip", "kg_wgrad.hip", "kg_agg.hip", "kg_aggconv.hip", "kg_gen.hip", "kg_genblock.hip", "kg_disc.hip", "kg_map.hip", "kg_comm.hip", "kg_misc.hip", "kg_mmd.hip", "kg_input.hip", "kg_sample.hip", "kg_eval.hip", "kg_prdc.hip", "kg_frechet.hip", "kg_cls.hip", "kg_nn.hip", "kg_nn_gram.hip", "kg_kin.hip"]
+SOURCES = ["kg_conv.hip", "kg_wgrad.hip", "kg_agg.hip", "kg_aggconv.hip", "kg_gen.hip", "kg_genblock.hip", "kg_disc.hip", "kg_map.hip", "kg_gendense.hip", "kg_comm.hip", "kg_misc.hip", "kg_mmd.hip", "kg_input.hip", "kg_sample.hip", "kg_eval.hip", "kg_prdc.hip", "kg_frechet.hip", "kg_cls.hip", "kg_nn.hip", "kg_nn_gram.hip", "kg_kin.hip"]
 
 
 def _stale() -> bool:
diff --git a/kinetic-gan_amd/csrc/kg_gendense.hip b/kinetic-gan_amd/csrc/kg_gendense.hip
--- /dev/null
+++ b/kinetic-gan_amd/csrc/kg_gendense.hip
@@ -0,0 +1,455 @@
+#include "kg_bn_math.h"
+#include "kg_common.h"
+#include "kg_linear_tile.h"
+
+namespace {
+
+constexpr int RT_MAX = KG_GD_MAX_BN_ROWS / 32;
+constexpr int MAXG = KG_GD_MAX_GROUPS;
+
+__device__ __forceinline__ float half_sum(float v) {
+#pragma unroll
+    for (int m = 16; m >= 1; m >>= 1) v += __shfl_xor(v, m, 64);
+    return v;
+}
+
+template <int TAPS, int NACC, bool XROW, int RTW>
+__global__ __launch_bounds__(NTM) void kg_gendense_fwd_kernel(const KgGenDenseArgs a) {
+    __shared__ float red[NWV * 16 * 64];
+    const int tid = threadIdx.x, lane = tid & 63, wave = tid >> 6;
+    const int l32 = lane & 31, h = lane >> 5;
+    const int o0 = blockIdx.x * 32;
+    const bool second = o0 >= a.C;
+    const int ow = o0 + l32 - (second ? a.C : 0);
+    const __amdgpu_buffer_rsrc_t rw = second ? rsrc_of(a.w2, (long)a.Cr * a.K * 4) : rsrc_of(a.w, (long)a.C * a.K * TAPS * 4);
+    const int xs = a.stage == KG_GD_TCN ? a.rep : 1;
+    const __amdgpu_buffer_rsrc_t rx = rsrc_of(a.x, XROW ? (long)a.N * a.x_ld * 4 : ((long)(a.K - 1) * a.x_ld + (long)a.N * xs) * 4);
+    constexpr int NJ = TAPS == 3 ? (NACC == 3 ? 2 : 4) : (RTW > 1 ? 8 : 5);
+    constexpr int KSN = NWV / RTW;
+    const int wrt = wave / KSN, ks = wave % KSN;
+    auto tile_of = [&](int i) { return ((int)blockIdx.y + (i / RTW) * (int)gridDim.y) * RTW + i % RTW; };
+    const int nch = (a.K + 7) / 8;
+    const int nrt = (a.N + 31) / 32;
+    float val[RT_MAX][NACC];
+#pragma unroll
+    for (int i = 0; i < RT_MAX; ++i)
+#pragma unroll
+        for (int q = 0; q < NACC; ++q) val[i][q] = 0.f;
+#pragma unroll
+    for (int p = 0; p < RT_MAX / RTW; ++p) {
+        if (tile_of(p * RTW) >= nrt) continue;
+        const int rt = tile_of(p * RTW) + wrt;
+        const int n = rt * 32 + l32;
+        const bool n_ok = rt < nrt && n < a.N;
+        kg_f32x16 acc[NACC];
+#pragma unroll
+        for (int q = 0; q < NACC; ++q)
+#pragma unroll
+            for (int r = 0; r < 16; ++r) acc[q][r] = 0.f;
+        for (int c0 = ks; c0 < nch; c0 += KSN * NJ) {
+            float av[NJ][TAPS][4], bv[NJ][4];
+#pragma unroll
+            for (int j = 0; j < NJ; ++j) {
+                const int c = c0 + KSN * j;
+                const int k = c * 8 + 4 * h;
+                const bool live = c < nch && k < a.K;
+                const unsigned woff = (unsigned)(((long)ow * a.K + k) * TAPS) * 4u;
+#pragma unroll
+                for (int q = 0; q < TAPS; ++q) load_vec<4>(rw, live ? woff + 16u * q : OOB, av[j][q]);
+                if constexpr (XROW) {
+                    load_vec<4>(rx, (live && n_ok) ? (unsigned)((long)n * a.x_ld + k) * 4u : OOB, bv[j]);
+                } else {
+#pragma unroll
+                    for (int t = 0; t < 4; ++t) bv[j][t] = load1(rx, (live && n_ok) ? (unsigned)((long)(k + t) * a.x_ld + (long)n * xs) * 4u : OOB);
+                }
+            }
+#pragma unroll
+            for (int j = 0; j < NJ; ++j)
+#pragma unroll
+                for (int t = 0; t < 4; ++t) {
+                    if constexpr (TAPS == 1) {
+                        acc[0] = __builtin_amdgcn_mfma_f32_32x32x2f32(av[j][0][t], bv[j][t], acc[0], 0, 0, 0);
+                    } else if constexpr (NACC == 1) {
+                        acc[0] = __builtin_amdgcn_mfma_f32_32x32x2f32(av[j][(3 * t + 1) / 4][(3 * t + 1) % 4], bv[j][t], acc[0], 0, 0, 0);
+                    } else {
+#pragma unroll
+                        for (int q = 0; q < 3; ++q)
+                            acc[q] = __builtin_amdgcn_mfma_f32_32x32x2f32(av[j][(3 * t + q) / 4][(3 * t + q) % 4], bv[j][t], acc[q], 0, 0, 0);
+                    }
+                }
+        }
+#pragma unroll
+        for (int q = 0; q < NACC; ++q) {
+            if (q > 0 || p > 0) __syncthreads();
+#pragma unroll
+            for (int r = 0; r < 16; ++r) red[(wave * 16 + r) * 64 + lane] = acc[q][r];
+            __syncthreads();
+#pragma unroll
+            for (int j = 0; j < RTW; ++j) {
+                float v = 0.f;
+#pragma unroll
+                for (int k2 = 0; k2 < KSN; ++k2) v += red[((j * KSN + k2) * 16 + wave) * 64 + lane];
+                val[p * RTW + j][q] = v;
+            }
+        }
+    }
+    const int o = o0 + row_of_reg(wave, h);
+    const int ng = a.N / a.groups;
+    const float cnt = (float)ng * (float)a.rep;
+    int grp[RT_MAX];
+#pragma unroll
+    for (int i = 0; i < RT_MAX; ++i) {
+        const int rt = tile_of(i);
+        const int n = rt * 32 + l32;
+        grp[i] = (rt < nrt && n < a.N) ? n / ng : -1;
+    }
+    const float nmid = (float)(a.rep - 2);
+    auto frame_sum = [&](const float (&v)[NACC]) {
+        if constexpr (NACC == 1) return (float)a.rep * v[0];
+        else return (v[0] + v[2]) + nmid * v[1];
+    };
+    auto frame_sq = [&](const float (&v)[NACC], float m) {
+        if constexpr (NACC == 1) return (float)a.rep * ((v[0] - m) * (v[0] - m));
+        else return ((v[0] - m) * (v[0] - m) + (v[2] - m) * (v[2] - m)) + nmid * ((v[1] - m) * (v[1] - m));
+    };
+    float sc[MAXG], sh[MAXG];
+    auto bn_finish = [&](int cb, int Cb) {
+        const float gam = a.gamma ? a.gamma[cb] : 1.f, bet = a.beta ? a.beta[cb] : 0.f;
+#pragma unroll
+        for (int g = 0; g < MAXG; ++g) {
+            sc[g] = 1.f; sh[g] = 0.f;
+            if (g >= a.groups) continue;
+            float s = 0.f;
+#pragma unroll
+            for (int i = 0; i < RT_MAX; ++i) s += grp[i] == g ? frame_sum(val[i]) : 0.f;
+            const float mean = half_sum(s) / cnt;
+            float q = 0.f;
+#pragma unroll
+            for (int i = 0; i < RT_MAX; ++i) q += grp[i] == g ? frame_sq(val[i], mean) : 0.f;
+            const float var = half_sum(q) / cnt;
+            float lc[4];
+            kg_bn_fwd_coef(lc, 1, 0, mean, var, gam, bet, a.eps);
+            sc[g] = lc[0]; sh[g] = lc[1];
+            if (l32 == 0) {
+                kg_bn_fwd_coef(a.coef + (long)g * 4 * Cb, Cb, cb, mean, var, gam, bet, a.eps);
+                if (a.running_mean) kg_bn_running_update(a.running_mean[cb], a.running_var[cb], a.momentum, mean, var, cnt);
+            }
+        }
+        if (l32 == 0 && cb == 0 && a.num_batches_tracked) *a.num_batches_tracked += a.groups;
+    };
+    if (a.stage == KG_GD_HEAD) {
+        const float as = a.a ? *a.a : 1.f;
+        const int cr = o - a.C;
+        const float rb = (second && a.bias) ? a.bias[cr] : 0.f;
+#pragma unroll
+        for (int i = 0; i < RT_MAX; ++i) {
+            if (grp[i] < 0) continue;
+            const int n = tile_of(i) * 32 + l32;
+            const float v = val[i][0];
+            a.yc[(long)o * a.yc_sC + n] = v;
+            if (!second) {
+                float* zp = a.z + (long)o * a.z_sC + (long)n * a.rep;
+                for (int t = 0; t < a.rep; ++t) zp[t] = v * as;
+            } else {
+                const float rv = v + rb;
+                val[i][0] = rv;
+                float* rp = a.r + (long)cr * a.r_sC + (long)n * a.rep;
+                for (int t = 0; t < a.rep; ++t) rp[t] = rv;
+            }
+        }
+        if (second && a.coef) bn_finish(cr, a.Cr);
+        return;
+    }
+    const float bt = a.bias ? a.bias[o] : 0.f;
+#pragma unroll
+    for (int i = 0; i < RT_MAX; ++i) {
+        if constexpr (NACC == 1) {
+            val[i][0] += bt;
+        } else {
+            const float p0 = val[i][0], p1 = val[i][1], p2 = val[i][2];
+            val[i][0] = (p1 + p2) + bt;
+            val[i][1] = ((p0 + p1) + p2) + bt;
+            val[i][2] = (p0 + p1) + bt;
+        }
+    }
+    if (a.coef) bn_finish(o, a.C);
+    const float nwc = (a.nw && a.noise) ? a.nw[o] : 0.f;
+#pragma unroll
+    for (int i = 0; i < RT_MAX; ++i) {
+        if (grp[i] < 0) continue;
+        const int n = tile_of(i) * 32 + l32;
+        float sx = 1.f, bx = 0.f, sr = 1.f, br = 0.f;
+#pragma unroll
+        for (int g = 0; g < MAXG; ++g)
+            if (grp[i] == g) { sx = sc[g]; bx = sh[g]; }
+        if (a.coef_r) {
+            sr = a.coef_r[(long)grp[i] * 4 * a.C + o];
+            br = a.coef_r[(long)grp[i] * 4 * a.C + a.C + o];
+        }
+        const float rv = a.r ? a.r[(long)o * a.r_sC + (long)n * a.rep] : 0.f;
+        float* up = a.u + (long)o * a.u_sC + (long)n * a.rep;
+        float* op = a.out + (long)o * a.out_sC + (long)n * a.rep;
+        const float* np = a.noise + (long)n * a.rep;
+        for (int t = 0; t < a.rep; ++t) {
+            float v;
+            if constexpr (NACC == 1) v = val[i][0];
+            else v = t == 0 ? val[i][0] : (t == a.rep - 1 ? val[i][2] : val[i][1]);
+            up[t] = v;
+            if (a.coef) { v *= sx; v += bx; }
+            if (a.r) v += a.coef_r ? rv * sr : rv;
+            if (a.coef_r) v += br;
+            if (a.nw && a.noise) v = fmaf(nwc, np[t], v);
+            op[t] = kg_act(v, a.act, a.slope);
+        }
+    }
+}
+
+template <int REP>
+__global__ __launch_bounds__(NTM) void kg_gendense_bwd_tcn_kernel(const KgGenDenseBwdArgs a) {
+    __shared__ float red[NWV * 16 * 64];
+    const int tid = threadIdx.x, lane = tid & 63, wave = tid >> 6;
+    const int l32 = lane & 31, h = lane >> 5;
+    const int i0 = blockIdx.x * 32, n0 = blockIdx.y * 32;
+    const int il = i0 + l32, n = n0 + l32;
+    const bool n_ok = n < a.N;
+    const int rep = REP > 0 ? REP : a.rep;
+    const __amdgpu_buffer_rsrc_t rw = rsrc_of(a.w, (long)a.C * a.C * 3 * 4);
+    const __amdgpu_buffer_rsrc_t rd = rsrc_of(a.du, ((long)(a.C - 1) * a.du_sC + (long)a.N * rep) * 4);
+    constexpr int NJ = REP > 0 ? 4 : 1;
+    constexpr int NT3 = REP == 1 ? 1 : 3;
+    kg_f32x16 acc;
+#pragma unroll
+    for (int r = 0; r < 16; ++r) acc[r] = 0.f;
+    const int nch = a.C / 4;
+    for (int c0 = wave; c0 < nch; c0 += NWV * NJ) {
+        float av[NJ][2][NT3], sv[NJ][2][NT3];
+#pragma unroll
+        for (int j = 0; j < NJ; ++j) {
+            const int q = c0 + NWV * j;
+            const bool live = q < nch;
+#pragma unroll
+            for (int t2 = 0; t2 < 2; ++t2) {
+                const int c = q * 4 + 2 * h + t2;
+                const unsigned woff = (unsigned)(((long)c * a.C + il) * 3) * 4u;
+                if constexpr (REP == 1) {
+                    av[j][t2][0] = load1(rw, live ? woff + 4u : OOB);
+                    sv[j][t2][0] = load1(rd, (live && n_ok) ? (unsigned)((long)c * a.du_sC + n) * 4u : OOB);
+                } else {
+#pragma unroll
+                    for (int p = 0; p < 3; ++p) av[j][t2][p] = load1(rw, live ? woff + 4u * p : OOB);
+                    const unsigned doff = (unsigned)((long)c * a.du_sC + (long)n * rep) * 4u;
+                    float s0 = 0.f, s1 = 0.f, s2 = 0.f;
+                    if constexpr (REP > 0) {
+                        float d[REP];
+#pragma unroll
+                        for (int t = 0; t < REP; ++t) d[t] = load1(rd, (live && n_ok) ? doff + 4u * t : OOB);
+#pragma unroll
+                        for (int t = 0; t < REP; ++t) {
+                            s1 += d[t];
+                            if (t >= 1) s0 += d[t];
+                            if (t <= REP - 2) s2 += d[t];
+                        }
+                    } else {
+                        for (int t = 0; t < rep; ++t) {
+                            const float d = load1(rd, (live && n_ok) ? doff + 4u * t : OOB);
+                            s1 += d;
+                            if (t >= 1) s0 += d;
+                            if (t <= rep - 2) s2 += d;
+                        }
+                    }
+                    sv[j][t2][0] = s0; sv[j][t2][1] = s1; sv[j][t2][2] = s2;
+                }
+            }
+        }
+#pragma unroll
+        for (int j = 0; j < NJ; ++j)
+#pragma unroll
+            for (int t2 = 0; t2 < 2; ++t2)
+#pragma unroll
+                for (int p = 0; p < NT3; ++p) acc = __builtin_amdgcn_mfma_f32_32x32x2f32(av[j][t2][p], sv[j][t2][p], acc, 0, 0, 0);
+    }
+    const float v = reduce_rows(acc, red, wave, lane);
+    const int i = i0 + row_of_reg(wave, h);
+    if (!n_ok) return;
+    const float as = a.a ? *a.a : 1.f;
+    a.zf[(long)i * a.zf_sC + n] = v;
+    a.gyc[(long)i * a.gyc_sC + n] = v * as;
+    if (a.dr) {
+        const float* dp = a.dr + (long)i * a.dr_sC + (long)n * rep;
+        float s = 0.f;
+        for (int t = 0; t < rep; ++t) s += dp[t];
+        a.gyc[(long)(a.C + i) * a.gyc_sC + n] = s;
+    }
+}
+
+template <bool ROWMAJ, bool TAIL>
+__global__ __launch_bounds__(NTM) void kg_gendense_bwd_head_kernel(const KgGenDenseBwdArgs a) {
+    __shared__ float red[NWV * 16 * 64];
+    const int tid = threadIdx.x, lane = tid & 63, wave = tid >> 6;
+    const int l32 = lane & 31, h = lane >> 5;
+    const int i0 = blockIdx.x * 32;
+    const int il = i0 + l32;
+    const bool i_ok = il < a.K;
+    const int M = a.C + a.Cr;
+    const __amdgpu_buffer_rsrc_t rw1 = rsrc_of(a.w, (long)a.C * a.K * 4), rw2 = rsrc_of(a.w2, (long)a.Cr * a.K * 4);
+    const __amdgpu_buffer_rsrc_t rg = rsrc_of(a.gyc, ((long)(M - 1) * a.gyc_sC + a.N) * 4);
+    constexpr int NJ = 4;
+    const int nch = M / 8;
+    const int nrt = (a.N + 31) / 32;
+    float nws = 0.f;
+    for (int rt = blockIdx.y; rt < nrt; rt += gridDim.y) {
+        const int n = rt * 32 + l32;
+        const bool n_ok = n < a.N;
+        kg_f32x16 acc;
+#pragma unroll
+        for (int r = 0; r < 16; ++r) acc[r] = 0.f;
+        for (int c0 = wave; c0 < nch; c0 += NWV * NJ) {
+            float wv[NJ][4], gv[NJ][4];
+#pragma unroll
+            for (int j = 0; j < NJ; ++j) {
+                const int c = c0 + NWV * j;
+                const int k = c * 8 + 4 * h;
+                const bool live = c < nch;
+                const bool sec = k >= a.C;
+#pragma unroll
+                for (int t = 0; t < 4; ++t) {
+                    const unsigned woff = (unsigned)((long)(k + t - (sec ? a.C : 0)) * a.K + il) * 4u;
+                    wv[j][t] = load1(sec ? rw2 : rw1, (live && i_ok) ? woff : OOB);
+                    gv[j][t] = load1(rg, (live && n_ok) ? (unsigned)((long)(k + t) * a.gyc_sC + n) * 4u : OOB);
+                }
+            }
+#pragma unroll
+            for (int j = 0; j < NJ; ++j)
+#pragma unroll
+                for (int t = 0; t < 4; ++t) {
+                    if constexpr (ROWMAJ) acc = __builtin_amdgcn_mfma_f32_32x32x2f32(gv[j][t], wv[j][t], acc, 0, 0, 0);
+                    else                  acc = __builtin_amdgcn_mfma_f32_32x32x2f32(wv[j][t], gv[j][t], acc, 0, 0, 0);
+                }
+        }
+        if (rt != (int)blockIdx.y) __syncthreads();
+        float v = reduce_rows(acc, red, wave, lane);
+        if constexpr (ROWMAJ) {
+            const int nn = rt * 32 + row_of_reg(wave, h);
+            if (i_ok && nn < a.N) a.gx[(long)nn * a.gx_ld + il] = v;
+        } else {
+            const int i = i0 + row_of_reg(wave, h);
+            if (i < a.K && n_ok) {
+                if constexpr (TAIL) {
+                    v *= kg_dact_from_out(a.out[(long)i * a.out_sC + n], a.act, a.slope);
+                    if (a.noise) nws = fmaf(v, a.noise[n], nws);
+                }
+                a.gx[(long)i * a.gx_ld + n] = v;
+            }
+        }
+    }
+    if constexpr (TAIL) {
+        const int i = i0 + row_of_reg(wave, h);
+        nws = half_sum(nws);
+        if (l32 == 0 && i < a.K && a.dnw && a.noise) a.dnw[i] += nws;
+    }
+}
+
+bool aligned16(const void* p) { return ((uintptr_t)p & 15) == 0; }
+
+}
+
+static int gendense_fwd(const KgGenDenseArgs* a, void* stream, bool launch) {
+    KG_REQUIRE(a != nullptr, "kg_gendense_fwd: null args");
+    KG_REQUIRE(a->stage == KG_GD_HEAD || a->stage == KG_GD_TCN, "kg_gendense_fwd: stage=%d", a->stage);
+    KG_REQUIRE(a->N > 0 && a->K > 0 && a->C > 0 && a->Cr >= 0, "kg_gendense_fwd: bad dims N=%d K=%d C=%d Cr=%d", a->N, a->K, a->C, a->Cr);
+    KG_REQUIRE(a->K % 4 == 0 && a->C % 32 == 0 && a->Cr % 32 == 0, "kg_gendense_fwd: K=%d %% 4, C=%d / Cr=%d %% 32", a->K, a->C, a->Cr);
+    KG_REQUIRE(a->rep >= 1 && a->rep <= 64, "kg_gendense_fwd: rep=%d outside [1, 64]", a->rep);
+    KG_REQUIRE(a->groups >= 1 && a->groups <= KG_GD_MAX_GROUPS && a->N % a->groups == 0, "kg_gendense_fwd: groups=%d (1..%d, dividing N=%d)",
+               a->groups, KG_GD_MAX_GROUPS, a->N);
+    KG_REQUIRE(a->x != nullptr && a->w != nullptr, "kg_gendense_fwd: null x / w");
+    KG_REQUIRE(aligned16(a->w) && aligned16(a->w2), "kg_gendense_fwd: w / w2 not 16-byte aligned");
+    KG_REQUIRE(a->act == KG_ACT_NONE || a->act == KG_ACT_LRELU || a->act == KG_ACT_TANH, "kg_gendense_fwd: act=%d", a->act);
+    KG_REQUIRE((long)a->N * a->rep * (a->C + a->Cr) < (1L << 28) && (long)(a->C + a->Cr) * a->K * 3 < (1L << 28),
+               "kg_gendense_fwd: operand too large for 32-bit offsets");
+    const bool bn = a->coef != nullptr;
+    KG_REQUIRE(!bn || a->N <= KG_GD_MAX_BN_ROWS, "kg_gendense_fwd: statistics need N=%d <= %d rows", a->N, KG_GD_MAX_BN_ROWS);
+    KG_REQUIRE(!bn || a->momentum >= 0.f, "kg_gendense_fwd: cumulative moving average (momentum < 0) is kg_bn_fwd's");
+    KG_REQUIRE((a->running_mean == nullptr) == (a->running_var == nullptr), "kg_gendense_fwd: running_mean / running_var");
+    const int nrt = kg_cdiv(a->N, 32);
+    hipStream_t s = (hipStream_t)stream;
+    if (a->stage == KG_GD_HEAD) {
+        KG_REQUIRE(a->Cr == 0 || a->w2 != nullptr, "kg_gendense_fwd: residual rows without w2");
+        KG_REQUIRE(a->yc != nullptr && a->z != nullptr && (a->Cr == 0 || a->r != nullptr), "kg_gendense_fwd: null yc / z / r");
+        KG_REQUIRE(!bn || a->Cr > 0, "kg_gendense_fwd: head statistics are the residual branch's");
+        KG_REQUIRE(a->yc_sC >= a->N && a->z_sC >= (long)a->N * a->rep && (a->Cr == 0 || a->r_sC >= (long)a->N * a->rep), "kg_gendense_fwd: plane strides");
+        dim3 grid((a->C + a->Cr) / 32, bn ? 1 : nrt);
+        if (a->x_rowmajor) {
+            KG_REQUIRE(a->x_ld >= a->K && a->x_ld % 4 == 0 && aligned16(a->x), "kg_gendense_fwd: sample-major x needs x_ld %% 4 == 0 and 16-byte alignment");
+            if (!launch) return 0;
+            if (bn) hipLaunchKernelGGL((kg_gendense_fwd_kernel<1, 1, true, 4>), grid, dim3(NTM), 0, s, *a);
+            else    hipLaunchKernelGGL((kg_gendense_fwd_kernel<1, 1, true, 1>), grid, dim3(NTM), 0, s, *a);
+        } else {
+            KG_REQUIRE(a->x_ld >= a->N, "kg_gendense_fwd: x_ld=%ld < N=%d", (long)a->x_ld, a->N);
+            if (!launch) return 0;
+            if (bn) hipLaunchKernelGGL((kg_gendense_fwd_kernel<1, 1, false, 4>), grid, dim3(NTM), 0, s, *a);
+            else    hipLaunchKernelGGL((kg_gendense_fwd_kernel<1, 1, false, 1>), grid, dim3(NTM), 0, s, *a);
+        }
+        return kg_launch_status("kg_gendense_fwd");
+    }
+    KG_REQUIRE(a->Cr == 0 && a->x_rowmajor == 0 && a->x_ld >= (long)a->N * a->rep, "kg_gendense_fwd: the temporal conv reads a plane of rep frames (Cr = 0)");
+    KG_REQUIRE(a->u != nullptr && a->out != nullptr, "kg_gendense_fwd: null u / out");
+    KG_REQUIRE(a->u_sC >= (long)a->N * a->rep && a->out_sC >= (long)a->N * a->rep && (a->r == nullptr || a->r_sC >= (long)a->N * a->rep),
+               "kg_gendense_fwd: plane strides");
+    KG_REQUIRE(a->coef_r == nullptr || a->r != nullptr, "kg_gendense_fwd: coef_r without r");
+    if (!launch) return 0;
+    dim3 grid(a->C / 32, bn ? 1 : nrt);
+    if (a->rep == 1 && bn) hipLaunchKernelGGL((kg_gendense_fwd_kernel<3, 1, false, 4>), grid, dim3(NTM), 0, s, *a);
+    else if (a->rep == 1)  hipLaunchKernelGGL((kg_gendense_fwd_kernel<3, 1, false, 1>), grid, dim3(NTM), 0, s, *a);
+    else if (bn)           hipLaunchKernelGGL((kg_gendense_fwd_kernel<3, 3, false, 4>), grid, dim3(NTM), 0, s, *a);
+    else                   hipLaunchKernelGGL((kg_gendense_fwd_kernel<3, 3, false, 1>), grid, dim3(NTM), 0, s, *a);
+    return kg_launch_status("kg_gendense_fwd");
+}
+
+extern "C" int kg_gendense_fwd(const KgGenDenseArgs* a, void* stream) { return gendense_fwd(a, stream, true); }
+extern "C" int kg_gendense_check(const KgGenDenseArgs* a) { return gendense_fwd(a, nullptr, false); }
+
+static int gendense_bwd(const KgGenDenseBwdArgs* a, void* stream, bool launch) {
+    KG_REQUIRE(a != nullptr, "kg_gendense_bwd: null args");
+    KG_REQUIRE(a->stage == KG_GD_HEAD || a->stage == KG_GD_TCN, "kg_gendense_bwd: stage=%d", a->stage);
+    KG_REQUIRE(a->N > 0 && a->C > 0 && a->Cr >= 0 && a->C % 32 == 0 && a->Cr % 32 == 0, "kg_gendense_bwd: bad dims N=%d C=%d Cr=%d", a->N, a->C, a->Cr);
+    KG_REQUIRE(a->rep >= 1 && a->rep <= 64, "kg_gendense_bwd: rep=%d outside [1, 64]", a->rep);
+    KG_REQUIRE(a->w != nullptr && a->gyc != nullptr && a->gyc_sC >= a->N, "kg_gendense_bwd: null w / gyc, gyc_sC");
+    KG_REQUIRE((long)a->N * a->rep * (a->C + a->Cr) < (1L << 28), "kg_gendense_bwd: operand too large for 32-bit offsets");
+    const int nrt = kg_cdiv(a->N, 32);
+    hipStream_t s = (hipStream_t)stream;
+    if (a->stage == KG_GD_TCN) {
+        KG_REQUIRE(a->du != nullptr && a->zf != nullptr, "kg_gendense_bwd: null du / zf");
+        KG_REQUIRE(a->du_sC >= (long)a->N * a->rep && a->zf_sC >= a->N, "kg_gendense_bwd: plane strides");
+        KG_REQUIRE(a->dr == nullptr || (a->Cr == a->C && a->dr_sC >= (long)a->N * a->rep), "kg_gendense_bwd: dr needs Cr == C and its stride");
+        KG_REQUIRE((long)a->C * a->C * 3 < (1L << 28), "kg_gendense_bwd: weight too large for 32-bit offsets");
+        if (!launch) return 0;
+        dim3 grid(a->C / 32, nrt);
+        if (a->rep == 1)      hipLaunchKernelGGL(kg_gendense_bwd_tcn_kernel<1>, grid, dim3(NTM), 0, s, *a);
+        else if (a->rep == 2) hipLaunchKernelGGL(kg_gendense_bwd_tcn_kernel<2>, grid, dim3(NTM), 0, s, *a);
+        else if (a->rep == 4) hipLaunchKernelGGL(kg_gendense_bwd_tcn_kernel<4>, grid, dim3(NTM), 0, s, *a);
+        else                  hipLaunchKernelGGL(kg_gendense_bwd_tcn_kernel<0>, grid, dim3(NTM), 0, s, *a);
+        return kg_launch_status("kg_gendense_bwd");
+    }
+    KG_REQUIRE(a->K > 0 && (long)(a->C + a->Cr) * a->K < (1L << 28), "kg_gendense_bwd: K=%d", a->K);
+    KG_REQUIRE(a->Cr == 0 || a->w2 != nullptr, "kg_gendense_bwd: residual rows without w2");
+    KG_REQUIRE(a->gx != nullptr && a->gx_ld >= (a->gx_rowmajor ? a->K : a->N), "kg_gendense_bwd: gx / gx_ld");
+    const int it = kg_cdiv(a->K, 32);
+    if (a->gx_rowmajor) {
+        KG_REQUIRE(a->out == nullptr, "kg_gendense_bwd: the tail rides on a plane gx only");
+        if (!launch) return 0;
+        hipLaunchKernelGGL((kg_gendense_bwd_head_kernel<true, false>), dim3(it, nrt), dim3(NTM), 0, s, *a);
+    } else if (a->out != nullptr) {
+        KG_REQUIRE(a->N <= KG_GD_MAX_BN_ROWS && a->out_sC >= a->N, "kg_gendense_bwd: the tail needs N=%d <= %d rows", a->N, KG_GD_MAX_BN_ROWS);
+        KG_REQUIRE(a->act == KG_ACT_NONE || a->act == KG_ACT_LRELU || a->act == KG_ACT_TANH, "kg_gendense_bwd: act=%d", a->act);
+        KG_REQUIRE((a->dnw == nullptr) == (a->noise == nullptr), "kg_gendense_bwd: dnw and noise go together");
+        if (!launch) return 0;
+        hipLaunchKernelGGL((kg_gendense_bwd_head_kernel<false, true>), dim3(it, 1), dim3(NTM), 0, s, *a);
+    } else {
+        if (!launch) return 0;
+        hipLaunchKernelGGL((kg_gendense_bwd_head_kernel<false, false>), dim3(it, nrt), dim3(NTM), 0, s, *a);
+    }
+    return kg_launch_status("kg_gendense_bwd");
+}
+
+extern "C" int kg_gendense_bwd(const KgGenDenseBwdArgs* a, void* stream) { return gendense_bwd(a, stream, true); }
+extern "C" int kg_gendense_bwd_check(const KgGenDenseBwdArgs* a) { return gendense_bwd(a, nullptr, false); }
diff --git a/kinetic-gan_amd/csrc/kg_linear_tile.h b/kinetic-gan_amd/csrc/kg_linear_tile.h
--- /dev/null
+++ b/kinetic-gan_amd/csrc/kg_linear_tile.h
@@ -0,0 +1,51 @@
+#pragma once
+#include "kg_common.h"
+
+namespace {
+
+constexpr int NTM = 1024;
+constexpr int NWV = 16;
+constexpr unsigned OOB = 0x80000000u;
+typedef float kg_f32x4 __attribute__((ext_vector_type(4)));
+typedef float kg_f32x2 __attribute__((ext_vector_type(2)));
+
+__device__ __forceinline__ __amdgpu_buffer_rsrc_t rsrc_of(const void* p, long bytes) {
+    return __builtin_amdgcn_make_buffer_rsrc(kg_uniform_ptr(p), 0, p ? (int)(bytes > 0x7fffffffL ? 0x7fffffffL : bytes) : 0, 0x00020000);
+}
+__device__ __forceinline__ float load1(__amdgpu_buffer_rsrc_t r, unsigned off) {
+    return __builtin_bit_cast(float, __builtin_amdgcn_raw_buffer_load_b32(r, off, 0, 0));
+}
+
+template <int VW>
+__device__ __forceinline__ void load_vec(__amdgpu_buffer_rsrc_t r, unsigned off, float (&v)[VW]) {
+    if constexpr (VW == 4) {
+        const kg_f32x4 t = __builtin_bit_cast(kg_f32x4, __builtin_amdgcn_raw_buffer_load_b128(r, off, 0, 0));
+        v[0] = t[0]; v[1] = t[1]; v[2] = t[2]; v[3] = t[3];
+    } else if constexpr (VW == 2) {
+        const kg_f32x2 t = __builtin_bit_cast(kg_f32x2, __builtin_amdgcn_raw_buffer_load_b64(r, off, 0, 0));
+        v[0] = t[0]; v[1] = t[1];
+    } else {
+        v[0] = load1(r, off);
+    }
+}
+template <int VW>
+__device__ __forceinline__ void mask_tail(float (&v)[VW], int k, int len) {
+    if (k + VW > len) {
+#pragma unroll
+        for (int t = 0; t < VW; ++t)
+            if (k + t >= len) v[t] = 0.f;
+    }
+}
+
+__device__ __forceinline__ float reduce_rows(const kg_f32x16& acc, float* red, int wave, int lane) {
+#pragma unroll
+    for (int r = 0; r < 16; ++r) red[(wave * 16 + r) * 64 + lane] = acc[r];
+    __syncthreads();
+    float v = 0.f;
+#pragma unroll
+    for (int w = 0; w < NWV; ++w) v += red[(w * 16 + wave) * 64 + lane];
+    return v;
+}
+__device__ __forceinline__ int row_of_reg(int r, int h) { return (r & 3) + 8 * (r >> 2) + 4 * h; }
+
+}
diff --git a/kinetic-gan_amd/csrc/kg_map.hip b/kinetic-gan_amd/csrc/kg_map.hip
--- a/kinetic-gan_amd/csrc/kg_map.hip
+++ b/kinetic-gan_amd/csrc/kg_map.hip
@@ -1,53 +1,10 @@
 #include "kg_common.h"
+#include "kg_linear_tile.h"
 
 namespace {
 
-constexpr int NTM = 1024;
-constexpr int NWV = 16;
 constexpr int NJB = 6;
 constexpr int NJA = 5;
-constexpr unsigned OOB = 0x80000000u;
-typedef float kg_f32x4 __attribute__((ext_vector_type(4)));
-typedef float kg_f32x2 __attribute__((ext_vector_type(2)));
-
-__device__ __forceinline__ __amdgpu_buffer_rsrc_t rsrc_of(const void* p, long bytes) {
-    return __builtin_amdgcn_make_buffer_rsrc(kg_uniform_ptr(p), 0, p ? (int)(bytes > 0x7fffffffL ? 0x7fffffffL : bytes) : 0, 0x00020000);
-}
-__device__ __forceinline__ float load1(__amdgpu_buffer_rsrc_t r, unsigned off) {
-    return __builtin_bit_cast(float, __builtin_amdgcn_raw_buffer_load_b32(r, off, 0, 0));
-}
-
-template <int VW>
-__device__ __forceinline__ void load_vec(__amdgpu_buffer_rsrc_t r, unsigned off, float (&v)[VW]) {
-    if constexpr (VW == 4) {
-        const kg_f32x4 t = __builtin_bit_cast(kg_f32x4, __builtin_amdgcn_raw_buffer_load_b128(r, off, 0, 0));
-        v[0] = t[0]; v[1] = t[1]; v[2] = t[2]; v[3] = t[3];
-    } else if constexpr (VW == 2) {
-        const kg_f32x2 t = __builtin_bit_cast(kg_f32x2, __builtin_amdgcn_raw_buffer_load_b64(r, off, 0, 0));
-        v[0] = t[0]; v[1] = t[1];
-    } else {
-        v[0] = load1(r, off);
-    }
-}
-template <int VW>
-__device__ __forceinline__ void mask_tail(float (&v)[VW], int k, int len) {
-    if (k + VW > len) {
-#pragma unroll
-        for (int t = 0; t < VW; ++t)
-            if (k + t >= len) v[t] = 0.f;
-    }
-}
-
-__device__ __forceinline__ float reduce_rows(const kg_f32x16& acc, float* red, int wave, int lane) {
-#pragma unroll
-    for (int r = 0; r < 16; ++r) red[(wave * 16 + r) * 64 + lane] = acc[r];
-    __syncthreads();
-    float v = 0.f;
-#pragma unroll
-    for (int w = 0; w < NWV; ++w) v += red[(w * 16 + wave) * 64 + lane];
-    return v;
-}
-__device__ __forceinline__ int row_of_reg(int r, int h) { return (r & 3) + 8 * (r >> 2) + 4 * h; }
 
 template <int VW>
 __device__ __forceinline__ void load_xin(const KgLinearArgs& a, __amdgpu_buffer_rsrc_t rx, __amdgpu_buffer_rsrc_t re, int n, long lab, int k,
diff --git a/kinetic-gan_amd/gen_trunk.py b/kinetic-gan_amd/gen_trunk.py
--- a/kinetic-gan_amd/gen_trunk.py
+++ b/kinetic-gan_amd/gen_trunk.py
@@ -14,6 +14,10 @@
 SLOPE = 0.2
 FUSED = os.environ.get("KG_GEN_FUSED", "1") != "0"
 FUSED_MIN_COLS = int(os.environ.get("KG_GEN_FUSED_MINCOLS", "16"))
+DENSE = os.environ.get("KG_GEN_DENSE", "1") != "0"
+DENSE_BN_FWD = os.environ.get("KG_GEN_DENSE_BN_FWD", "0") == "1"
+_NV_CONV, _NV_GEN_EXPAND, _NV_GENDENSE_FWD, _NV_GENDENSE_BWD = nv.conv, nv.gen_expand, nv.gendense_fwd, nv.gendense_bwd
+_dense_ok = {}
 
 
 class GenBlockGeom:
@@ -156,6 +160,33 @@
             nv.genblock_supported(g.dims, n, p["wg"], p["wr"] if g.res == "conv" else None, p["wt"], backward=backward))
 
 
+def dense_geometry(g: GenBlockGeom, n: int, groups: int = 1, backward: bool = False, tail: bool = False) -> bool:
+    if not (g.ok and g.V == 1 and g.Vc == 1 and g.Tc == 1 and g.Kp == 1 and g.U is None and g.res in ("none", "conv")):
+        return False
+    key = (g.dims, n, groups, backward, tail)
+    if key not in _dense_ok:
+        _dense_ok[key] = nv.gendense_geometry_ok(g.dims, n, groups, backward=backward, tail=tail)
+    return _dense_ok[key]
+
+
+def _dense_route(g: GenBlockGeom, n: int, p, x, groups: int = 1, backward: bool = False) -> bool:
+    if not (DENSE and x.is_cuda and nv.conv is _NV_CONV and nv.gen_expand is _NV_GEN_EXPAND and
+            nv.gendense_fwd is _NV_GENDENSE_FWD and nv.gendense_bwd is _NV_GENDENSE_BWD):
+        return False
+    ws = [p["wg"], p["wt"]] + ([p["wr"]] if g.res == "conv" else [])
+    if not all(t.is_cuda and t.is_contiguous() and t.data_ptr() % 16 == 0 for t in ws):
+        return False
+    if x.stride(1) == 1 and x.shape[0] > 1 and (x.data_ptr() % 16 or x.stride(0) % 4):
+        return False
+    if not backward and (g.bn_t or g.res == "conv") and not DENSE_BN_FWD:
+        return False
+    return dense_geometry(g, n, groups, backward=backward)
+
+
+def _no_bn_tail(g: GenBlockGeom) -> bool:
+    return not g.bn_t and g.res == "none"
+
+
 def fwd_pass(meta: GenTrunkMeta, w, noise, adjs, params, bns, groups: int, keep: bool):
     x = w.view(w.shape[0], w.shape[1], 1, 1)
     tape = []
@@ -165,6 +196,15 @@
         p = meta.block_params(params, i)
         bn_t, bn_r = bns[i]
         n, C = nall, g.cout
+        if x is not None and _dense_route(g, n, p, x, groups):
+            res = nv.gendense_fwd(g.dims, x=x, wg=p["wg"], wr=p["wr"], br=p["br"], wt=p["wt"], bt=p["bt"], a_eff=adjs[i],
+                                  bn_t=_bn_job(bn_t, p["gam_t"], p["bet_t"]) if bn_t is not None else None,
+                                  bn_r=_bn_job(bn_r, p["gam_r"], p["bet_r"]) if bn_r is not None else None,
+                                  groups=groups, noise=noise[i], nw=p["nw"], slope=SLOPE)
+            if keep:
+                tape.append(dict(x=x, **res))
+            x = res["out"]
+            continue
         if _fusable(g, n, p):
             res = nv.genblock_fwd(g.dims, x=x if pend is None else None, pend=pend, wg=p["wg"], wr=p["wr"], br=p["br"],
                                   wt=p["wt"], bt=p["bt"], B=adjs[i], U=g.U,
@@ -228,6 +268,7 @@
     outer_jobs, adj_jobs = [], []
     sl = slice(lo, hi)
     coef_next = None
+    tail_done = False
     for i in range(meta.nb - 1, -1, -1):
         geo = meta.geoms[i]
         tp = tape[i]
@@ -238,6 +279,33 @@
         st = geo.spec_t
         wt_sink = ops._sink_of(p["wt"])
         wg_sink = ops._sink_of(p["wg"])
+        if _dense_route(geo, n, p, x, backward=True):
+            if tail_done:
+                du, dr = g, None
+            else:
+                du, dr = nv.gen_tail_bwd(g, out, geo.act, slope=SLOPE, coef=coef_next, **tail)
+            coef_next, tail_done = None, False
+            prev = None
+            if i > 0:
+                pg, pp = meta.geoms[i - 1], meta.block_params(params, i - 1)
+                if _no_bn_tail(pg) and _dense_route(pg, n, pp, tape[i - 1]["x"][sl], backward=True) and \
+                        dense_geometry(geo, n, backward=True, tail=True):
+                    prev = dict(out=tape[i - 1]["out"][sl], act=pg.act, noise=noise[i - 1][sl], dnw=ops._sink_of(pp["nw"]))
+            res = nv.gendense_bwd(geo.dims, du=du, dr=dr if geo.res == "conv" else None, wg=p["wg"], wr=p["wr"], wt=p["wt"],
+                                  a_eff=adjs[i], gx_rowmajor=i == 0, prev=prev, want_gx=i > 0 or need_gx0, slope=SLOPE)
+            gyc, zf = res["gyc"], res["zf"]
+            ops._wgrad_into(wt_sink[1:] if geo.T == 1 else wt_sink, z, du, st)
+            ops._rowsum_into([ops._sink_of(p["bt"])], du)
+            ops._wgrad_into(wg_sink[:geo.Mg * geo.cin], x, gyc[:, :geo.Mg], geo.spec_g)
+            if geo.res == "conv":
+                ops._wgrad_into(ops._sink_of(p["wr"]), x, gyc[:, geo.Mg:], geo.spec_r)
+                ops._rowsum_into([ops._sink_of(p["br"])], dr)
+            dbt = nv.agg_outer(zf, yc[:, :geo.Mg], geo.Kp, 1, defer=outer_jobs)
+            adj_jobs.append(dict(dbt=dbt, u=geo.U, a=geo.A_fixed, out=imp_sinks[i].view(geo.K, geo.V, geo.V), accumulate=True))
+            g, tail_done = res["gx"], prev is not None
+            if g is None:
+                break
+            continue
         if _fusable(geo, n, p, backward=True):
             coef = coef_next if coef_next is not None else nv.gen_tail_bwd(g, out, geo.act, slope=SLOPE, stats_only=True, **tail)
             prev = None
```

Result: no change. 20790 samples/s, median of 6 (+0.6%).
